# amaas/stanford-ctc

Measured on AMD Instinct MI355X. Metric: audio frames/sec (CTC fwd-bwd + BRNN grad) at T=1000, L=5, H=1824, |Sigma|=33, higher is better.
Workload: dtype f32; 1 GPU; WSJ-shape cfg-3: T=1000 A=33 5x1824 BRNN (temporalLayer 3, inputDim 483) U=100, minibatch 32 per GPU, one costAndGrad per step; utterances_per_gpu=32, parallelism=single-gpu

## Files before the change

### include/sctc.h

```cpp
#ifndef SCTC_H_
#define SCTC_H_

#include <stddef.h>
#include <stdint.h>

#ifdef __cplusplus
extern "C" {
#endif

#define SCTC_ABI_VERSION 6

#define SCTC_OK 0
#define SCTC_ERR_ARG (-1)
#define SCTC_ERR_HIP (-2)
#define SCTC_ERR_WORKSPACE (-3)
#define SCTC_ERR_TIMEOUT (-4)
#define SCTC_ERR_STATE (-5)

#define SCTC_F32 0
#define SCTC_F64 1
#define SCTC_F16 2
#define SCTC_BF16 3
#define SCTC_BF16X3 4
#define SCTC_OPERANDS_16BIT 0x100
// ... 262 lines not shown
int sctc_word_lm_score_batch(const sctc_word_lm_score_config* cfg, const int32_t* labels_dev, float* terms_dev,
                             int32_t* word_ids_dev, double* sums_dev, int32_t* counts_dev, int32_t* status_dev,
                             void* workspace_dev, size_t workspace_bytes, void* stream);

int sctc_nbest_rank_words_batch(int32_t B, int32_t K, const int32_t* K_b, const int32_t* U_b, double alpha, double beta,
                                const double* scores_dev, const int32_t* status_dev, const double* lm_sums_dev,
                                const double* first_scores_dev, const double* word_sums_dev,
                                const int32_t* word_counts_dev, const int32_t* word_status_dev, double word_alpha,
                                double word_beta, double* rescored_dev, int32_t* order_dev, void* stream);


typedef struct sctc_intern_config {
    int32_t N;
    int32_t G;
    int32_t A;
    int32_t space;
    const int32_t* U_b;
    const int64_t* label_off;
    const int32_t* group_off;
} sctc_intern_config;

int sctc_intern_words_workspace_bytes(const sctc_intern_config* cfg, size_t* bytes);

int sctc_intern_words_batch(const sctc_intern_config* cfg, const int32_t* labels_dev, int32_t* word_ids_dev,
                            int32_t* counts_dev, int32_t* status_dev, void* workspace_dev, size_t workspace_bytes,
                            void* stream);

#define SCTC_MBR_CHARS 0
#define SCTC_MBR_WORDS 1
#define SCTC_MBR_CONF 1
#define SCTC_MBR_DIST 2

typedef struct sctc_mbr_config {
    int32_t B;
    int32_t K;
    int32_t unit;
    int32_t flags;
    int32_t A;
    int32_t space;
    double scale;
    const int32_t* K_b;
    const int32_t* U_b;
    const int64_t* label_off;
} sctc_mbr_config;

int sctc_nbest_mbr_workspace_bytes(const sctc_mbr_config* cfg, size_t* bytes);

int sctc_nbest_mbr_batch(const sctc_mbr_config* cfg, const int32_t* labels_dev, const double* scores_dev,
                         const int32_t* order_dev, double* post_dev, double* risk_dev, int32_t* best_dev,
                         int32_t* mbr_order_dev, int32_t* dist_dev, double* conf_dev, int32_t* conf_len_dev,
                         void* workspace_dev, size_t workspace_bytes, void* stream);


#define SCTC_TNC_LOG_PROBS 0
#define SCTC_TNC_LOGITS 1

typedef struct sctc_tnc_config {
    int32_t T, N, C;
    int32_t dtype;
    int32_t mode;
    int32_t blank;
    int64_t stride_t, stride_n, stride_c;
} sctc_tnc_config;


int sctc_ctc_tnc_probs(const sctc_tnc_config* cfg, const void* input_dev, const int32_t* T_n_dev, void* probs_dev,
                       void* stream);

int sctc_ctc_tnc_empty(const sctc_tnc_config* cfg, const void* probs_dev, const int32_t* T_n_dev, const int32_t* idx_dev,
                       const int32_t* sym_dev, int32_t n_idx, void* grad_dev, double* cost_dev, int32_t* skip_dev,
                       void* stream);

int sctc_ctc_tnc_grad(const sctc_tnc_config* cfg, const void* grad_dev, const int32_t* T_n_dev, const double* cost_dev,
                      const int32_t* skip_dev, const double* scale_dev, void* out_dev, void* stream);

typedef struct sctc_mwer_config {
    int32_t T, N, K, C;
    int32_t dtype;
    int32_t mode;
    int64_t stride_t, stride_n, stride_c;
    double scale;
    int32_t subtract_mean;
} sctc_mwer_config;

int sctc_ctc_mwer_probs(const sctc_mwer_config* cfg, const void* input_dev, const int32_t* T_n_dev, const int32_t* K_n_dev,
                        void* probs_dev, void* stream);

int sctc_ctc_mwer_coef(const sctc_mwer_config* cfg, const double* cost_dev, const int32_t* skip_dev, const double* errors_dev,
                       const int32_t* T_n_dev, const int32_t* K_n_dev, double* loss_dev, double* coef_dev,
                       double* posterior_dev, double* expected_dev, int32_t* real_dev, int32_t* inactive_dev, void* stream);

int sctc_ctc_mwer_combine(const sctc_mwer_config* cfg, const void* probs_dev, const void* grad_dev, const double* coef_dev,
                          const int32_t* real_dev, const int32_t* T_n_dev, const int32_t* inactive_dev, void* out_dev,
                          void* stream);


typedef struct sctc_brnn_config {
    int32_t input_dim;
    int32_t output_dim;
    int32_t layer_size;
    int32_t num_layers;
    int32_t temporal_layer;
    int32_t max_frames;
    int32_t max_utts;
    float max_act;
    float reg;
    int32_t train;
    int32_t operand_dtype;
} sctc_brnn_config;

typedef struct sctc_tensor_info {
    int64_t offset;
    int32_t rows, cols, ld, kind;
} sctc_tensor_info;

typedef struct sctc_brnn_sizes {
    int64_t param_elems;
    int64_t param_count;
    size_t workspace_bytes;
    int32_t n_tensors;
} sctc_brnn_sizes;

typedef struct sctc_brnn* sctc_brnn_t;

int sctc_brnn_query(const sctc_brnn_config* cfg, sctc_brnn_sizes* out);
int sctc_brnn_create(const sctc_brnn_config* cfg, float* params_dev, float* grads_dev,
                     void* workspace_dev, size_t workspace_bytes, sctc_brnn_t* out);
int sctc_brnn_destroy(sctc_brnn_t h);
int sctc_brnn_tensor_info(sctc_brnn_t h, int32_t index, sctc_tensor_info* out);

typedef struct sctc_minibatch {
    int32_t B;
    const int32_t* T_b;
    const float* feats_dev;
    const int32_t* labels;
    const int32_t* U_b;
} sctc_minibatch;

#define SCTC_FLAG_SYNC_SKIP 1
#define SCTC_FLAG_ACCUMULATE 2
#define SCTC_FLAG_NO_REG_GRAD 4

int sctc_brnn_cost_and_grad(sctc_brnn_t h, const sctc_minibatch* mb, int32_t flags,
                            double* cost_host, int32_t* skip_host, double* regcost_host,
                            void* stream);
int sctc_brnn_cost_and_grad_async(sctc_brnn_t h, const sctc_minibatch* mb, int32_t flags,
                                  double* cost_dev, int32_t* skip_dev, void* stream);
void* sctc_brnn_grad_event(sctc_brnn_t h, int32_t index);
int sctc_stream_wait_event(void* stream, void* event);
int sctc_brnn_allreduce_grads(sctc_brnn_t h, void* rccl_comm, void* compute_stream, void* side_stream,
                              double* side_dev, int32_t side_count, int32_t backward_queued);
int sctc_brnn_check(sctc_brnn_t h, void* stream);
int sctc_brnn_recurrent_path(sctc_brnn_t h, int32_t* forward_path, int32_t* bptt_path, int32_t* retries);

int sctc_brnn_forward(sctc_brnn_t h, const sctc_minibatch* mb, float* probs_dev, void* stream);

int sctc_brnn_ctc_workspace_bytes(sctc_brnn_t h, const sctc_minibatch* mb, size_t* needed, size_t* reserved);
int sctc_brnn_set_ctc_workspace(sctc_brnn_t h, void* workspace_dev, size_t workspace_bytes);

typedef struct sctc_mwer_minibatch {
    int32_t K;
    const int32_t* K_b;
    const int32_t* hyp_labels;
    const int32_t* hyp_U;
    const double* errors;
    double scale;
    int32_t subtract_mean;
    double ctc_weight;
} sctc_mwer_minibatch;

typedef struct sctc_mwer_outputs {
    double* loss;
    double* expected;
    int32_t* inactive;
    double* ctc_cost;
    int32_t* ctc_skip;
    double* posterior;
    int32_t* real;
} sctc_mwer_outputs;

int sctc_brnn_mwer_workspace_bytes(sctc_brnn_t h, const sctc_minibatch* mb, const sctc_mwer_minibatch* mw, size_t* needed);
int sctc_brnn_set_mwer_workspace(sctc_brnn_t h, void* workspace_dev, size_t workspace_bytes);

int sctc_brnn_mwer_cost_and_grad(sctc_brnn_t h, const sctc_minibatch* mb, const sctc_mwer_minibatch* mw, int32_t flags,
                                 const sctc_mwer_outputs* out_host, double* regcost_host, void* stream);
int sctc_brnn_mwer_cost_and_grad_async(sctc_brnn_t h, const sctc_minibatch* mb, const sctc_mwer_minibatch* mw, int32_t flags,
                                       const sctc_mwer_outputs* out_dev, void* stream);

#define SCTC_PHASE_FWD_GEMM 0
#define SCTC_PHASE_FWD_REC 1
#define SCTC_PHASE_CTC 2
#define SCTC_PHASE_BWD_GEMM 3
#define SCTC_PHASE_BWD_REC 4
#define SCTC_PHASE_OTHER 5
#define SCTC_N_PHASES 6
int sctc_brnn_set_profiling(sctc_brnn_t h, int32_t enable);
int sctc_brnn_debug_buffer(sctc_brnn_t h, int32_t which, void** dev_ptr, int64_t* rows, int64_t* cols,
                           int64_t* ld);
int sctc_brnn_debug_buffer16(sctc_brnn_t h, int32_t which, void** dev_ptr, int64_t* rows, int64_t* cols,
                             int64_t* ld, int32_t* dtype);
int sctc_brnn_debug_read(sctc_brnn_t h, uint32_t* out, int32_t n_words);
int sctc_brnn_phase_ms(sctc_brnn_t h, float* ms_out );
int sctc_brnn_flops(sctc_brnn_t h, const sctc_minibatch* mb, double* total, double* gemm,
                    double* recurrent);

int sctc_gemm_f32(const float* A_dev, int64_t lda, int32_t a_kcontig, const float* B_dev,
                  int64_t ldb, int32_t b_kcontig, float* C_dev, int64_t ldc, int32_t M, int32_t N,
                  int32_t K, const float* bias_dev, int32_t relu, void* workspace_dev,
                  size_t workspace_bytes, void* stream);

int sctc_gemm_h16(const float* A_dev, int64_t lda, int32_t a_kcontig, const float* B_dev,
                  int64_t ldb, int32_t b_kcontig, float* C_dev, int64_t ldc, int32_t M, int32_t N,
                  int32_t K, const float* bias_dev, int32_t relu, int32_t operand_dtype,
                  void* workspace_dev, size_t workspace_bytes, void* stream);


int sctc_axpy(float* y_dev, const float* x_dev, float alpha, int64_t n, void* stream);
int sctc_scale(float* x_dev, float alpha, int64_t n, void* stream);
int sctc_sumsq(const float* x_dev, int64_t n, double* out_dev, void* workspace_dev,
               size_t workspace_bytes, void* stream);
int sctc_nesterov_step(float* w_dev, float* v_dev, const float* g_dev, int64_t n, float mom,
                       float alpha, float max_gnorm, float grad_scale, const double* sumsq_dev,
                       void* stream);

int sctc_sumsq_reg(const float* g_dev, const float* w_dev, const float* v_dev, float mom,
                   float grad_scale, float reg, int64_t n,
                   const int64_t* noreg_ranges_host, int32_t n_ranges, double* out_dev,
                   void* workspace_dev, size_t workspace_bytes, void* stream);
int sctc_nesterov_step_reg(float* w_dev, float* v_dev, const float* g_dev, int64_t n, float mom,
                           float alpha, float max_gnorm, float grad_scale, float reg,
                           const int64_t* noreg_ranges_host, int32_t n_ranges,
                           const double* sumsq_dev, void* stream);

#ifdef __cplusplus
}
#endif
#endif
```

### stanford-ctc_amd/_sctc.py

```python
import ctypes
import os

_HERE = os.path.dirname(os.path.abspath(__file__))
LIB_PATH = os.environ.get("SCTC_LIB_PATH") or os.path.join(_HERE, "libsctc_hip.so")

F32, F64, F16, BF16, BF16X3 = 0, 1, 2, 3, 4

c_i32p = ctypes.POINTER(ctypes.c_int32)
c_i64p = ctypes.POINTER(ctypes.c_int64)
c_f32p = ctypes.POINTER(ctypes.c_float)
c_f64p = ctypes.POINTER(ctypes.c_double)
vp = ctypes.c_void_p


class CtcBatch(ctypes.Structure):
    _fields_ = [("B", ctypes.c_int32), ("A", ctypes.c_int32), ("blank", ctypes.c_int32),
                ("dtype", ctypes.c_int32), ("ld", ctypes.c_int64), ("T_b", c_i32p),
                ("U_b", c_i32p), ("frame_off", c_i64p), ("labels", c_i32p),
                ("label_off", c_i64p), ("rowbase_dev", vp)]


class BrnnConfig(ctypes.Structure):
    _fields_ = [("input_dim", ctypes.c_int32), ("output_dim", ctypes.c_int32),
                ("layer_size", ctypes.c_int32), ("num_layers", ctypes.c_int32),
# ... 98 lines not shown


def word_lm_slots(U_b):
    import numpy as np
    per = (np.asarray(U_b, dtype=np.int64) + 1) // 2 + 1
    cuts = np.concatenate([[0], np.cumsum(per)]).astype(np.int64)
    return cuts[:-1], int(cuts[-1])


class InternConfig(ctypes.Structure):
    _fields_ = [("N", ctypes.c_int32), ("G", ctypes.c_int32), ("A", ctypes.c_int32), ("space", ctypes.c_int32),
                ("U_b", c_i32p), ("label_off", c_i64p), ("group_off", c_i32p)]


class MbrConfig(ctypes.Structure):
    _fields_ = [("B", ctypes.c_int32), ("K", ctypes.c_int32), ("unit", ctypes.c_int32), ("flags", ctypes.c_int32),
                ("A", ctypes.c_int32), ("space", ctypes.c_int32), ("scale", ctypes.c_double), ("K_b", c_i32p),
                ("U_b", c_i32p), ("label_off", c_i64p)]


MBR_CHARS, MBR_WORDS = 0, 1
MBR_CONF, MBR_DIST = 1, 2
MBR_MAX_U = ALIGN_MAX_U


def intern_slots(U_b):
    import numpy as np
    per = (np.asarray(U_b, dtype=np.int64) + 1) // 2
    cuts = np.concatenate([[0], np.cumsum(per)]).astype(np.int64)
    return cuts[:-1], int(cuts[-1])


class TncConfig(ctypes.Structure):
    _fields_ = [("T", ctypes.c_int32), ("N", ctypes.c_int32), ("C", ctypes.c_int32), ("dtype", ctypes.c_int32),
                ("mode", ctypes.c_int32), ("blank", ctypes.c_int32), ("stride_t", ctypes.c_int64),
                ("stride_n", ctypes.c_int64), ("stride_c", ctypes.c_int64)]


TNC_LOG_PROBS, TNC_LOGITS = 0, 1
TNC_LANE_MAX_C = 32


class MwerConfig(ctypes.Structure):
    _fields_ = [("T", ctypes.c_int32), ("N", ctypes.c_int32), ("K", ctypes.c_int32), ("C", ctypes.c_int32),
                ("dtype", ctypes.c_int32), ("mode", ctypes.c_int32), ("stride_t", ctypes.c_int64),
                ("stride_n", ctypes.c_int64), ("stride_c", ctypes.c_int64), ("scale", ctypes.c_double),
                ("subtract_mean", ctypes.c_int32)]


class MwerMinibatch(ctypes.Structure):
    _fields_ = [("K", ctypes.c_int32), ("K_b", c_i32p), ("hyp_labels", c_i32p), ("hyp_U", c_i32p), ("errors", c_f64p),
                ("scale", ctypes.c_double), ("subtract_mean", ctypes.c_int32), ("ctc_weight", ctypes.c_double)]


class MwerOutputs(ctypes.Structure):
    _fields_ = [("loss", vp), ("expected", vp), ("inactive", vp), ("ctc_cost", vp), ("ctc_skip", vp), ("posterior", vp),
                ("real", vp)]


MWER_MAX_K = 256

N_PHASES = 6

PROTOTYPES = {
    "sctc_abi_version": (ctypes.c_int, []),
    "sctc_last_error": (ctypes.c_char_p, []),
    "sctc_set_device": (ctypes.c_int, [ctypes.c_int]),
    "sctc_device_info": (ctypes.c_int, [c_i32p, c_i32p, c_i64p, ctypes.c_char_p, ctypes.c_int]),
    "sctc_set_shared_device": (ctypes.c_int, [ctypes.c_int32]),
    "sctc_shared_device": (ctypes.c_int, []),
    "sctc_device_pci_bus_id": (ctypes.c_int, [ctypes.c_int32, ctypes.c_char_p, ctypes.c_int32]),
    "sctc_ctc_workspace_bytes": (ctypes.c_size_t, [ctypes.POINTER(CtcBatch)]),
    "sctc_ctc_loss_batch": (ctypes.c_int, [ctypes.POINTER(CtcBatch), vp, vp, vp, vp, vp,
                                           ctypes.c_size_t, vp]),
    "sctc_softmax_rows": (ctypes.c_int, [vp, vp, ctypes.c_int64, ctypes.c_int32, ctypes.c_int64,
                                         vp]),
    "sctc_argmax_rows": (ctypes.c_int, [vp, ctypes.c_int32, vp, ctypes.c_int64, ctypes.c_int32,
                                        ctypes.c_int64, vp]),
    "sctc_lm_create": (ctypes.c_int, [vp, vp, vp, ctypes.c_int64, ctypes.c_int32, ctypes.c_int32,
                                      ctypes.POINTER(vp)]),
    "sctc_lm_destroy": (ctypes.c_int, [vp]),
    "sctc_ctc_beam_workspace_bytes": (ctypes.c_size_t, [ctypes.POINTER(BeamConfig)]),
    "sctc_ctc_beam_decode_batch": (ctypes.c_int, [ctypes.POINTER(BeamConfig), vp, vp, vp, vp, vp,
                                                  ctypes.c_size_t, vp]),
    "sctc_lexicon_create": (ctypes.c_int, [vp, vp, ctypes.c_int64, ctypes.c_int32, ctypes.c_int32, vp, vp,
                                           ctypes.c_int64, vp, vp, ctypes.c_int64, ctypes.c_int32,
                                           ctypes.POINTER(vp)]),
    "sctc_lexicon_create_ngram": (ctypes.c_int, [vp, vp, ctypes.c_int64, ctypes.c_int32, ctypes.c_int32, vp, vp,
                                                 ctypes.c_int64, vp, vp, vp, vp, ctypes.c_int64, ctypes.c_int64,
                                                 ctypes.c_int32, ctypes.c_int32, ctypes.POINTER(vp)]),
    "sctc_lexicon_destroy": (ctypes.c_int, [vp]),
    "sctc_lexicon_bytes": (ctypes.c_size_t, [vp]),
    "sctc_ctc_lexbeam_workspace_bytes": (ctypes.c_size_t, [ctypes.POINTER(LexBeamConfig)]),
    "sctc_ctc_lexbeam_decode_batch": (ctypes.c_int, [ctypes.POINTER(LexBeamConfig), vp, vp, vp, vp, vp,
                                                     ctypes.c_size_t, vp]),
    "sctc_nnlm_create": (ctypes.c_int, [ctypes.c_int32, ctypes.c_int32, ctypes.c_int32, c_i32p, ctypes.POINTER(vp),
                                        ctypes.POINTER(vp), ctypes.c_int32, ctypes.c_int32, ctypes.POINTER(vp)]),
    "sctc_nnlm_destroy": (ctypes.c_int, [vp]),
    "sctc_nnlm_bytes": (ctypes.c_size_t, [vp]),
    "sctc_nnlm_rows": (ctypes.c_int, [vp, vp, ctypes.c_int64, vp, vp]),
    "sctc_ctc_nnbeam_workspace_bytes": (ctypes.c_size_t, [ctypes.POINTER(NNBeamConfig)]),
    "sctc_ctc_nnbeam_decode_batch": (ctypes.c_int, [ctypes.POINTER(NNBeamConfig), vp, vp, vp, vp, vp,
                                                    ctypes.c_size_t, vp]),
    "sctc_rnnlm_create": (ctypes.c_int, [ctypes.c_int32, ctypes.c_int32, vp, vp, vp, vp, vp, ctypes.c_int32,
                                         ctypes.POINTER(vp)]),
    "sctc_rnnlm_destroy": (ctypes.c_int, [vp]),
    "sctc_rnnlm_bytes": (ctypes.c_size_t, [vp]),
    "sctc_rnnlm_step": (ctypes.c_int, [vp, vp, vp, ctypes.c_int64, vp, vp, vp]),
    "sctc_ctc_rnnbeam_workspace_bytes": (ctypes.c_size_t, [ctypes.POINTER(RNNBeamConfig)]),
    "sctc_ctc_rnnbeam_decode_batch": (ctypes.c_int, [ctypes.POINTER(RNNBeamConfig), vp, vp, vp, vp, vp,
                                                     ctypes.c_size_t, vp]),
    "sctc_edit_distance_workspace_bytes": (ctypes.c_int, [ctypes.POINTER(EditConfig), ctypes.POINTER(ctypes.c_size_t)]),
    "sctc_edit_distance_batch": (ctypes.c_int, [ctypes.POINTER(EditConfig), vp, vp, vp, vp, vp, vp, ctypes.c_size_t,
                                                vp]),
    "sctc_ctc_align_workspace_bytes": (ctypes.c_int, [ctypes.POINTER(AlignConfig), ctypes.POINTER(ctypes.c_size_t)]),
    "sctc_ctc_align_batch": (ctypes.c_int, [ctypes.POINTER(AlignConfig), vp, vp, vp, vp, vp, vp, vp, ctypes.c_size_t,
                                            vp]),
    "sctc_ctc_bestpath_batch": (ctypes.c_int, [ctypes.POINTER(BestPathConfig), vp, vp, vp, vp, vp, vp]),
    "sctc_log_rows": (ctypes.c_int, [vp, vp, ctypes.c_int64, ctypes.c_int32, ctypes.c_int64, vp]),
    "sctc_lm_score_workspace_bytes": (ctypes.c_int, [ctypes.POINTER(LmScoreConfig), ctypes.c_int32,
                                                     ctypes.POINTER(ctypes.c_size_t)]),
    "sctc_lm_score_batch": (ctypes.c_int, [ctypes.POINTER(LmScoreConfig), vp, vp, vp, vp, vp, ctypes.c_size_t, vp]),
    "sctc_nbest_rank_batch": (ctypes.c_int, [ctypes.c_int32, ctypes.c_int32, c_i32p, c_i32p, ctypes.c_double,
                                             ctypes.c_double, vp, vp, vp, vp, vp, vp, vp]),
    "sctc_word_lm_score_workspace_bytes": (ctypes.c_int, [ctypes.POINTER(WordLmScoreConfig),
                                                          ctypes.POINTER(ctypes.c_size_t)]),
    "sctc_word_lm_score_batch": (ctypes.c_int, [ctypes.POINTER(WordLmScoreConfig), vp, vp, vp, vp, vp, vp, vp,
                                                ctypes.c_size_t, vp]),
    "sctc_nbest_rank_words_batch": (ctypes.c_int, [ctypes.c_int32, ctypes.c_int32, c_i32p, c_i32p, ctypes.c_double,
                                                   ctypes.c_double, vp, vp, vp, vp, vp, vp, vp, ctypes.c_double,
                                                   ctypes.c_double, vp, vp, vp]),
    "sctc_intern_words_workspace_bytes": (ctypes.c_int, [ctypes.POINTER(InternConfig), ctypes.POINTER(ctypes.c_size_t)]),
    "sctc_intern_words_batch": (ctypes.c_int, [ctypes.POINTER(InternConfig), vp, vp, vp, vp, vp, ctypes.c_size_t, vp]),
    "sctc_nbest_mbr_workspace_bytes": (ctypes.c_int, [ctypes.POINTER(MbrConfig), ctypes.POINTER(ctypes.c_size_t)]),
    "sctc_nbest_mbr_batch": (ctypes.c_int, [ctypes.POINTER(MbrConfig), vp, vp, vp, vp, vp, vp, vp, vp, vp, vp, vp,
                                            ctypes.c_size_t, vp]),
    "sctc_ctc_tnc_probs": (ctypes.c_int, [ctypes.POINTER(TncConfig), vp, vp, vp, vp]),
    "sctc_ctc_tnc_empty": (ctypes.c_int, [ctypes.POINTER(TncConfig), vp, vp, vp, vp, ctypes.c_int32, vp, vp, vp, vp]),
    "sctc_ctc_tnc_grad": (ctypes.c_int, [ctypes.POINTER(TncConfig), vp, vp, vp, vp, vp, vp, vp]),
    "sctc_ctc_mwer_probs": (ctypes.c_int, [ctypes.POINTER(MwerConfig), vp, vp, vp, vp, vp]),
    "sctc_ctc_mwer_coef": (ctypes.c_int, [ctypes.POINTER(MwerConfig), vp, vp, vp, vp, vp, vp, vp, vp, vp, vp, vp, vp]),
    "sctc_ctc_mwer_combine": (ctypes.c_int, [ctypes.POINTER(MwerConfig), vp, vp, vp, vp, vp, vp, vp, vp]),
    "sctc_brnn_query": (ctypes.c_int, [ctypes.POINTER(BrnnConfig), ctypes.POINTER(BrnnSizes)]),
    "sctc_brnn_create": (ctypes.c_int, [ctypes.POINTER(BrnnConfig), vp, vp, vp, ctypes.c_size_t,
                                        ctypes.POINTER(vp)]),
    "sctc_brnn_destroy": (ctypes.c_int, [vp]),
    "sctc_brnn_tensor_info": (ctypes.c_int, [vp, ctypes.c_int32, ctypes.POINTER(TensorInfo)]),
    "sctc_brnn_cost_and_grad": (ctypes.c_int, [vp, ctypes.POINTER(Minibatch), ctypes.c_int32,
                                               c_f64p, c_i32p, c_f64p, vp]),
    "sctc_brnn_cost_and_grad_async": (ctypes.c_int, [vp, ctypes.POINTER(Minibatch),
                                                     ctypes.c_int32, vp, vp, vp]),
    "sctc_brnn_check": (ctypes.c_int, [vp, vp]),
    "sctc_brnn_recurrent_path": (ctypes.c_int, [vp, c_i32p, c_i32p, c_i32p]),
    "sctc_brnn_grad_event": (vp, [vp, ctypes.c_int32]),
    "sctc_stream_wait_event": (ctypes.c_int, [vp, vp]),
    "sctc_brnn_forward": (ctypes.c_int, [vp, ctypes.POINTER(Minibatch), vp, vp]),
    "sctc_brnn_ctc_workspace_bytes": (ctypes.c_int, [vp, ctypes.POINTER(Minibatch), ctypes.POINTER(ctypes.c_size_t),
                                                     ctypes.POINTER(ctypes.c_size_t)]),
    "sctc_brnn_set_ctc_workspace": (ctypes.c_int, [vp, vp, ctypes.c_size_t]),
    "sctc_brnn_mwer_workspace_bytes": (ctypes.c_int, [vp, ctypes.POINTER(Minibatch), ctypes.POINTER(MwerMinibatch),
                                                      ctypes.POINTER(ctypes.c_size_t)]),
    "sctc_brnn_set_mwer_workspace": (ctypes.c_int, [vp, vp, ctypes.c_size_t]),
    "sctc_brnn_mwer_cost_and_grad": (ctypes.c_int, [vp, ctypes.POINTER(Minibatch), ctypes.POINTER(MwerMinibatch),
                                                    ctypes.c_int32, ctypes.POINTER(MwerOutputs), c_f64p, vp]),
    "sctc_brnn_mwer_cost_and_grad_async": (ctypes.c_int, [vp, ctypes.POINTER(Minibatch), ctypes.POINTER(MwerMinibatch),
                                                          ctypes.c_int32, ctypes.POINTER(MwerOutputs), vp]),
    "sctc_brnn_set_profiling": (ctypes.c_int, [vp, ctypes.c_int32]),
    "sctc_brnn_debug_read": (ctypes.c_int, [vp, vp, ctypes.c_int32]),
    "sctc_brnn_debug_buffer": (ctypes.c_int, [vp, ctypes.c_int32, ctypes.POINTER(vp), c_i64p, c_i64p, c_i64p]),
    "sctc_brnn_debug_buffer16": (ctypes.c_int, [vp, ctypes.c_int32, ctypes.POINTER(vp), c_i64p, c_i64p, c_i64p, c_i32p]),
    "sctc_brnn_phase_ms": (ctypes.c_int, [vp, c_f32p]),
    "sctc_brnn_flops": (ctypes.c_int, [vp, ctypes.POINTER(Minibatch), c_f64p, c_f64p, c_f64p]),
    "sctc_gemm_f32": (ctypes.c_int, [vp, ctypes.c_int64, ctypes.c_int32, vp, ctypes.c_int64,
                                     ctypes.c_int32, vp, ctypes.c_int64, ctypes.c_int32,
                                     ctypes.c_int32, ctypes.c_int32, vp, ctypes.c_int32, vp,
                                     ctypes.c_size_t, vp]),
    "sctc_gemm_h16": (ctypes.c_int, [vp, ctypes.c_int64, ctypes.c_int32, vp, ctypes.c_int64,
                                     ctypes.c_int32, vp, ctypes.c_int64, ctypes.c_int32,
                                     ctypes.c_int32, ctypes.c_int32, vp, ctypes.c_int32,
                                     ctypes.c_int32, vp, ctypes.c_size_t, vp]),
    "sctc_axpy": (ctypes.c_int, [vp, vp, ctypes.c_float, ctypes.c_int64, vp]),
    "sctc_scale": (ctypes.c_int, [vp, ctypes.c_float, ctypes.c_int64, vp]),
    "sctc_sumsq": (ctypes.c_int, [vp, ctypes.c_int64, vp, vp, ctypes.c_size_t, vp]),
    "sctc_nesterov_step": (ctypes.c_int, [vp, vp, vp, ctypes.c_int64, ctypes.c_float,
                                          ctypes.c_float, ctypes.c_float, ctypes.c_float, vp,
                                          vp]),
    "sctc_brnn_allreduce_grads": (ctypes.c_int, [vp, vp, vp, vp, vp, ctypes.c_int32, ctypes.c_int32]),
    "sctc_sumsq_reg": (ctypes.c_int, [vp, vp, vp, ctypes.c_float, ctypes.c_float, ctypes.c_float, ctypes.c_int64,
                                      c_i64p, ctypes.c_int32, vp, vp, ctypes.c_size_t, vp]),
    "sctc_nesterov_step_reg": (ctypes.c_int, [vp, vp, vp, ctypes.c_int64, ctypes.c_float,
                                              ctypes.c_float, ctypes.c_float, ctypes.c_float,
                                              ctypes.c_float, c_i64p, ctypes.c_int32, vp, vp]),
}

FLAG_SYNC_SKIP = 1
FLAG_ACCUMULATE = 2
FLAG_NO_REG_GRAD = 4

_lib = None


class SctcError(RuntimeError):
    pass


def device_bus_id(device=-1):
    buf = ctypes.create_string_buffer(64)
    check(lib().sctc_device_pci_bus_id(device, buf, 64), "device_pci_bus_id")
    return buf.value.decode()


def shared_device_from_ids(ids, rank):
    me = tuple(ids[rank])
    return sum(1 for x in ids if tuple(x) == me) > 1


def resolve_shared_device(group=None, my_id=None, log=True, device=None):
    import socket
    import sys
    import torch.distributed as dist
    L = lib()
    if my_id is None:
        my_id = (socket.gethostname(), device_bus_id(-1 if device is None else int(device)))
    rank, ids = 0, [tuple(my_id)]
    if dist.is_available() and dist.is_initialized() and dist.get_world_size(group) > 1:
        rank = dist.get_rank(group)
        gathered = [None] * dist.get_world_size(group)
        dist.all_gather_object(gathered, tuple(my_id), group=group)
        ids = [tuple(x) for x in gathered]
    if "SCTC_SHARED_DEVICE" in os.environ:
        shared, why = bool(L.sctc_shared_device()), "SCTC_SHARED_DEVICE in the environment"
    else:
        shared, why = shared_device_from_ids(ids, rank), "bus ids of %d rank(s)" % len(ids)
        if shared:
            L.sctc_set_shared_device(1)
        elif L.sctc_shared_device():
            why += "; the mode was already on (a timeout or another process on this GPU) and stays on"
            shared = True
    if log:
        sys.stderr.write("sctc: rank %d -> %s %s, shared=%d (%s)\n"
                         % (rank, my_id[0], my_id[1], int(shared), why))
        sys.stderr.flush()
    return shared, ids


def lib():
    global _lib
    if _lib is None:
        if not os.path.exists(LIB_PATH):
            raise ImportError(
                "libsctc_hip.so is missing (%s): build it with `python -c 'import "
                "__graft_entry__ as g; g.build()'` -- there is no CPU fallback" % LIB_PATH)
        try:
            import torch
        except ImportError:
            pass
        L = ctypes.CDLL(LIB_PATH)
        for name, (res, args) in PROTOTYPES.items():
            fn = getattr(L, name)
            fn.restype = res
            fn.argtypes = args
        if L.sctc_abi_version() != 6:
            raise ImportError("libsctc_hip.so ABI version mismatch")
        _lib = L
    return _lib


def check(rc, what=""):
    if rc < 0:
        msg = lib().sctc_last_error()
        msg = msg.decode() if msg else ""
        if rc == -1:
            raise ValueError("%s: %s" % (what, msg))
        raise SctcError("%s failed (rc=%d): %s" % (what, rc, msg))
    return rc


def require_gpu():
    import torch
    if not torch.cuda.is_available():
        raise SctcError("no HIP device visible: the stanford-ctc MI355X path has no CPU fallback")
    return torch


def current_stream_ptr():
    import torch
    return ctypes.c_void_p(torch.cuda.current_stream().cuda_stream)


def i32(arr):
    return arr.ctypes.data_as(c_i32p)


def i64(arr):
    return arr.ctypes.data_as(c_i64p)
```

### stanford-ctc_amd/csrc/brnn_engine.hip

```cpp
#include <algorithm>
#include <cmath>
#include <numeric>
#include <vector>

#include "common.h"
#include <dlfcn.h>

#include <mutex>

#include "brnn_mwer.h"
#include "brnn_mwer_plan.h"
#include "ctc_kernels.h"
#include "elementwise.h"
#include "gemm_f32.h"
#include "recurrent.h"

namespace sctc {
int ctc_run_batch(const sctc_ctc_batch* bt, const void* probs, void* grad, double* cost,
                  int32_t* skip, void* ws, size_t ws_bytes, hipStream_t stream, void* keep_stage);
void* ctc_new_stage();
void ctc_free_stage(void* p);
}

using namespace sctc;

static constexpr int PAD = 32;
static inline int LD(int padded_dim) { return (int)((padded_dim + 63) / 64 * 64); }
static constexpr int CTC_LP_MAX = 2048;

static int fwd_prec(int operand_dtype)
{
    return operand_dtype == SCTC_F16 ? 1 : (operand_dtype == SCTC_BF16X3 ? 3 : 0);
}
static int bwd_prec(int operand_dtype)
{
    return operand_dtype == SCTC_F16 ? 2 : (operand_dtype == SCTC_BF16X3 ? 3 : 0);
}

struct sctc_brnn {
    sctc_brnn_config cfg;
    int D, Dp, H, Hp, A, Ap, NL, TL;
    int64_t maxF;
    int maxB;
    float* params;
    float* grads;
    std::vector<sctc_tensor_info> tinfo;
    int64_t param_elems, param_count;

    float* X0;
    std::vector<float*> act;
    float *Z, *hF, *hB;
    float *logits, *probs, *dlogits;
    float *dA, *dBuf, *dF, *dBk;
    std::vector<uint16_t*> act16f, act16b;
    uint16_t *hF16b = nullptr, *hB16b = nullptr, *dF16b = nullptr, *dBk16b = nullptr;
    uint16_t *dlogits16 = nullptr, *dA16 = nullptr, *dBuf16 = nullptr;
    uint16_t* W16f = nullptr;
    std::vector<uint16_t*> WT16b;
    int32_t *d_rowbase, *d_nact, *d_Ts, *d_src_row, *d_idx_lo, *d_idx_hi, *d_xbase;
    void* ctc_ws;
    size_t ctc_ws_bytes;
    void* ctc_ws_ext = nullptr;
    size_t ctc_ws_ext_bytes = 0;
    float* splitk_ws;
    int64_t splitk_floats;
    float* xbuf;
    unsigned* counters;
    unsigned* rec_debug = nullptr;
    int rec_debug_on = 0;
    double* d_cost;
    int32_t* d_skip;
    double* d_cost_out;
    int32_t* d_skip_out;
    double* d_sumsq;
    double* sumsq_ws;
    int32_t* d_perm;

    std::vector<int32_t> order, Ts, rowbase, nact, src_row, idx_lo, idx_hi, xbase;
    int64_t n_xrows = 0;
    int64_t N = 0;
    int B = 0, Tmax = 0;
    int64_t npairs = 0;
    bool pairs_contig = false;

    std::vector<hipEvent_t> grad_ev;

    int profiling = 0;
    std::vector<hipEvent_t> tev;
    int tev_phase[128];
    int tev_n = 0;
    hipEvent_t ev[SCTC_N_PHASES + 1][2];
    bool ev_ready = false;
    float phase_ms[SCTC_N_PHASES];
    int rec_sync_mode = 0;
    bool fuse_add = true;
    int rec_poll_delay = -1;
    int rec_variant = REC_V_AUTO;
    int rec_force_fallback = 0;
    int rec_path[2] = {0, 0};
    int rec_retries = 0;
    const float* last_delta1 = nullptr;
    const uint16_t* last_delta1_16 = nullptr;
    void* ctc_stage = nullptr;
    PinnedStage plan_stage;
    std::vector<int32_t> ctc_U, ctc_labels;
    std::vector<int64_t> ctc_frame_off, ctc_label_off;
    void* mwer_ws = nullptr;
    size_t mwer_ws_bytes = 0;
    PinnedStage mwer_stage;
    std::vector<int32_t> mwer_T;
    std::vector<char> mwer_head;
};

static int weight_index(const sctc_brnn* h, int layer) { return 2 * layer; }
static int bias_index(const sctc_brnn* h, int layer) { return 2 * layer + 1; }
static int wf_index(const sctc_brnn* h) { return 2 * (h->NL + 1); }
static int wb_index(const sctc_brnn* h) { return 2 * (h->NL + 1) + 1; }

struct Dims {
    int D, Dp, H, Hp, A, Ap, NL, TL;
};

static int derive_dims(const sctc_brnn_config* c, Dims* d)
{
    SCTC_CHECK_ARG(c, "brnn: null config");
    SCTC_CHECK_ARG(c->input_dim >= 1 && c->output_dim >= 2 && c->layer_size >= 1 &&
                       c->num_layers >= 1,
                   "brnn: bad dimensions (inputDim %d outputDim %d layerSize %d numLayers %d)",
                   c->input_dim, c->output_dim, c->layer_size, c->num_layers);
    SCTC_CHECK_ARG(c->max_frames >= 1 && c->max_utts >= 1, "brnn: bad capacity");
    SCTC_CHECK_ARG(c->operand_dtype == SCTC_F32 || c->operand_dtype == SCTC_F16 || c->operand_dtype == SCTC_BF16X3,
                   "brnn: operand_dtype must be SCTC_F32, SCTC_F16 or SCTC_BF16X3 (got %d)", c->operand_dtype);
    d->D = c->input_dim;
    d->H = c->layer_size;
    d->A = c->output_dim;
    d->NL = c->num_layers;
    d->TL = (c->temporal_layer <= 0 || c->temporal_layer >= c->num_layers) ? -1 : c->temporal_layer;
    d->Dp = (int)round_up(d->D, PAD);
    d->Hp = (int)round_up(d->H, PAD);
    d->Ap = (int)round_up(d->A, PAD);
    if (d->TL > 0) {
        char why[128];
        if (!recurrent_supported(d->Hp, c->max_utts, why, sizeof(why)))
            return set_error(SCTC_ERR_ARG, "brnn: %s", why);
    }
    return SCTC_OK;
}

static void build_tensor_table(const Dims& d, std::vector<sctc_tensor_info>* t, int64_t* elems,
                               int64_t* count)
{
    t->clear();
    int64_t off = 0, cnt = 0;
    for (int l = 0; l <= d.NL; ++l) {
        const int in = l == 0 ? d.D : d.H, inp = l == 0 ? d.Dp : d.Hp;
        const int out = l == d.NL ? d.A : d.H, outp = l == d.NL ? d.Ap : d.Hp;
        sctc_tensor_info w = {off, out, in, LD(inp), 0};
        t->push_back(w);
        off += (int64_t)outp * LD(inp);
        sctc_tensor_info b = {off, out, 1, 1, 1};
        t->push_back(b);
        off += outp;
        cnt += (int64_t)out * in + out;
    }
    if (d.TL > 0) {
        for (int k = 0; k < 2; ++k) {
            sctc_tensor_info w = {off, d.H, d.H, LD(d.Hp), 2};
            t->push_back(w);
            off += (int64_t)d.Hp * LD(d.Hp);
            cnt += (int64_t)d.H * d.H;
        }
    }
    *elems = off;
    *count = cnt;
}

static size_t carve(const sctc_brnn_config* c, const Dims& d, sctc_brnn* h, void* ws, size_t bytes)
{
    Arena ar;
    ar.init(ws ? ws : (void*)256, ws ? bytes : (size_t)-1 / 2);
    const int64_t F = c->max_frames;
    const int Bm = c->max_utts;
    auto f = [&](int64_t n) { return ar.take<float>((size_t)n); };
    float* X0 = f(F * LD(d.Dp));
    std::vector<float*> act(d.NL + 1);
    act[0] = X0;
    for (int i = 1; i <= d.NL; ++i) act[i] = f(F * LD(d.Hp));
    float *Z = nullptr, *hF = nullptr, *hB = nullptr;
    if (d.TL > 0) { Z = f(F * LD(d.Hp)); hF = f(F * LD(d.Hp)); hB = f(F * LD(d.Hp)); }
    float* logits = f(F * LD(d.Ap));
    float* probs = f(F * LD(d.Ap));
    float *dlogits = nullptr, *dA = nullptr, *dBuf = nullptr, *dF = nullptr, *dBk = nullptr;
    if (c->train) {
        dlogits = f(F * LD(d.Ap));
        dA = f(F * LD(d.Hp));
        dBuf = f(F * LD(d.Hp));
        if (d.TL > 0) { dF = f(F * LD(d.Hp)); dBk = f(F * LD(d.Hp)); }
    }
    const bool h16 = c->operand_dtype == SCTC_F16;
    std::vector<uint16_t*> act16f(d.NL + 1, nullptr), act16b(d.NL + 1, nullptr), WT16b(d.NL + 1, nullptr);
    uint16_t *hF16b = nullptr, *hB16b = nullptr, *dF16b = nullptr, *dBk16b = nullptr, *dlogits16 = nullptr,
             *dA16 = nullptr, *dBuf16 = nullptr, *W16f = nullptr;
    if (h16) {
        auto hh = [&](int64_t n) { return ar.take<uint16_t>((size_t)n); };
        int64_t pe = 0, pc = 0;
        {
            std::vector<sctc_tensor_info> t;
            build_tensor_table(d, &t, &pe, &pc);
        }
        W16f = hh(pe);
        for (int i = 0; i <= d.NL; ++i) {
            const int dim = i == 0 ? d.Dp : d.Hp;
            act16f[i] = hh(F * LD(dim));
            if (c->train) act16b[i] = hh(F * LD(dim));
        }
        if (c->train) {
            for (int l = 1; l <= d.NL; ++l) {
                const int outp = l == d.NL ? d.Ap : d.Hp;
                WT16b[l] = hh((int64_t)d.Hp * LD(outp));
            }
            dlogits16 = hh(F * LD(d.Ap));
            dA16 = hh(F * LD(d.Hp));
            dBuf16 = hh(F * LD(d.Hp));
            if (d.TL > 0) {
                hF16b = hh(F * LD(d.Hp)); hB16b = hh(F * LD(d.Hp));
                dF16b = hh(F * LD(d.Hp)); dBk16b = hh(F * LD(d.Hp));
            }
        }
    }
    int32_t* d_rowbase = ar.take<int32_t>(F);
    int32_t* d_nact = ar.take<int32_t>(F);
    int32_t* d_Ts = ar.take<int32_t>(Bm);
    int32_t* d_src_row = ar.take<int32_t>(F);
    int32_t* d_idx_lo = ar.take<int32_t>(F);
    int32_t* d_idx_hi = ar.take<int32_t>(F);
    int32_t* d_xbase = ar.take<int32_t>(F);
    int32_t* d_perm = ar.take<int32_t>(Bm);
    size_t ctc_bytes = 0;
    void* ctc_ws = nullptr;
    if (c->train) {
        ctc_bytes = ctc_layout_slices(CTC_GENERIC, Bm, d.A, F, F * CTC_LP_MAX, CTC_LP_MAX, 8).bytes;
        ctc_ws = ar.take<char>(ctc_bytes);
    }
    const int64_t sk = brnn_splitk_floats(d.Dp, d.Hp, d.Ap, d.NL, d.TL > 0, F, c->train != 0, bwd_prec(c->operand_dtype),
                                          c->operand_dtype == SCTC_F16, gemm_switches_from_env());
    float* splitk_ws = sk ? f(sk) : nullptr;
    float* xbuf = d.TL > 0 ? f((int64_t)recurrent_xbuf_floats(d.Hp, recurrent_xrows_bound(F, F))) : nullptr;
    unsigned* counters = ar.take<unsigned>(REC_COUNTER_WORDS);
    unsigned* rec_debug = ar.take<unsigned>(2 * REC_DEBUG_WORDS);
    double* d_cost = ar.take<double>(Bm);
    int32_t* d_skip = ar.take<int32_t>(Bm);
    double* d_cost_out = ar.take<double>(Bm);
    int32_t* d_skip_out = ar.take<int32_t>(Bm);
    double* d_sumsq = ar.take<double>(d.NL + 3);
    double* sumsq_ws = ar.take<double>(sumsq_ws_bytes() / sizeof(double));
    if (h && !ar.overflow) {
        h->X0 = X0; h->act = act; h->Z = Z; h->hF = hF; h->hB = hB;
        h->logits = logits; h->probs = probs; h->dlogits = dlogits;
        h->dA = dA; h->dBuf = dBuf; h->dF = dF; h->dBk = dBk;
        h->d_rowbase = d_rowbase; h->d_nact = d_nact; h->d_Ts = d_Ts; h->d_src_row = d_src_row;
        h->d_idx_lo = d_idx_lo; h->d_idx_hi = d_idx_hi; h->d_perm = d_perm; h->d_xbase = d_xbase;
        h->ctc_ws = ctc_ws; h->ctc_ws_bytes = ctc_bytes;
        h->splitk_ws = splitk_ws; h->splitk_floats = sk;
        h->xbuf = xbuf; h->counters = counters; h->rec_debug = rec_debug;
        h->act16f = act16f; h->act16b = act16b; h->WT16b = WT16b; h->W16f = W16f;
        h->hF16b = hF16b; h->hB16b = hB16b; h->dF16b = dF16b; h->dBk16b = dBk16b;
        h->dlogits16 = dlogits16; h->dA16 = dA16; h->dBuf16 = dBuf16;
        h->d_cost = d_cost; h->d_skip = d_skip; h->d_cost_out = d_cost_out;
        h->d_skip_out = d_skip_out; h->d_sumsq = d_sumsq; h->sumsq_ws = sumsq_ws;
    }
    return ar.overflow && ws ? 0 : ar.used;
}


static int make_plan(sctc_brnn* h, const sctc_minibatch* mb, bool need_labels, hipStream_t stream)
{
    SCTC_CHECK_ARG(mb && mb->T_b && mb->feats_dev, "brnn: null minibatch field");
    SCTC_CHECK_ARG(mb->B >= 1 && mb->B <= h->maxB, "brnn: %d utterances, capacity %d", mb->B,
                   h->maxB);
    if (need_labels) SCTC_CHECK_ARG(mb->labels && mb->U_b, "brnn: labels required for training");
    const int B = mb->B;
    int64_t N = 0;
    for (int b = 0; b < B; ++b) {
        SCTC_CHECK_ARG(mb->T_b[b] >= 1, "brnn: utterance %d has no frames", b);
        N += mb->T_b[b];
    }
    SCTC_CHECK_ARG(N <= h->maxF, "Batch size exceeds max batch (%lld frames > %lld)", (long long)N,
                   (long long)h->maxF);
    h->B = B;
    h->N = N;
    h->order.resize(B);
    std::iota(h->order.begin(), h->order.end(), 0);
    std::stable_sort(h->order.begin(), h->order.end(),
                     [&](int a, int b) { return mb->T_b[a] > mb->T_b[b]; });
    h->Ts.resize(B);
    std::vector<int64_t> foff(B);
    {
        int64_t o = 0;
        for (int b = 0; b < B; ++b) { foff[b] = o; o += mb->T_b[b]; }
    }
    for (int r = 0; r < B; ++r) h->Ts[r] = mb->T_b[h->order[r]];
    const int Tmax = h->Ts[0];
    h->Tmax = Tmax;
    h->rowbase.assign(Tmax, 0);
    h->nact.assign(Tmax, 0);
    h->xbase.assign(Tmax, 0);
    {
        int na = B;
        int64_t base = 0, xb = 0;
        for (int t = 0; t < Tmax; ++t) {
            while (na > 0 && h->Ts[na - 1] <= t) --na;
            h->nact[t] = na;
            h->rowbase[t] = (int32_t)base;
            h->xbase[t] = (int32_t)xb;
            base += na;
            xb += recurrent_step_xrows(na);
        }
        h->n_xrows = xb;
    }
    h->src_row.resize(N);
    h->idx_lo.clear();
    h->idx_hi.clear();
    for (int t = 0; t < Tmax; ++t)
        for (int r = 0; r < h->nact[t]; ++r) {
            const int row = h->rowbase[t] + r;
            h->src_row[row] = (int32_t)(foff[h->order[r]] + t);
            if (t >= 1) {
                h->idx_hi.push_back(row);
                h->idx_lo.push_back(h->rowbase[t - 1] + r);
            }
        }
    h->npairs = (int64_t)h->idx_hi.size();
    h->pairs_contig = h->npairs > 0;
    for (int64_t k = 1; k < h->npairs && h->pairs_contig; ++k)
        h->pairs_contig = h->idx_hi[k] == h->idx_hi[0] + k && h->idx_lo[k] == h->idx_lo[0] + k;
    const size_t I = sizeof(int32_t);
    const size_t total = I * (3 * (size_t)Tmax + 2 * (size_t)B + (size_t)N + 2 * (size_t)h->npairs) + 8 * 64;
    char* pin = static_cast<char*>(h->plan_stage.acquire(total));
    size_t off = 0;
    auto up = [&](void* dev, const void* src, size_t bytes) -> int {
        if (bytes == 0) return SCTC_OK;
        const void* from = src;
        if (pin) {
            memcpy(pin + off, src, bytes);
            from = pin + off;
            off += (bytes + 63) & ~(size_t)63;
        }
        SCTC_HIP_TRY(hipMemcpyAsync(dev, from, bytes, hipMemcpyHostToDevice, stream));
        return SCTC_OK;
    };
    SCTC_TRY(up(h->d_rowbase, h->rowbase.data(), I * Tmax));
    SCTC_TRY(up(h->d_nact, h->nact.data(), I * Tmax));
    SCTC_TRY(up(h->d_xbase, h->xbase.data(), I * Tmax));
    SCTC_TRY(up(h->d_Ts, h->Ts.data(), I * B));
    SCTC_TRY(up(h->d_src_row, h->src_row.data(), I * N));
    SCTC_TRY(up(h->d_perm, h->order.data(), I * B));
    SCTC_TRY(up(h->d_idx_lo, h->idx_lo.data(), I * h->npairs));
    SCTC_TRY(up(h->d_idx_hi, h->idx_hi.data(), I * h->npairs));
    if (pin) SCTC_HIP_TRY(h->plan_stage.uploaded(stream));
    return SCTC_OK;
}


struct PhaseTimer {
    sctc_brnn* h;
    hipStream_t s;
    int cur = -1;
    void mark(int phase)
    {
        if (h->tev_n >= (int)h->tev.size()) return;
        (void)hipEventRecord(h->tev[h->tev_n], s);
        h->tev_phase[h->tev_n++] = phase;
    }
    void begin(int phase)
    {
        if (!h->profiling) return;
        if (h->profiling == 2) { mark(phase); return; }
        end();
        cur = phase;
        (void)hipEventRecord(h->ev[SCTC_N_PHASES][0], s);
    }
    void end()
    {
        if (h->profiling == 2) { mark(-1); return; }
        if (!h->profiling || cur < 0) return;
        (void)hipEventRecord(h->ev[SCTC_N_PHASES][1], s);
        (void)hipEventSynchronize(h->ev[SCTC_N_PHASES][1]);
        float ms = 0.f;
        (void)hipEventElapsedTime(&ms, h->ev[SCTC_N_PHASES][0], h->ev[SCTC_N_PHASES][1]);
        h->phase_ms[cur] += ms;
        cur = -1;
    }
};

struct GemmOperand { const float* p; int64_t ld; int kcontig; };
static GemmArgs gemm_args(GemmOperand A, GemmOperand B, int64_t M, int64_t N, int64_t K, float* C, int64_t ldc, int prec)
{
    GemmArgs g;
    memset(&g, 0, sizeof(g));
    g.A = A.p; g.lda = A.ld; g.a_kcontig = A.kcontig;
    g.B = B.p; g.ldb = B.ld; g.b_kcontig = B.kcontig;
    g.M = (int)M; g.N = (int)N; g.K = (int)K;
    g.C = C; g.ldc = ldc;
    g.prec = prec;
    g.splits = 1;
    return g;
}

static int launch_gemm(const sctc_brnn* h, GemmArgs& g, hipStream_t s)
{
    const GemmPlan p = gemm_plan(g);
    if (p.splits > 1 && h->splitk_ws && p.ws_floats <= h->splitk_floats) {
        g.splits = p.splits;
        g.splitk_ws = h->splitk_ws;
    }
    return launch_gemm_f32(g, s);
}

static const float* tensor_ptr(const sctc_brnn* h, const float* base, int idx)
{
    return base + h->tinfo[idx].offset;
}

static RecArgs rec_args(const sctc_brnn* h, bool bptt, float* pre)
{
    RecArgs r;
    memset(&r, 0, sizeof(r));
    r.W[0] = tensor_ptr(h, h->params, wf_index(h));
    r.W[1] = tensor_ptr(h, h->params, wb_index(h));
    r.ldw = LD(h->Hp);
    r.transpose = bptt;
    r.descending[0] = bptt;
    r.descending[1] = !bptt;
    r.pre[0] = r.pre[1] = pre;
    r.act[0] = bptt ? h->hF : nullptr;
    r.act[1] = bptt ? h->hB : nullptr;
    r.out[0] = bptt ? h->dF : h->hF;
    r.out[1] = bptt ? h->dBk : h->hB;
    r.ld = LD(h->Hp);
    r.Hp = h->Hp;
    r.B = h->B;
    r.Tmax = h->Tmax;
    r.rowbase = h->d_rowbase;
    r.T_b = h->d_Ts;
    r.max_act = h->cfg.max_act;
    r.xbuf = h->xbuf;
    r.xbase = h->d_xbase;
    r.n_xrows = (int)h->n_xrows;
    r.counters = h->counters;
    r.sync_mode = h->rec_sync_mode;
    r.variant = h->rec_force_fallback ? REC_V_FALLBACK : h->rec_variant;
    r.poll_delay = h->rec_poll_delay;
    r.debug = h->rec_debug_on ? h->rec_debug + (bptt ? REC_DEBUG_WORDS : 0) : nullptr;
    r.prec16 = h->cfg.operand_dtype == SCTC_F16;
    r.T_host = h->Ts.data();
    return r;
}


static int run_forward(sctc_brnn* h, const sctc_minibatch* mb, hipStream_t s, PhaseTimer& pt)
{
    const int64_t N = h->N;
    pt.begin(SCTC_PHASE_OTHER);
    const bool h16 = h->cfg.operand_dtype == SCTC_F16;
    if (h16) {
        SCTC_TRY(launch_gather_rows16(h->X0, h->act16f[0], h->cfg.train ? h->act16b[0] : nullptr, LD(h->Dp),
                                      mb->feats_dev, h->D, h->d_src_row, N, h->D, s));
        SCTC_TRY(launch_cvt16(h->params, h->W16f, nullptr, round_up(h->param_elems, 4), s));
    } else {
        SCTC_TRY(launch_gather_rows(h->X0, LD(h->Dp), mb->feats_dev, h->D, h->d_src_row, N, h->D, s));
    }
    bool fused_sum = false;
    for (int i = 1; i <= h->NL + 1; ++i) {
        pt.begin(SCTC_PHASE_FWD_GEMM);
        const int l = i - 1;
        const sctc_tensor_info& wi = h->tinfo[weight_index(h, l)];
        const int inp = l == 0 ? h->Dp : h->Hp;
        const int outp = i == h->NL + 1 ? h->Ap : h->Hp;
        float* dst = i == h->NL + 1 ? h->logits : (i == h->TL ? h->Z : h->act[i]);
        GemmArgs g = gemm_args({h->act[i - 1], LD(inp), 1}, {h->params + wi.offset, LD(inp), 1}, N, outp, inp, dst, LD(outp),
                               fwd_prec(h->cfg.operand_dtype));
        g.bias = tensor_ptr(h, h->params, bias_index(h, l));
        g.relu = (i <= h->NL && i != h->TL) ? 1 : 0;
        if (fused_sum) {
            g.A = h->hF;
            g.A2 = h->hB;
            g.a_sum = h->act[i - 1];
            fused_sum = false;
        }
        if (h16) {
            g.in16 = 1;
            g.A = reinterpret_cast<const float*>(h->act16f[i - 1]);
            g.B = reinterpret_cast<const float*>(h->W16f + wi.offset);
            if (dst != h->Z && dst != h->logits) {
                g.C16a = h->act16f[i];
                g.C16b = h->cfg.train ? h->act16b[i] : nullptr;
                g.ldc16 = LD(outp);
                g.skip_c32 = 1;
            }
        }
        SCTC_TRY(launch_gemm(h, g, s));
        if (i == h->TL) {
            pt.begin(SCTC_PHASE_FWD_REC);
            const RecArgs r = rec_args(h, false, h->Z);
            SCTC_TRY(launch_recurrent(r, s, &h->rec_path[0]));
            pt.begin(SCTC_PHASE_OTHER);
            if (h16) {
                SCTC_TRY(launch_add16(nullptr, h->hF, h->hB, h->act16f[i], h->cfg.train ? h->act16b[i] : nullptr,
                                      N * LD(h->Hp), s, h->cfg.train ? h->hF16b : nullptr,
                                      h->cfg.train ? h->hB16b : nullptr));
            } else if (g.prec == 0 && h->fuse_add) {
                fused_sum = true;
            } else {
                SCTC_TRY(launch_add(h->act[i], h->hF, h->hB, N * LD(h->Hp), s));
            }
        }
    }
    pt.begin(SCTC_PHASE_CTC);
    SCTC_TRY(launch_softmax_rows(h->logits, h->probs, N, h->A, LD(h->Ap), s));
    return SCTC_OK;
}

static int check_recurrent_error(sctc_brnn* h, hipStream_t s)
{
    if (h->TL <= 0) return SCTC_OK;
    unsigned e = 0;
    SCTC_HIP_TRY(hipMemcpyAsync(&e, h->counters + 2, sizeof(unsigned), hipMemcpyDeviceToHost, s));
    SCTC_HIP_TRY(hipStreamSynchronize(s));
    if (e != 0) {
        if (!recurrent_shared_device_mode())
            fprintf(stderr, "sctc: a persistent recurrent launch timed out (its workgroups were not co-resident): "
                            "shared-device mode is on for the rest of this process\n");
        recurrent_set_shared_device_mode(1);
        return set_error(SCTC_ERR_TIMEOUT, "recurrent kernel: a persistent launch gave up waiting for "
                         "its peers (the %d workgroups of a pass were not co-resident: device shared "
                         "with another process or CU-masked); shared-device mode is now on",
                         2 * (h->Hp / 16));
    }
    return SCTC_OK;
}

template <typename Step>
static int with_retry(sctc_brnn* h, bool retry_ok, Step step)
{
    int rc = step();
    for (int attempt = 0; rc == SCTC_ERR_TIMEOUT && retry_ok && attempt < 2; ++attempt) {
        if (getenv("SCTC_VERBOSE"))
            fprintf(stderr, "sctc: %s -- retrying the step %s\n", err_buf(),
                    attempt == 0 ? "under the device lease" : "on the per-step fallback");
        ++h->rec_retries;
        h->rec_force_fallback = attempt == 1;
        rc = step();
        h->rec_force_fallback = 0;
    }
    return rc;
}


static int run_ctc(sctc_brnn* h, const sctc_minibatch* mb, hipStream_t s)
{
    const int B = h->B;
    std::vector<int32_t>& U = h->ctc_U;
    std::vector<int32_t>& labels = h->ctc_labels;
    std::vector<int64_t>& frame_off = h->ctc_frame_off;
    std::vector<int64_t>& label_off = h->ctc_label_off;
    U.assign(B, 0);
    labels.clear();
    frame_off.assign(B, 0);
    label_off.assign(B, 0);
    std::vector<int64_t> src_off(B);
    {
        int64_t o = 0;
        for (int b = 0; b < B; ++b) { src_off[b] = o; o += mb->U_b[b]; }
    }
    for (int r = 0; r < B; ++r) {
        const int b = h->order[r];
        U[r] = mb->U_b[b];
        frame_off[r] = r;
        label_off[r] = (int64_t)labels.size();
        labels.insert(labels.end(), mb->labels + src_off[b], mb->labels + src_off[b] + mb->U_b[b]);
    }
    sctc_ctc_batch bt;
    bt.B = B;
    bt.A = h->A;
    bt.blank = 0;
    bt.dtype = SCTC_F32;
    bt.ld = LD(h->Ap);
    bt.T_b = h->Ts.data();
    bt.U_b = U.data();
    bt.frame_off = frame_off.data();
    bt.labels = labels.data();
    bt.label_off = label_off.data();
    bt.rowbase_dev = h->d_rowbase;
    if (!h->ctc_stage) h->ctc_stage = ctc_new_stage();
    return ctc_run_batch(&bt, h->probs, h->dlogits, h->d_cost, h->d_skip, h->ctc_ws_ext ? h->ctc_ws_ext : h->ctc_ws,
                         h->ctc_ws_ext ? h->ctc_ws_ext_bytes : h->ctc_ws_bytes, s, h->ctc_stage);
}

__global__ void unpermute_results_kernel(const double* cost, const int32_t* skip,
                                         const int32_t* perm, int B, double* cost_out,
                                         int32_t* skip_out)
{
    const int r = blockIdx.x * blockDim.x + threadIdx.x;
    if (r < B) {
        cost_out[perm[r]] = cost[r];
        skip_out[perm[r]] = skip[r];
    }
}

static int run_backward(sctc_brnn* h, int flags, hipStream_t s, PhaseTimer& pt)
{
    const int64_t N = h->N;
    const int acc = (flags & SCTC_FLAG_ACCUMULATE) ? 1 : 0;
    const float reg = (flags & SCTC_FLAG_NO_REG_GRAD) ? 0.f : h->cfg.reg;
    const int bprec = bwd_prec(h->cfg.operand_dtype);
    const bool h16 = h->cfg.operand_dtype == SCTC_F16;
    const float* d_in = h->dlogits;
    const uint16_t* d_in16 = h->dlogits16;
    int d_in_ld = LD(h->Ap);
    float* bufs[2] = {h->dA, h->dBuf};
    uint16_t* bufs16[2] = {h->dA16, h->dBuf16};
    if (h16) {
        SCTC_TRY(launch_cvt16(h->dlogits, nullptr, h->dlogits16, N * LD(h->Ap), s));
        for (int l = 1; l <= h->NL; ++l) {
            const sctc_tensor_info& wl = h->tinfo[weight_index(h, l)];
            const int outp = l == h->NL ? h->Ap : h->Hp;
            SCTC_TRY(launch_transpose_bf16(h->params + wl.offset, LD(h->Hp), h->WT16b[l], LD(outp), outp, h->Hp, s));
        }
    }
    int which = 0;
    bool fused_sum = false;
    for (int i = h->NL; i >= 0; --i) {
        pt.begin(SCTC_PHASE_BWD_GEMM);
        const sctc_tensor_info& wi = h->tinfo[weight_index(h, i)];
        const int inp = i == 0 ? h->Dp : h->Hp;
        const int outp = i == h->NL ? h->Ap : h->Hp;
        const float* W = h->params + wi.offset;
        {
            GemmArgs g = gemm_args({d_in, d_in_ld, 0}, {h->act[i], LD(inp), 0}, outp, inp, N, h->grads + wi.offset, LD(inp), bprec);
            if (fused_sum) {
                g.A = h->dF;
                g.A2 = h->dBk;
                g.a_sum = const_cast<float*>(d_in);
                fused_sum = false;
            }
            g.accumulate = acc;
            if (reg > 0.f) { g.addend = W; g.ldadd = LD(inp); g.add_scale = reg; }
            g.colsum_a = h->grads + h->tinfo[bias_index(h, i)].offset;
            g.splitk_ws = h->splitk_ws;
            if (h16) {
                g.in16 = 1;
                g.A = reinterpret_cast<const float*>(d_in16);
                g.B = reinterpret_cast<const float*>(h->act16b[i]);
            }
            SCTC_TRY(launch_gemm(h, g, s));
            if (!(h->TL > 0 && i >= h->TL))
                SCTC_HIP_TRY(hipEventRecord(h->grad_ev[weight_index(h, i)], s));
        }
        if (i == 0) break;
        pt.begin(SCTC_PHASE_BWD_GEMM);
        float* d_out = bufs[which];
        {
            GemmArgs g = gemm_args({d_in, d_in_ld, 1}, {W, LD(inp), 0}, N, inp, outp, d_out, LD(inp), bprec);
            if (i != h->TL) { g.mask = h->act[i]; g.ldmask = LD(h->Hp); }
            if (h16) {
                g.in16 = 1;
                g.A = reinterpret_cast<const float*>(d_in16);
                g.B = reinterpret_cast<const float*>(h->WT16b[i]);
                g.ldb = LD(outp);
                g.b_kcontig = 1;
                g.C16b = bufs16[which];
                g.ldc16 = LD(inp);
                if (i != h->TL) {
                    g.mask = nullptr;
                    g.mask16 = h->act16b[i];
                    g.ldmask16 = LD(h->Hp);
                    g.skip_c32 = 1;
                }
            }
            SCTC_TRY(launch_gemm(h, g, s));
        }
        if (i == h->TL) {
            pt.begin(SCTC_PHASE_BWD_REC);
            const RecArgs r = rec_args(h, true, d_out);
            SCTC_TRY(launch_recurrent(r, s, &h->rec_path[1]));
            for (int l = h->NL; l >= h->TL; --l)
                SCTC_HIP_TRY(hipEventRecord(h->grad_ev[weight_index(h, l)], s));
            pt.begin(SCTC_PHASE_BWD_GEMM);
            if (h16) SCTC_TRY(launch_add16(nullptr, h->dF, h->dBk, nullptr, bufs16[which], N * LD(h->Hp), s,
                                           h->dF16b, h->dBk16b));
            for (int k = 0; k < 2; ++k) {
                const sctc_tensor_info& ri = h->tinfo[k == 0 ? wf_index(h) : wb_index(h)];
                GemmArgs g = gemm_args({k == 0 ? h->dF : h->dBk, LD(h->Hp), 0}, {k == 0 ? h->hF : h->hB, LD(h->Hp), 0}, h->Hp, h->Hp,
                                       h->npairs, h->grads + ri.offset, LD(h->Hp), bprec);
                const uint16_t* a16 = k == 0 ? h->dF16b : h->dBk16b;
                const uint16_t* b16 = k == 0 ? h->hF16b : h->hB16b;
                if (h->pairs_contig) {
                    const int64_t hi0 = h->idx_hi[0], lo0 = h->idx_lo[0];
                    g.A += (k == 0 ? hi0 : lo0) * LD(h->Hp);
                    g.B += (k == 0 ? lo0 : hi0) * LD(h->Hp);
                    a16 += (k == 0 ? hi0 : lo0) * LD(h->Hp);
                    b16 += (k == 0 ? lo0 : hi0) * LD(h->Hp);
                } else {
                    g.idx_a = k == 0 ? h->d_idx_hi : h->d_idx_lo;
                    g.idx_b = k == 0 ? h->d_idx_lo : h->d_idx_hi;
                }
                g.accumulate = acc;
                if (reg > 0.f) {
                    g.addend = h->params + ri.offset;
                    g.ldadd = LD(h->Hp);
                    g.add_scale = reg;
                }
                g.splitk_ws = h->splitk_ws;
                if (h16) {
                    g.in16 = 1;
                    g.A = reinterpret_cast<const float*>(a16);
                    g.B = reinterpret_cast<const float*>(b16);
                }
                SCTC_TRY(launch_gemm(h, g, s));
                SCTC_HIP_TRY(hipEventRecord(h->grad_ev[k == 0 ? wf_index(h) : wb_index(h)], s));
            }
            pt.begin(SCTC_PHASE_OTHER);
            if (!h16) {
                if (bprec == 0 && h->fuse_add) fused_sum = true;
                else SCTC_TRY(launch_add(d_out, h->dF, h->dBk, N * LD(h->Hp), s));
            }
        }
        d_in = d_out;
        d_in16 = bufs16[which];
        d_in_ld = LD(h->Hp);
        which ^= 1;
    }
    h->last_delta1 = d_in;
    h->last_delta1_16 = h16 ? d_in16 : nullptr;
    return SCTC_OK;
}

static int run_cost_and_grad(sctc_brnn* h, const sctc_minibatch* mb, int flags, hipStream_t s,
                             bool* all_skipped)
{
    SCTC_CHECK_ARG(h && h->cfg.train, "brnn: model was created with train=0");
    PhaseTimer pt{h, s};
    if (h->profiling) memset(h->phase_ms, 0, sizeof(h->phase_ms));
    h->tev_n = 0;
    SCTC_TRY(make_plan(h, mb, true, s));
    if (h->TL > 0) SCTC_TRY(recurrent_clear_error(h->counters, s));
    SCTC_TRY(run_forward(h, mb, s, pt));
    SCTC_TRY(run_ctc(h, mb, s));
    pt.begin(SCTC_PHASE_OTHER);
    hipLaunchKernelGGL(unpermute_results_kernel, dim3((h->B + 63) / 64), dim3(64), 0, s, h->d_cost,
                       h->d_skip, h->d_perm, h->B, h->d_cost_out, h->d_skip_out);
    *all_skipped = false;
    if (flags & SCTC_FLAG_SYNC_SKIP) {
        std::vector<int32_t> sk(h->B);
        SCTC_HIP_TRY(hipMemcpyAsync(sk.data(), h->d_skip, sizeof(int32_t) * h->B,
                                    hipMemcpyDeviceToHost, s));
        SCTC_HIP_TRY(hipStreamSynchronize(s));
        bool all = true;
        for (int v : sk) all = all && v != 0;
        *all_skipped = all;
    }
    if (!*all_skipped) SCTC_TRY(run_backward(h, flags, s, pt));
    pt.end();
    return SCTC_OK;
}


static int mwer_check_desc(const sctc_mwer_minibatch* mw, const char* what)
{
    SCTC_CHECK_ARG(mw, "%s: null MWER descriptor", what);
    SCTC_CHECK_ARG(mw->K >= 1 && mw->K <= BRNN_MWER_MAX_K, "%s: K = %d hypotheses outside 1..%d", what, mw->K, BRNN_MWER_MAX_K);
    SCTC_CHECK_ARG(std::isfinite(mw->scale) && mw->scale >= 0.0, "%s: scale %g is not finite or is negative", what, mw->scale);
    SCTC_CHECK_ARG(std::isfinite(mw->ctc_weight) && mw->ctc_weight >= 0.0, "%s: ctc_weight %g is not finite or is negative", what,
                   mw->ctc_weight);
    SCTC_CHECK_ARG(mw->subtract_mean == 0 || mw->subtract_mean == 1, "%s: subtract_mean %d is neither 0 nor 1", what,
                   mw->subtract_mean);
    SCTC_CHECK_ARG(mw->K_b && mw->hyp_U && mw->errors, "%s: null field in the MWER descriptor", what);
    return SCTC_OK;
}

struct MwerHost {
    std::vector<int32_t> T, U, labels;
    std::vector<int64_t> frame_off, label_off;
    std::vector<int32_t> src, kb;
    std::vector<double> errors;
    BrnnMwerPlan plan;
};

static int mwer_prepare(const sctc_brnn* h, const sctc_minibatch* mb, const sctc_mwer_minibatch* mw, const char* what, MwerHost* out)
{
    SCTC_CHECK_ARG(mb && mb->T_b, "%s: null minibatch field", what);
    SCTC_CHECK_ARG(mb->B >= 1 && mb->B <= h->maxB, "%s: %d utterances, capacity %d", what, mb->B, h->maxB);
    const int B = mb->B, K = mw->K, A = h->A;
    const bool with_ref = mw->ctc_weight > 0.0;
    const int S = K + (with_ref ? 1 : 0);
    if (with_ref) SCTC_CHECK_ARG(mb->labels && mb->U_b, "%s: ctc_weight > 0 needs the reference labels", what);
    int64_t N = 0;
    int Tmax = 0;
    for (int b = 0; b < B; ++b) {
        SCTC_CHECK_ARG(mb->T_b[b] >= 1, "%s: utterance %d has no frames", what, b);
        N += mb->T_b[b];
        Tmax = std::max(Tmax, mb->T_b[b]);
    }
    SCTC_CHECK_ARG(N <= h->maxF, "Batch size exceeds max batch (%lld frames > %lld)", (long long)N, (long long)h->maxF);
    SCTC_CHECK_ARG(N * S <= INT32_MAX, "%s: N * S = %lld rows do not fit the int32 row index", what, (long long)(N * S));
    std::vector<int64_t> hyp_off((size_t)B * K, -1), ref_off(B, 0);
    {
        int64_t at = 0, rat = 0;
        for (int b = 0; b < B; ++b) {
            SCTC_CHECK_ARG(mw->K_b[b] >= 0 && mw->K_b[b] <= K, "%s: K_b[%d] = %d outside 0..%d", what, b, mw->K_b[b], K);
            for (int k = 0; k < mw->K_b[b]; ++k) {
                const int64_t o = (int64_t)b * K + k;
                if (!std::isfinite(mw->errors[o])) continue;
                const int32_t U = mw->hyp_U[o];
                SCTC_CHECK_ARG(U >= 0, "%s: hypothesis %d of utterance %d has length %d", what, k, b, U);
                SCTC_CHECK_ARG(U == 0 || mw->hyp_labels, "%s: null hyp_labels", what);
                for (int i = 0; i < U; ++i)
                    SCTC_CHECK_ARG(mw->hyp_labels[at + i] >= 1 && mw->hyp_labels[at + i] < A, "%s: label %d of hypothesis %d of "
                                   "utterance %d is %d, outside [1, %d)", what, i, k, b, mw->hyp_labels[at + i], A);
                hyp_off[o] = at;
                at += U;
            }
            if (with_ref) {
                const int32_t U = mb->U_b[b];
                SCTC_CHECK_ARG(U >= 1, "%s: utterance %d has an empty reference label sequence", what, b);
                for (int i = 0; i < U; ++i)
                    SCTC_CHECK_ARG(mb->labels[rat + i] >= 1 && mb->labels[rat + i] < A, "%s: reference label %d of utterance %d is "
                                   "%d, outside [1, %d)", what, i, b, mb->labels[rat + i], A);
                ref_off[b] = rat;
                rat += U;
            }
        }
    }
    std::vector<int> order(B);
    std::iota(order.begin(), order.end(), 0);
    std::stable_sort(order.begin(), order.end(), [&](int a, int b) { return mb->T_b[a] > mb->T_b[b]; });
    MwerHost& m = *out;
    m.T.clear(); m.U.clear(); m.labels.clear(); m.frame_off.clear(); m.label_off.clear();
    m.src.assign((size_t)B * S, BRNN_MWER_SRC_UNREAD);
    m.kb.assign(B, 0);
    m.errors.assign((size_t)B * K, 0.0);
    auto add_row = [&](int r, int s, int T, int U, const int32_t* lab) {
        m.src[(size_t)r * S + s] = (int32_t)m.T.size();
        m.T.push_back(T);
        m.U.push_back(U);
        m.frame_off.push_back((int64_t)r * S + s);
        m.label_off.push_back((int64_t)m.labels.size());
        m.labels.insert(m.labels.end(), lab, lab + U);
    };
    for (int r = 0; r < B; ++r) {
        const int b = order[r];
        m.kb[r] = mw->K_b[b];
        for (int k = 0; k < K; ++k) {
            const int64_t o = (int64_t)b * K + k;
            m.errors[(size_t)r * K + k] = mw->errors[o];
            if (hyp_off[o] < 0) continue;
            if (mw->hyp_U[o] == 0) m.src[(size_t)r * S + k] = BRNN_MWER_SRC_EMPTY;
            else add_row(r, k, mb->T_b[b], mw->hyp_U[o], mw->hyp_labels + hyp_off[o]);
        }
        if (with_ref) add_row(r, K, mb->T_b[b], mb->U_b[b], mb->labels + ref_off[b]);
    }
    size_t ctc_bytes = 0;
    if (!m.T.empty())
        SCTC_TRY(ctc_workspace_bytes((int)m.T.size(), A, 0, SCTC_F32, m.T.data(), m.U.data(), &ctc_bytes));
    m.plan = brnn_mwer_plan(B, K, with_ref, A, N, Tmax, ctc_bytes);
    return SCTC_OK;
}

static int run_mwer(sctc_brnn* h, const sctc_mwer_minibatch* mw, MwerHost& m, hipStream_t s)
{
    const BrnnMwerPlan& pl = m.plan;
    const int B = pl.B, K = pl.K, S = pl.S;
    char* const base = static_cast<char*>(h->mwer_ws);
    {
        std::vector<int32_t> rb(pl.Tmax);
        for (int t = 0; t < pl.Tmax; ++t) rb[t] = h->rowbase[t] * S;
        char* pin = static_cast<char*>(h->mwer_stage.acquire(pl.head_bytes));
        h->mwer_head.resize(pin ? 0 : pl.head_bytes);
        char* host = pin ? pin : h->mwer_head.data();
        memset(host, 0, pl.head_bytes);
        memcpy(host + pl.off_errors, m.errors.data(), sizeof(double) * m.errors.size());
        memcpy(host + pl.off_rowbase, rb.data(), sizeof(int32_t) * rb.size());
        memcpy(host + pl.off_kb, m.kb.data(), sizeof(int32_t) * m.kb.size());
        memcpy(host + pl.off_src, m.src.data(), sizeof(int32_t) * m.src.size());
// ... 34 lines not shown
        bt.B = (int32_t)m.T.size();
        bt.A = h->A;
        bt.blank = 0;
        bt.dtype = SCTC_F32;
        bt.ld = pl.ldk;
        bt.T_b = m.T.data();
        bt.U_b = m.U.data();
        bt.frame_off = m.frame_off.data();
        bt.labels = m.labels.data();
        bt.label_off = m.label_off.data();
        bt.rowbase_dev = a.rowbase_S;
        if (!h->ctc_stage) h->ctc_stage = ctc_new_stage();
        SCTC_TRY(ctc_run_batch(&bt, a.kprobs, a.kgrad, const_cast<double*>(a.ctc_cost), const_cast<int32_t*>(a.ctc_skip),
                               at(pl.off_ctc), pl.ctc_bytes, s, h->ctc_stage));
    }
    SCTC_TRY(launch_brnn_mwer_empty(a, s));
    sctc_mwer_config mc;
    memset(&mc, 0, sizeof(mc));
    mc.T = pl.Tmax; mc.N = B; mc.K = K; mc.C = h->A;
    mc.dtype = SCTC_F32;
    mc.mode = SCTC_TNC_LOGITS;
    mc.scale = mw->scale;
    mc.subtract_mean = mw->subtract_mean;
    SCTC_TRY(sctc_ctc_mwer_coef(&mc, a.cost, a.skip, reinterpret_cast<const double*>(at(pl.off_errors)), h->d_Ts, a.kb,
                                reinterpret_cast<double*>(at(pl.off_loss)), const_cast<double*>(a.coef),
                                reinterpret_cast<double*>(at(pl.off_post)), reinterpret_cast<double*>(at(pl.off_expected)),
                                const_cast<int32_t*>(a.real), const_cast<int32_t*>(a.inactive), s));
    SCTC_TRY(launch_brnn_mwer_combine(a, s));
    BrnnMwerResults rs;
    memset(&rs, 0, sizeof(rs));
    rs.perm = h->d_perm;
    rs.loss = reinterpret_cast<const double*>(at(pl.off_loss));
    rs.expected = reinterpret_cast<const double*>(at(pl.off_expected));
    rs.post = reinterpret_cast<const double*>(at(pl.off_post));
    rs.ref_cost = a.ref_cost;
    rs.inactive = a.inactive;
    rs.real = a.real;
    rs.ref_skip = a.ref_skip;
    rs.out_loss = reinterpret_cast<double*>(at(pl.off_out_loss));
    rs.out_expected = reinterpret_cast<double*>(at(pl.off_out_expected));
    rs.out_post = reinterpret_cast<double*>(at(pl.off_out_post));
    rs.out_ctc_cost = reinterpret_cast<double*>(at(pl.off_out_ctc_cost));
    rs.out_inactive = reinterpret_cast<int32_t*>(at(pl.off_out_inactive));
    rs.out_real = reinterpret_cast<int32_t*>(at(pl.off_out_real));
    rs.out_ctc_skip = reinterpret_cast<int32_t*>(at(pl.off_out_ctc_skip));
    rs.ctc_weight = mw->ctc_weight;
    rs.B = B; rs.K = K; rs.with_ref = S > K;
    return launch_brnn_mwer_results(rs, s);
}

static int run_mwer_cost_and_grad(sctc_brnn* h, const sctc_minibatch* mb, const sctc_mwer_minibatch* mw, int flags,
                                  const sctc_mwer_outputs* out, bool out_on_host, hipStream_t s)
{
    SCTC_TRY(mwer_check_desc(mw, "brnn_mwer"));
    SCTC_CHECK_ARG(h, "brnn_mwer: null handle");
    SCTC_CHECK_ARG(h->cfg.train, "brnn_mwer: model was created with train=0");
    SCTC_CHECK_ARG(!(flags & SCTC_FLAG_SYNC_SKIP), "brnn_mwer: SCTC_FLAG_SYNC_SKIP does not apply to the MWER step");
    SCTC_CHECK_ARG(mb && mb->feats_dev, "brnn_mwer: null minibatch field");
    MwerHost m;
    SCTC_TRY(mwer_prepare(h, mb, mw, "brnn_mwer", &m));
    if (m.plan.bytes > h->mwer_ws_bytes || !h->mwer_ws)
        return set_error(SCTC_ERR_WORKSPACE, "brnn_mwer: workspace %zu bytes < %zu needed (sctc_brnn_set_mwer_workspace)",
                         h->mwer_ws_bytes, m.plan.bytes);
    PhaseTimer pt{h, s};
    if (h->profiling) memset(h->phase_ms, 0, sizeof(h->phase_ms));
    h->tev_n = 0;
    SCTC_TRY(make_plan(h, mb, false, s));
    if (h->TL > 0) SCTC_TRY(recurrent_clear_error(h->counters, s));
    SCTC_TRY(run_forward(h, mb, s, pt));
    SCTC_TRY(run_mwer(h, mw, m, s));
    pt.begin(SCTC_PHASE_OTHER);
    SCTC_TRY(run_backward(h, flags, s, pt));
    pt.end();
    if (out) {
        const BrnnMwerPlan& pl = m.plan;
        const char* base = static_cast<const char*>(h->mwer_ws);
        const hipMemcpyKind kind = out_on_host ? hipMemcpyDeviceToHost : hipMemcpyDeviceToDevice;
        const size_t nB = (size_t)pl.B, nBK = (size_t)pl.B * pl.K;
        auto copy = [&](void* dst, size_t off, size_t bytes) -> int {
            if (dst) SCTC_HIP_TRY(hipMemcpyAsync(dst, base + off, bytes, kind, s));
            return SCTC_OK;
        };
        SCTC_TRY(copy(out->loss, pl.off_out_loss, nB * sizeof(double)));
        SCTC_TRY(copy(out->expected, pl.off_out_expected, nB * sizeof(double)));
        SCTC_TRY(copy(out->inactive, pl.off_out_inactive, nB * sizeof(int32_t)));
        SCTC_TRY(copy(out->ctc_cost, pl.off_out_ctc_cost, nB * sizeof(double)));
        SCTC_TRY(copy(out->ctc_skip, pl.off_out_ctc_skip, nB * sizeof(int32_t)));
        SCTC_TRY(copy(out->posterior, pl.off_out_post, nBK * sizeof(double)));
        SCTC_TRY(copy(out->real, pl.off_out_real, nBK * sizeof(int32_t)));
    }
    return SCTC_OK;
}

extern "C" {

int sctc_brnn_query(const sctc_brnn_config* cfg, sctc_brnn_sizes* out)
{
    SCTC_CHECK_ARG(out, "brnn_query: null output");
    Dims d;
    SCTC_TRY(derive_dims(cfg, &d));
    std::vector<sctc_tensor_info> t;
    build_tensor_table(d, &t, &out->param_elems, &out->param_count);
    out->n_tensors = (int32_t)t.size();
    out->workspace_bytes = carve(cfg, d, nullptr, nullptr, 0);
    return SCTC_OK;
}

int sctc_brnn_create(const sctc_brnn_config* cfg, float* params_dev, float* grads_dev,
                     void* workspace_dev, size_t workspace_bytes, sctc_brnn_t* out)
{
    SCTC_CHECK_ARG(out && params_dev && workspace_dev, "brnn_create: null argument");
    Dims d;
    SCTC_TRY(derive_dims(cfg, &d));
    SCTC_CHECK_ARG(!cfg->train || grads_dev, "brnn_create: train model needs a gradient buffer");
    SCTC_CHECK_ARG(((uintptr_t)params_dev & 15) == 0 && ((uintptr_t)workspace_dev & 255) == 0,
                   "brnn_create: params must be 16-byte and workspace 256-byte aligned");
    sctc_brnn* h = new sctc_brnn();
    h->cfg = *cfg;
    h->D = d.D; h->Dp = d.Dp; h->H = d.H; h->Hp = d.Hp; h->A = d.A; h->Ap = d.Ap;
    h->NL = d.NL; h->TL = d.TL;
    h->maxF = cfg->max_frames;
    h->maxB = cfg->max_utts;
    h->params = params_dev;
    h->grads = grads_dev;
    build_tensor_table(d, &h->tinfo, &h->param_elems, &h->param_count);
    const size_t need = carve(cfg, d, nullptr, nullptr, 0);
    if (workspace_bytes < need) {
        delete h;
        return set_error(SCTC_ERR_WORKSPACE, "brnn_create: workspace %zu bytes < %zu needed",
                         workspace_bytes, need);
    }
    carve(cfg, d, h, workspace_dev, workspace_bytes);
    hipError_t e = hipSuccess;
    if (cfg->train) e = hipMemset(h->dlogits, 0, sizeof(float) * h->maxF * LD(h->Ap));
    if (e == hipSuccess) e = hipMemset(h->counters, 0, sizeof(unsigned) * REC_COUNTER_WORDS);
    if (e != hipSuccess) {
        delete h;
        return set_error(SCTC_ERR_HIP, "brnn_create: %s", hipGetErrorString(e));
    }
    h->grad_ev.resize(h->tinfo.size(), nullptr);
    for (size_t i = 0; i < h->tinfo.size(); ++i)
        if (cfg->train && h->tinfo[i].kind != 1 &&
            hipEventCreateWithFlags(&h->grad_ev[i], hipEventDisableTiming) != hipSuccess) {
            delete h;
            return set_error(SCTC_ERR_HIP, "brnn_create: hipEventCreate failed");
        }
    const char* sm = getenv("SCTC_REC_SYNC");
    h->rec_sync_mode = sm ? atoi(sm) : 1;
    const char* rv = getenv("SCTC_REC_VARIANT");
    h->rec_variant = rv ? atoi(rv) : REC_V_AUTO;
    const char* pd = getenv("SCTC_REC_POLL_DELAY");
    h->rec_poll_delay = pd ? atoi(pd) : -1;
    if (const char* fa = getenv("SCTC_FUSE_ADD")) h->fuse_add = atoi(fa) != 0;
    const char* dbg = getenv("SCTC_REC_DEBUG");
    h->rec_debug_on = dbg ? atoi(dbg) : 0;
    *out = h;
    return SCTC_OK;
}

int sctc_brnn_destroy(sctc_brnn_t h)
{
    if (!h) return SCTC_OK;
    if (h->ev_ready)
        for (int i = 0; i <= SCTC_N_PHASES; ++i) {
            (void)hipEventDestroy(h->ev[i][0]);
            (void)hipEventDestroy(h->ev[i][1]);
        }
    if (h->ctc_stage) ctc_free_stage(h->ctc_stage);
    for (hipEvent_t e : h->grad_ev)
        if (e) (void)hipEventDestroy(e);
    for (hipEvent_t e : h->tev)
        if (e) (void)hipEventDestroy(e);
    delete h;
    return SCTC_OK;
}

int sctc_brnn_tensor_info(sctc_brnn_t h, int32_t index, sctc_tensor_info* out)
{
    SCTC_CHECK_ARG(h && out && index >= 0 && index < (int)h->tinfo.size(),
                   "brnn_tensor_info: bad index %d", index);
    *out = h->tinfo[index];
    return SCTC_OK;
}

int sctc_brnn_cost_and_grad_async(sctc_brnn_t h, const sctc_minibatch* mb, int32_t flags,
                                  double* cost_dev, int32_t* skip_dev, void* stream)
{
    hipStream_t s = (hipStream_t)stream;
    bool all_skipped = false;
    SCTC_TRY(run_cost_and_grad(h, mb, flags, s, &all_skipped));
    if (cost_dev)
        SCTC_HIP_TRY(hipMemcpyAsync(cost_dev, h->d_cost_out, sizeof(double) * h->B,
                                    hipMemcpyDeviceToDevice, s));
    if (skip_dev)
        SCTC_HIP_TRY(hipMemcpyAsync(skip_dev, h->d_skip_out, sizeof(int32_t) * h->B,
                                    hipMemcpyDeviceToDevice, s));
    return SCTC_OK;
}

void* sctc_brnn_grad_event(sctc_brnn_t h, int32_t index)
{
    if (!h || index < 0 || index >= (int)h->grad_ev.size()) {
        set_error(SCTC_ERR_ARG, "brnn_grad_event: bad index %d", index);
        return nullptr;
    }
    return (void*)h->grad_ev[index];
}

int sctc_stream_wait_event(void* stream, void* event)
{
    SCTC_CHECK_ARG(event, "stream_wait_event: null event");
    SCTC_HIP_TRY(hipStreamWaitEvent((hipStream_t)stream, (hipEvent_t)event, 0));
    return SCTC_OK;
}

namespace {
struct Rccl {
    typedef int (*AllReduce)(const void*, void*, size_t, int, int, void*, hipStream_t);
    typedef const char* (*ErrStr)(int);
    void* lib = nullptr;
    AllReduce all_reduce = nullptr;
    ErrStr err_str = nullptr;
    bool tried = false;
};
Rccl g_rccl;
std::mutex g_rccl_mu;
}

int sctc_brnn_allreduce_grads(sctc_brnn_t h, void* rccl_comm, void* compute_stream, void* side_stream,
                              double* side_dev, int32_t side_count, int32_t backward_queued)
{
    SCTC_CHECK_ARG(h && rccl_comm, "brnn_allreduce_grads: null handle / communicator");
    SCTC_CHECK_ARG(h->grads, "brnn_allreduce_grads: the model has no gradient buffer (train = 0)");
    SCTC_CHECK_ARG(side_stream && side_stream != compute_stream, "brnn_allreduce_grads: needs a side stream of its own");
    SCTC_CHECK_ARG(side_count >= 0 && (side_count == 0 || side_dev), "brnn_allreduce_grads: bad side message");
    Rccl::AllReduce rccl_all_reduce = nullptr;
    Rccl::ErrStr rccl_err_str = nullptr;
    {
        std::lock_guard<std::mutex> lock(g_rccl_mu);
        if (!g_rccl.tried) {
            g_rccl.tried = true;
            const char* names[3] = {"librccl.so.1", "librccl.so", "/opt/rocm/lib/librccl.so"};
            for (int k = 0; k < 3 && !g_rccl.lib; ++k) g_rccl.lib = dlopen(names[k], RTLD_NOW | RTLD_GLOBAL);
            if (g_rccl.lib) {
                g_rccl.all_reduce = (Rccl::AllReduce)dlsym(g_rccl.lib, "ncclAllReduce");
                g_rccl.err_str = (Rccl::ErrStr)dlsym(g_rccl.lib, "ncclGetErrorString");
            }
        }
        rccl_all_reduce = g_rccl.all_reduce;
        rccl_err_str = g_rccl.err_str;
    }
    if (!rccl_all_reduce)
        return set_error(SCTC_ERR_STATE, "brnn_allreduce_grads: librccl.so (ncclAllReduce) could not be loaded");
    hipStream_t cs = (hipStream_t)compute_stream, ss = (hipStream_t)side_stream;
    constexpr int NCCL_SUM = 0, NCCL_FLOAT = 7, NCCL_DOUBLE = 8;
    auto reduce = [&](void* p, size_t n, int dt) -> int {
        const int rc = rccl_all_reduce(p, p, n, dt, NCCL_SUM, rccl_comm, ss);
        if (rc != 0)
            return set_error(SCTC_ERR_HIP, "ncclAllReduce failed: %s", rccl_err_str ? rccl_err_str(rc) : "?");
        return SCTC_OK;
    };
    hipEvent_t ev = nullptr;
    SCTC_HIP_TRY(hipEventCreateWithFlags(&ev, hipEventDisableTiming));
    int rc = SCTC_OK;
    auto after_compute = [&]() -> int {
        SCTC_HIP_TRY(hipEventRecord(ev, cs));
        SCTC_HIP_TRY(hipStreamWaitEvent(ss, ev, 0));
        return SCTC_OK;
    };
    if (!backward_queued) rc = after_compute();
    const int n = (int)h->tinfo.size();
    auto slice_end = [&](int i) -> int64_t { return i + 1 < n ? h->tinfo[i + 1].offset : h->param_elems; };
    for (int i = h->NL; i >= 0 && rc == SCTC_OK; --i) {
        const int w = weight_index(h, i);
        if (backward_queued) {
            const hipError_t e = hipStreamWaitEvent(ss, h->grad_ev[w], 0);
            if (e != hipSuccess) { rc = set_error(SCTC_ERR_HIP, "hipStreamWaitEvent: %s", hipGetErrorString(e)); break; }
        }
        rc = reduce(h->grads + h->tinfo[w].offset, (size_t)(slice_end(w + 1) - h->tinfo[w].offset), NCCL_FLOAT);
        if (rc == SCTC_OK && i == h->TL) {
            for (int k : {wf_index(h), wb_index(h)}) {
                if (backward_queued) {
                    const hipError_t e = hipStreamWaitEvent(ss, h->grad_ev[k], 0);
                    if (e != hipSuccess) { rc = set_error(SCTC_ERR_HIP, "hipStreamWaitEvent: %s", hipGetErrorString(e)); break; }
                }
                rc = reduce(h->grads + h->tinfo[k].offset, (size_t)(slice_end(k) - h->tinfo[k].offset), NCCL_FLOAT);
                if (rc != SCTC_OK) break;
            }
        }
    }
    if (rc == SCTC_OK && side_count > 0) {
        rc = after_compute();
        if (rc == SCTC_OK) rc = reduce(side_dev, (size_t)side_count, NCCL_DOUBLE);
    }
    if (rc == SCTC_OK) {
        hipError_t e = hipEventRecord(ev, ss);
        if (e == hipSuccess) e = hipStreamWaitEvent(cs, ev, 0);
        if (e != hipSuccess) rc = set_error(SCTC_ERR_HIP, "brnn_allreduce_grads: %s", hipGetErrorString(e));
    }
    (void)hipEventDestroy(ev);
    return rc;
}

int sctc_brnn_check(sctc_brnn_t h, void* stream)
{
    SCTC_CHECK_ARG(h, "brnn_check: null handle");
    return check_recurrent_error(h, (hipStream_t)stream);
}

static int cost_and_grad_once(sctc_brnn_t h, const sctc_minibatch* mb, int32_t flags,
                              double* cost_host, int32_t* skip_host, double* regcost_host,
                              void* stream)
{
    hipStream_t s = (hipStream_t)stream;
    bool all_skipped = false;
    SCTC_TRY(run_cost_and_grad(h, mb, flags, s, &all_skipped));
    int nw = 0;
    if (regcost_host && h->cfg.reg > 0.f) {
        for (size_t i = 0; i < h->tinfo.size(); ++i) {
            const sctc_tensor_info& t = h->tinfo[i];
            if (t.kind == 1) continue;
            const int64_t rows_p = round_up(t.rows, PAD);
            SCTC_TRY(launch_sumsq(h->params + t.offset, rows_p * t.ld, h->d_sumsq + nw,
                                  h->sumsq_ws, s));
            ++nw;
        }
    }
    if (cost_host)
        SCTC_HIP_TRY(hipMemcpyAsync(cost_host, h->d_cost_out, sizeof(double) * h->B,
                                    hipMemcpyDeviceToHost, s));
    if (skip_host)
        SCTC_HIP_TRY(hipMemcpyAsync(skip_host, h->d_skip_out, sizeof(int32_t) * h->B,
                                    hipMemcpyDeviceToHost, s));
    std::vector<double> ss(nw);
    if (nw)
        SCTC_HIP_TRY(hipMemcpyAsync(ss.data(), h->d_sumsq, sizeof(double) * nw,
                                    hipMemcpyDeviceToHost, s));
    SCTC_TRY(check_recurrent_error(h, s));
    if (regcost_host) {
        double rc = 0.0;
        for (double v : ss) rc += 0.5 * (double)h->cfg.reg * v;
        *regcost_host = rc;
    }
    return SCTC_OK;
}

int sctc_brnn_cost_and_grad(sctc_brnn_t h, const sctc_minibatch* mb, int32_t flags,
                            double* cost_host, int32_t* skip_host, double* regcost_host,
                            void* stream)
{
    SCTC_CHECK_ARG(h, "brnn_cost_and_grad: null handle");
    return with_retry(h, !(flags & SCTC_FLAG_ACCUMULATE), [&]() {
        return cost_and_grad_once(h, mb, flags, cost_host, skip_host, regcost_host, stream);
    });
}

static int forward_once(sctc_brnn_t h, const sctc_minibatch* mb, float* probs_dev, void* stream)
{
    hipStream_t s = (hipStream_t)stream;
    PhaseTimer pt{h, s};
    if (h->profiling) memset(h->phase_ms, 0, sizeof(h->phase_ms));
    h->tev_n = 0;
    SCTC_TRY(make_plan(h, mb, false, s));
    if (h->TL > 0) SCTC_TRY(recurrent_clear_error(h->counters, s));
    SCTC_TRY(run_forward(h, mb, s, pt));
    SCTC_TRY(launch_scatter_rows(probs_dev, h->A, h->probs, LD(h->Ap), h->d_src_row, h->N, h->A, s));
    pt.end();
    return check_recurrent_error(h, s);
}

int sctc_brnn_forward(sctc_brnn_t h, const sctc_minibatch* mb, float* probs_dev, void* stream)
{
    SCTC_CHECK_ARG(h && probs_dev, "brnn_forward: null argument");
    return with_retry(h, true, [&]() { return forward_once(h, mb, probs_dev, stream); });
}

int sctc_set_shared_device(int32_t on)
{
    recurrent_set_shared_device_mode(on);
    return SCTC_OK;
}

int sctc_shared_device(void) { return recurrent_shared_device_mode(); }

int sctc_device_pci_bus_id(int32_t device, char* out, int32_t out_len)
{
    SCTC_CHECK_ARG(out && out_len >= 16, "device_pci_bus_id: buffer of >= 16 bytes needed");
    int dev = device;
    if (dev < 0) SCTC_HIP_TRY(hipGetDevice(&dev));
    SCTC_HIP_TRY(hipDeviceGetPCIBusId(out, out_len, dev));
    return SCTC_OK;
}

int sctc_brnn_recurrent_path(sctc_brnn_t h, int32_t* forward_path, int32_t* bptt_path, int32_t* retries)
{
    SCTC_CHECK_ARG(h, "brnn_recurrent_path: null handle");
    if (forward_path) *forward_path = h->rec_path[0];
    if (bptt_path) *bptt_path = h->rec_path[1];
    if (retries) *retries = h->rec_retries;
    return SCTC_OK;
}

int sctc_brnn_debug_read(sctc_brnn_t h, uint32_t* out, int32_t n_words)
{
    SCTC_CHECK_ARG(h && out && n_words >= 0 && n_words <= 2 * REC_DEBUG_WORDS, "debug_read: bad argument");
    SCTC_HIP_TRY(hipMemcpy(out, h->rec_debug, sizeof(uint32_t) * n_words, hipMemcpyDeviceToHost));
    return SCTC_OK;
}

int sctc_brnn_debug_buffer(sctc_brnn_t h, int32_t which, void** dev_ptr, int64_t* rows, int64_t* cols,
                           int64_t* ld)
{
    SCTC_CHECK_ARG(h && dev_ptr && rows && cols && ld, "debug_buffer: null argument");
    SCTC_CHECK_ARG(!(h->cfg.operand_dtype == SCTC_F16 && ((which >= 1 && which <= h->NL) || which == 200)),
                   "debug_buffer: in the fp16-operand configuration the hidden layers' activations and the deltas "
                   "between them exist as 16-bit shadows only (buffer %d has no fp32 copy; 0, 100, 101 do)", which);
    const float* p = nullptr;
    int64_t c = h->Hp, l = LD(h->Hp);
    if (which >= 0 && which <= h->NL) {
        p = h->act[which];
        if (which == 0) { c = h->Dp; l = LD(h->Dp); }
    } else if (which == 100) p = h->hF;
    else if (which == 101) p = h->hB;
    else if (which == 102) p = h->Z;
    else if (which == 200) p = h->last_delta1;
    else if (which == 201) p = h->dF;
    else if (which == 202) p = h->dBk;
    SCTC_CHECK_ARG(p, "debug_buffer: no buffer %d (layers 0..%d, 100 hF, 101 hB, 102 z of the temporal layer, 200 delta_1, "
                   "201 / 202 the BPTT outputs deltasFor / deltasBack)", which, h->NL);
    *dev_ptr = (void*)p;
    *rows = h->N;
    *cols = c;
    *ld = l;
    return SCTC_OK;
}

int sctc_brnn_debug_buffer16(sctc_brnn_t h, int32_t which, void** dev_ptr, int64_t* rows, int64_t* cols,
                             int64_t* ld, int32_t* dtype)
{
    SCTC_CHECK_ARG(h && dev_ptr && rows && cols && ld && dtype, "debug_buffer16: null argument");
    SCTC_CHECK_ARG(h->cfg.operand_dtype == SCTC_F16, "debug_buffer16: only the fp16-operand configuration keeps 16-bit shadows");
    const uint16_t* p = nullptr;
    int64_t c = h->Hp, l = LD(h->Hp);
    int32_t dt = SCTC_BF16;
    if (which >= 0 && which <= h->NL) { p = h->act16f[which]; dt = SCTC_F16; }
    else if (which >= 50 && which <= 50 + h->NL) p = h->act16b[which - 50];
    else if (which == 100) p = h->hF16b;
    else if (which == 101) p = h->hB16b;
    else if (which == 200) p = h->last_delta1_16;
    else if (which == 201) p = h->dF16b;
    else if (which == 202) p = h->dBk16b;
    else if (which == 203 && h->NL >= 2 && h->last_delta1_16)
        p = h->last_delta1_16 == h->dA16 ? h->dBuf16 : h->dA16;
    if (which == 0 || which == 50) { c = h->Dp; l = LD(h->Dp); }
    SCTC_CHECK_ARG(p, "debug_buffer16: no buffer %d (0..%d float16 / 50..%d bfloat16 shadows of hActs[i]; bfloat16: 100 hF, 101 hB, "
                   "200 delta_1, 201 deltasFor, 202 deltasBack, 203 the delta the other ping-pong buffer was left with; the "
                   "bfloat16 ones exist in a training model after a cost_and_grad call)", which, h->NL, 50 + h->NL);
    *dev_ptr = (void*)p;
    *rows = h->N;
    *cols = c;
    *ld = l;
    *dtype = dt;
    return SCTC_OK;
}

int sctc_brnn_ctc_workspace_bytes(sctc_brnn_t h, const sctc_minibatch* mb, size_t* needed, size_t* reserved)
{
    SCTC_CHECK_ARG(h && mb && needed, "brnn_ctc_workspace_bytes: null argument");
    SCTC_CHECK_ARG(h->cfg.train, "brnn_ctc_workspace_bytes: the model was created with train = 0 (no CTC)");
    SCTC_CHECK_ARG(mb->B >= 1 && mb->B <= h->cfg.max_utts && mb->T_b && mb->U_b, "brnn_ctc_workspace_bytes: bad minibatch");
    SCTC_TRY(ctc_workspace_bytes(mb->B, h->A, 0, SCTC_F32, mb->T_b, mb->U_b, needed));
    if (reserved) *reserved = h->ctc_ws_ext ? h->ctc_ws_ext_bytes : h->ctc_ws_bytes;
    return SCTC_OK;
}

int sctc_brnn_set_ctc_workspace(sctc_brnn_t h, void* workspace_dev, size_t workspace_bytes)
{
    SCTC_CHECK_ARG(h, "null handle");
    SCTC_CHECK_ARG(h->cfg.train, "brnn_set_ctc_workspace: the model was created with train = 0 (no CTC)");
    SCTC_CHECK_ARG((workspace_dev == nullptr) == (workspace_bytes == 0), "brnn_set_ctc_workspace: a buffer and its size, or NULL and 0");
    SCTC_CHECK_ARG(((uintptr_t)workspace_dev & 255) == 0, "brnn_set_ctc_workspace: the buffer must be 256-byte aligned");
    h->ctc_ws_ext = workspace_dev;
    h->ctc_ws_ext_bytes = workspace_bytes;
    return SCTC_OK;
}

int sctc_brnn_mwer_workspace_bytes(sctc_brnn_t h, const sctc_minibatch* mb, const sctc_mwer_minibatch* mw, size_t* needed)
{
    SCTC_TRY(mwer_check_desc(mw, "brnn_mwer_workspace_bytes"));
    SCTC_CHECK_ARG(h && needed, "brnn_mwer_workspace_bytes: null argument");
    SCTC_CHECK_ARG(h->cfg.train, "brnn_mwer_workspace_bytes: the model was created with train = 0");
    MwerHost m;
    SCTC_TRY(mwer_prepare(h, mb, mw, "brnn_mwer_workspace_bytes", &m));
    *needed = m.plan.bytes;
    return SCTC_OK;
}

int sctc_brnn_set_mwer_workspace(sctc_brnn_t h, void* workspace_dev, size_t workspace_bytes)
{
    SCTC_CHECK_ARG(h, "null handle");
    SCTC_CHECK_ARG(h->cfg.train, "brnn_set_mwer_workspace: the model was created with train = 0");
    SCTC_CHECK_ARG((workspace_dev == nullptr) == (workspace_bytes == 0), "brnn_set_mwer_workspace: a buffer and its size, or NULL and 0");
    SCTC_CHECK_ARG(((uintptr_t)workspace_dev & 255) == 0, "brnn_set_mwer_workspace: the buffer must be 256-byte aligned");
    h->mwer_ws = workspace_dev;
    h->mwer_ws_bytes = workspace_bytes;
    return SCTC_OK;
}

int sctc_brnn_mwer_cost_and_grad_async(sctc_brnn_t h, const sctc_minibatch* mb, const sctc_mwer_minibatch* mw, int32_t flags,
                                       const sctc_mwer_outputs* out_dev, void* stream)
{
    return run_mwer_cost_and_grad(h, mb, mw, flags, out_dev, false, (hipStream_t)stream);
}

static int mwer_cost_and_grad_once(sctc_brnn_t h, const sctc_minibatch* mb, const sctc_mwer_minibatch* mw, int32_t flags,
                                   const sctc_mwer_outputs* out_host, double* regcost_host, void* stream)
{
    hipStream_t s = (hipStream_t)stream;
    SCTC_TRY(run_mwer_cost_and_grad(h, mb, mw, flags, out_host, true, s));
    int nw = 0;
    if (regcost_host && h->cfg.reg > 0.f) {
        for (size_t i = 0; i < h->tinfo.size(); ++i) {
            const sctc_tensor_info& t = h->tinfo[i];
            if (t.kind == 1) continue;
            SCTC_TRY(launch_sumsq(h->params + t.offset, round_up(t.rows, PAD) * t.ld, h->d_sumsq + nw, h->sumsq_ws, s));
            ++nw;
        }
    }
    std::vector<double> ss(nw);
    if (nw) SCTC_HIP_TRY(hipMemcpyAsync(ss.data(), h->d_sumsq, sizeof(double) * nw, hipMemcpyDeviceToHost, s));
    SCTC_HIP_TRY(hipStreamSynchronize(s));
    SCTC_TRY(check_recurrent_error(h, s));
    if (regcost_host) {
        double rc = 0.0;
        for (double v : ss) rc += 0.5 * (double)h->cfg.reg * v;
        *regcost_host = rc;
    }
    return SCTC_OK;
}

int sctc_brnn_mwer_cost_and_grad(sctc_brnn_t h, const sctc_minibatch* mb, const sctc_mwer_minibatch* mw, int32_t flags,
                                 const sctc_mwer_outputs* out_host, double* regcost_host, void* stream)
{
    SCTC_TRY(mwer_check_desc(mw, "brnn_mwer"));
    SCTC_CHECK_ARG(h, "brnn_mwer: null handle");
    return with_retry(h, !(flags & SCTC_FLAG_ACCUMULATE), [&]() {
        return mwer_cost_and_grad_once(h, mb, mw, flags, out_host, regcost_host, stream);
    });
}

int sctc_brnn_set_profiling(sctc_brnn_t h, int32_t enable)
{
    SCTC_CHECK_ARG(h, "null handle");
    if (enable && !h->ev_ready) {
        for (int i = 0; i <= SCTC_N_PHASES; ++i) {
            SCTC_HIP_TRY(hipEventCreate(&h->ev[i][0]));
            SCTC_HIP_TRY(hipEventCreate(&h->ev[i][1]));
        }
        h->ev_ready = true;
    }
    if (enable == 2 && h->tev.empty()) {
        h->tev.resize(128);
        for (hipEvent_t& e : h->tev) SCTC_HIP_TRY(hipEventCreate(&e));
    }
    h->profiling = enable == 2 ? 2 : (enable ? 1 : 0);
    h->tev_n = 0;
    return SCTC_OK;
}

int sctc_brnn_phase_ms(sctc_brnn_t h, float* ms_out)
{
    SCTC_CHECK_ARG(h && ms_out, "null argument");
    if (h->profiling == 2 && h->tev_n >= 2) {
        SCTC_HIP_TRY(hipEventSynchronize(h->tev[h->tev_n - 1]));
        memset(h->phase_ms, 0, sizeof(h->phase_ms));
        for (int i = 0; i + 1 < h->tev_n; ++i) {
            if (h->tev_phase[i] < 0) continue;
            float ms = 0.f;
            SCTC_HIP_TRY(hipEventElapsedTime(&ms, h->tev[i], h->tev[i + 1]));
            h->phase_ms[h->tev_phase[i]] += ms;
        }
    }
    memcpy(ms_out, h->phase_ms, sizeof(h->phase_ms));
    return SCTC_OK;
}

int sctc_brnn_flops(sctc_brnn_t h, const sctc_minibatch* mb, double* total, double* gemm,
                    double* recurrent)
{
    SCTC_CHECK_ARG(h && mb && mb->T_b, "null argument");
    double fg = 0.0, fr = 0.0;
    for (int b = 0; b < mb->B; ++b) {
        const double T = mb->T_b[b];
        for (int l = 0; l <= h->NL; ++l) {
            const double in = l == 0 ? h->D : h->H, out = l == h->NL ? h->A : h->H;
            fg += 2.0 * out * in * T;
            if (h->cfg.train) {
                fg += 2.0 * out * in * T;
                if (l > 0) fg += 2.0 * out * in * T;
            }
        }
        if (h->TL > 0) {
            const double HH = (double)h->H * h->H;
            fr += 2.0 * 2.0 * HH * (T - 1);
            if (h->cfg.train) {
                fr += 2.0 * 2.0 * HH * (T - 1);
                fg += 2.0 * 2.0 * HH * (T - 1);
            }
        }
    }
    if (total) *total = fg + fr;
    if (gemm) *gemm = fg;
    if (recurrent) *recurrent = fr;
    return SCTC_OK;
}

}
```

### stanford-ctc_amd/csrc/recurrent.h

```cpp
#pragma once
#include <hip/hip_runtime.h>
#include <stdint.h>

#include "recurrent_plan.h"

namespace sctc {

struct RecArgs {
    const float* W[2];
    int64_t ldw;
    int32_t transpose;
    int32_t descending[2];
    const float* pre[2];
    const float* act[2];
    float* out[2];
    int64_t ld;
    int32_t Hp;
    int32_t B;
    int32_t Tmax;
    const int32_t* rowbase;
    const int32_t* T_b;
    float max_act;
    float* xbuf;
    const int32_t* xbase;
    int32_t n_xrows;
    unsigned* counters;
    int32_t sync_mode;
    int32_t poll_delay;
    int32_t variant;
    unsigned* debug;
    int32_t b_off;
    const int32_t* T_host;
    int32_t linear_map;
    int32_t prec16;
};
static constexpr int REC_DEBUG_ALL_OFF = 2 * 16 * 8;
static constexpr int REC_DEBUG_WORDS = 2 * 16 * 8 + 512 * 8;
#ifndef SCTC_REC_FLAG_STRIDE
#define SCTC_REC_FLAG_STRIDE 8
#endif
static constexpr int REC_FLAG_STRIDE = SCTC_REC_FLAG_STRIDE;
static constexpr int REC_COUNTER_WORDS = 32 + 4 * 128 * REC_FLAG_STRIDE;

static inline int recurrent_step_xrows(int alive) { return alive >= 17 ? (alive + 15) & ~15 : (alive + 3) & ~3; }
static inline int64_t recurrent_xrows_bound(int64_t rows, int64_t tmax) { return rows + 3 * tmax + 12 * (rows / 17 + 1); }
size_t recurrent_xbuf_floats(int Hp, int64_t max_xrows);
int recurrent_supported(int Hp, int B, char* why, int why_len);
static constexpr int REC_PATH_NONE = 0;
static constexpr int REC_PATH_PERSISTENT = 1;
static constexpr int REC_PATH_PERSISTENT_LEASED = 2;
static constexpr int REC_PATH_FALLBACK = 3;
int launch_recurrent(const RecArgs& a, hipStream_t stream, int* path = nullptr);
int recurrent_clear_error(unsigned* counters, hipStream_t stream);
int recurrent_shared_device_mode();
void recurrent_set_shared_device_mode(int on);

}
```

### stanford-ctc_amd/csrc/recurrent.hip

```cpp
#include <algorithm>
#include <map>
#include <mutex>
#include <string>
#include <type_traits>
#include <utility>

#include "common.h"
#include "device_share.h"
#include "recurrent.h"
#include "xlane.h"

namespace sctc {

typedef void (*RecKernel)(RecArgs);
static constexpr int REC_THREADS = 256;
typedef float f32x4 __attribute__((ext_vector_type(4)));
typedef unsigned int u32x4 __attribute__((ext_vector_type(4)));
typedef unsigned int u32x2 __attribute__((ext_vector_type(2)));

static constexpr unsigned long long SPIN_TIMEOUT_TICKS = 50000000ull;

__device__ __forceinline__ void first_poll_delay(int units)
{
    for (int i = 0; i < units; ++i) __builtin_amdgcn_s_sleep(1);
// ... 356 lines not shown
    const int base = nch >> 2, rem = nch & 3;
    const int cnt = base + (wave < rem ? 1 : 0);
    const int c_beg = wave * base + min(wave, rem);
    float4* Wl = lds4 + (size_t)wave * NLDS * 64;
    float4* red = lds4 + (size_t)4 * NLDS * 64;

    auto load_w = [&](int c) {
        const float* W = p.W[g];
        float4 v;
        if (!p.transpose) {
            v = *reinterpret_cast<const float4*>(W + (int64_t)(row0 + uj) * p.ldw + 16 * c + 4 * kq);
        } else {
            const float* col = W + (int64_t)(16 * c + 4 * kq) * p.ldw + row0 + uj;
            v.x = col[0];
            v.y = col[p.ldw];
            v.z = col[2 * p.ldw];
            v.w = col[3 * p.ldw];
        }
        return v;
    };
    float4 wreg[NREG > 0 ? NREG : 1];
#pragma unroll
    for (int u = 0; u < NREG; ++u) wreg[u] = load_w(c_beg + min(u, cnt - 1));
#pragma unroll 4
    for (int u = NREG; u < NCQ; ++u) Wl[(u - NREG) * 64 + lane] = load_w(c_beg + min(u, cnt - 1));
    __syncthreads();

    const bool desc = p.descending[g] != 0;
    const float* pre = p.pre[g];
    const float* act = p.act[g];
    float* out = p.out[g];
    const int64_t ld = p.ld;
    const float hi = p.max_act > 0.f ? p.max_act : INFINITY;
    unsigned* flags = p.counters + 32 + chain * 128 * REC_FLAG_STRIDE;
    unsigned* err = p.counters + 2;
    const unsigned chunk_stride = (unsigned)p.n_xrows * 64u;
    float* xg = p.xbuf + (size_t)g * p.n_xrows * Hp;
    const __amdgpu_buffer_rsrc_t xrsrc = __builtin_amdgcn_make_buffer_rsrc(
        xg, 0, (int)((size_t)p.n_xrows * Hp * sizeof(float)), 0x00020000);

    const int ub = tile * 16 + uj;
    const int uT = ub < p.B ? p.T_b[ub] : 0;
    const int Tchain = tile * 16 < p.B ? p.T_b[tile * 16] : 0;
    const int tile_T = lane_order_steps(uT, tile, p.b_off, p.variant);

    const int dbg_sel = (p.debug && chain == 0 && tid == 0) ? (wg == 0 ? 0 : (wg == nwg - 1 ? 1 : -1)) : -1;
    auto stamp = [&](int j, int k) {
        if (dbg_sel >= 0 && j >= 64 && j < 80)
            p.debug[(dbg_sel * 16 + (j - 64)) * 8 + k] = (unsigned)clock64();
        if (p.debug && tid == 0 && j == 70) {
            p.debug[REC_DEBUG_ALL_OFF + blockIdx.x * 8 + k] = (unsigned)wall_clock64();
            if (k == 0) p.debug[REC_DEBUG_ALL_OFF + blockIdx.x * 8 + 7] = 1u + (unsigned)chain;
#ifdef SCTC_REC_WHERE
            if (k == 0)
                p.debug[REC_DEBUG_ALL_OFF + blockIdx.x * 8 + 6] =
                    ((__builtin_amdgcn_s_getreg(20 | (0 << 6) | ((4 - 1) << 11)) & 0xf) << 16) |
                    ((__builtin_amdgcn_s_getreg(4 | (0 << 6) | ((32 - 1) << 11)) >> 8) & 0xff);
#endif
        }
    };

    if ((p.variant == REC_V_Q_PRIO_DIR && g == 0) || (p.variant == REC_V_Q_PRIO_TILE && tile == 0) || (p.variant == REC_V_Q_PRIO_PARITY && ((g ^ tile) & 1) == 0))
        __builtin_amdgcn_s_setprio(3);
    int rb_next = uT > 0 ? p.rowbase[desc ? uT - 1 : 0] : 0;
    int xb_next = p.xbase[0], xb_cur = 0;
    for (int j = 0; j < Tchain; ++j) {
        stamp(j, 0);
        f32x4 acc[4];
#pragma unroll
        for (int q = 0; q < 4; ++q) acc[q] = {0.f, 0.f, 0.f, 0.f};
        const bool active = j < uT;
        const int xb_prev = xb_cur;
        const int rb = rb_next;
        xb_cur = xb_next;
        {
            const int jn = min(j + 1, Tchain - 1);
            const int tn = desc ? uT - 1 - jn : jn;
            rb_next = p.rowbase[min(max(tn, 0), p.Tmax - 1)];
            xb_next = p.xbase[jn];
        }
        const int64_t orow = active ? (int64_t)rb + p.b_off + ub : 0;
        const unsigned xrow = active ? (unsigned)xb_cur + (unsigned)ub : 0u;
        const unsigned prow = (active && j > 0) ? (unsigned)xb_prev + (unsigned)ub : 0u;
        unsigned xin = prow * 64u + (unsigned)kq * 16u;
        unsigned xout = xrow * 64u + (unsigned)kq * 16u;
        if (j > 0 && j <= tile_T && active) xin = ((unsigned)xb_prev + (unsigned)tile * 16u) * 64u + (unsigned)lane * 16u;
        if (j < tile_T) xout = ((unsigned)xb_cur + (unsigned)tile * 16u) * 64u + (unsigned)lane * 16u;
        float4 pre4 = make_float4(0.f, 0.f, 0.f, 0.f), act4 = pre4;
        if (wave == 0 && active) {
            pre4 = *reinterpret_cast<const float4*>(pre + orow * ld + row0 + 4 * kq);
            if (act) act4 = *reinterpret_cast<const float4*>(act + orow * ld + row0 + 4 * kq);
        }

        if (j > 0) {
            wait_all(flags, nwg, (unsigned)j, err, p.poll_delay);
            stamp(j, 1);
            float4 x[NCQ];
#pragma unroll
            for (int u = 0; u < NCQ; ++u) {
                x[u] = ld_x(xrsrc, xin, (unsigned)(c_beg + min(u, cnt - 1)) * chunk_stride);
                __builtin_amdgcn_sched_barrier(0);
                __builtin_amdgcn_s_sleep(1);
                __builtin_amdgcn_sched_barrier(0);
            }
            __builtin_amdgcn_sched_barrier(0);
#pragma unroll
            for (int u = 0; u < NCQ; ++u) {
                if (u < NCQ - 1 || cnt == NCQ) {
                    const float4 a = u < NREG ? wreg[u < NREG ? u : 0] : Wl[(u - NREG) * 64 + lane];
                    SCTC_MFMA4(acc, a, x[u])
                }
            }
            if (p.debug) {
                asm volatile("" : "+v"(acc[0]), "+v"(acc[1]), "+v"(acc[2]), "+v"(acc[3]));
                stamp(j, 2);
            }
            if (wave != 0) {
                const f32x4 s = (acc[0] + acc[1]) + (acc[2] + acc[3]);
                red[(wave - 1) * 64 + lane] = make_float4(s[0], s[1], s[2], s[3]);
            }
            __syncthreads();
            stamp(j, 3);
        }

        if (wave == 0 && active) {
            float4 s = make_float4(0.f, 0.f, 0.f, 0.f);
            if (j > 0) {
                const float4 r1 = red[lane], r2 = red[64 + lane], r3 = red[128 + lane];
                const f32x4 q = (acc[0] + acc[1]) + (acc[2] + acc[3]);
                s = make_float4((q[0] + r1.x) + (r2.x + r3.x), (q[1] + r1.y) + (r2.y + r3.y),
                                (q[2] + r1.z) + (r2.z + r3.z), (q[3] + r1.w) + (r2.w + r3.w));
            }
            const float4 o = step_result(pre4, s, act4, act != nullptr, hi);
            *reinterpret_cast<float4*>(out + orow * ld + row0 + 4 * kq) = o;
            st_x(xrsrc, xout, (unsigned)wg * chunk_stride, o, sync_mode);
        }
        stamp(j, 4);
        if (j + 1 < Tchain) publish_step(flags + wg * REC_FLAG_STRIDE, (unsigned)(j + 1), sync_mode);
        stamp(j, 5);
    }
}

template <int... I, class F>
__device__ __forceinline__ void static_for_seq(std::integer_sequence<int, I...>, F&& f)
{
    (f(std::integral_constant<int, I>()), ...);
}
template <int N, class F>
__device__ __forceinline__ void static_for(F&& f)
{
    static_for_seq(std::make_integer_sequence<int, N>(), static_cast<F&&>(f));
}

template <int NCQ, int NREGF, int NT, int NBAT, int R, int PUB, int PB, int UG = 2>
__global__ __launch_bounds__(256, 1) void brnn_recurrent_t_kernel(RecArgs p)
{
    extern __shared__ __attribute__((aligned(16))) float4 lds4[];
    constexpr int NFR = UG * NCQ;
    constexpr int NLDSF = NFR - NREGF;
    constexpr int XB = (NCQ + NBAT - 1) / NBAT;
    constexpr int NC = UG * NT;
    constexpr int NPL = UG == 1 ? 2 : 1;
    static_assert(UG == 1 || UG == 2, "16 or 32 units per block");
    static_assert(NC <= 4 && NPL * NC <= 4, "one result per wave, one 16-byte flag load per lane");
    static_assert(NBAT % R == 0 && NBAT >= 2 * R && R >= 2, "ring");
    static_assert((NBAT - 1) * XB < NCQ, "no empty batch");
    static_assert(PUB >= 0 && PUB + 2 <= PB && PB <= NBAT - R + 1 && PB >= 1,
                  "the flag is published (behind batch PUB) before the next phase's flags are polled (in front of batch PB - 1) and "
                  "seen (in front of batch PB), and that before the next phase's first exchange loads (batch NBAT - R + 1)");
    const int tid = threadIdx.x, lane = tid & 63;
    const int wave = __builtin_amdgcn_readfirstlane(tid >> 6);
    const int Hp = p.Hp, nch = Hp >> 4, nprod = nch / UG;
    const int combo = blockIdx.x & (2 * UG - 1), ublk = blockIdx.x / (2 * UG);
    const int g = combo & 1, half = combo >> 1;
    const int row0 = ublk * 16 * UG;
    const int uj = lane & 15, kq = lane >> 4;
    const int sync_mode = p.sync_mode;
    const int base = nch >> 2, rem = nch & 3;
    const int cnt = base + (wave < rem ? 1 : 0);
    const int c_beg = wave * base + min(wave, rem);
    float4* Wl = lds4 + (size_t)wave * NLDSF * 64;
    float4* red = lds4 + (size_t)4 * NLDSF * 64;

    auto load_w = [&](int c, int ug) {
        const float* W = p.W[g];
        const int r = row0 + 16 * ug + uj;
        float4 v;
        if (!p.transpose) {
            v = *reinterpret_cast<const float4*>(W + (int64_t)r * p.ldw + 16 * c + 4 * kq);
        } else {
            const float* col = W + (int64_t)(16 * c + 4 * kq) * p.ldw + r;
            v.x = col[0];
            v.y = col[p.ldw];
            v.z = col[2 * p.ldw];
            v.w = col[3 * p.ldw];
        }
        return v;
    };
    float4 wreg[NREGF > 0 ? NREGF : 1];
    auto load_w0 = [&](int f) {
        const float4 w = load_w(c_beg + min(f / UG, cnt - 1), f % UG);
        return (f / UG) < cnt ? w : make_float4(0.f, 0.f, 0.f, 0.f);
    };
#pragma unroll
    for (int f = 0; f < NREGF; ++f) {
        const float4 w = load_w0(f);
        asm("v_accvgpr_write_b32 %0, %1" : "=a"(wreg[f].x) : "v"(w.x));
        asm("v_accvgpr_write_b32 %0, %1" : "=a"(wreg[f].y) : "v"(w.y));
        asm("v_accvgpr_write_b32 %0, %1" : "=a"(wreg[f].z) : "v"(w.z));
        asm("v_accvgpr_write_b32 %0, %1" : "=a"(wreg[f].w) : "v"(w.w));
    }
#pragma unroll 4
    for (int f = NREGF; f < NFR; ++f) Wl[(f - NREGF) * 64 + lane] = load_w0(f);
    __syncthreads();

    const bool desc = p.descending[g] != 0;
    const float* pre = p.pre[g];
    const float* act = p.act[g];
    const float* act_or_pre = act ? act : pre;
    float* out = p.out[g];
    const int64_t ld = p.ld;
    const float hi = p.max_act > 0.f ? p.max_act : INFINITY;
    unsigned* err = p.counters + 2;
    const unsigned chunk_stride = (unsigned)p.n_xrows * 64u;
    float* xg = p.xbuf + (size_t)g * p.n_xrows * Hp;
    const __amdgpu_buffer_rsrc_t xrsrc = __builtin_amdgcn_make_buffer_rsrc(
        xg, 0, (int)((size_t)p.n_xrows * Hp * sizeof(float)), 0x00020000);

    struct Sub {
        int ub[NT], uT[NT], tile_T[NT];
        unsigned trow[NT];
        int T;
        unsigned* flags;
        int rb_next[NT];
        unsigned xb_next, xb_cur;
    };
    auto init_sub = [&](Sub& S, int sub) {
#pragma unroll
        for (int i = 0; i < NT; ++i) {
            const int tile = (i * 2 + sub) * UG + half;
            S.trow[i] = (unsigned)tile * 16u;
            S.ub[i] = tile * 16 + uj;
            S.uT[i] = S.ub[i] < p.B ? p.T_b[S.ub[i]] : 0;
            S.tile_T[i] = lane_order_steps(S.uT[i], tile, p.b_off, p.variant);
            S.rb_next[i] = S.uT[i] > 0 ? p.rowbase[desc ? S.uT[i] - 1 : 0] : 0;
        }
        S.T = __builtin_amdgcn_readfirstlane((int)S.trow[0] < p.B ? p.T_b[S.trow[0]] : 0);
        S.flags = p.counters + 32 + (size_t)((combo * 2 + sub) * 64) * REC_FLAG_STRIDE;
        S.xb_next = (unsigned)p.xbase[0];
        S.xb_cur = 0;
    };
    int vzero;
    asm volatile("v_mov_b32 %0, 0" : "=v"(vzero));
    Sub A, Bc;
    init_sub(A, 0);
    init_sub(Bc, 1);

    const int dbg_sel = (p.debug && combo == 0 && tid == 0) ? (ublk == 0 ? 0 : (ublk == nprod - 1 ? 1 : -1)) : -1;
    unsigned* dbg_lds = reinterpret_cast<unsigned*>(red + (size_t)2 * NC * 3 * 64);
#if defined(SCTC_T_STAMPS) || defined(SCTC_T_STAMP_CHUNKS)
    auto stamp = [&](int sub, int j, int k) {
        if (dbg_sel >= 0 && j >= 64 && j < 72)
            dbg_lds[((j - 64) * 2 + sub) * 8 + k] = (unsigned)wall_clock64();
    };
#else
    auto stamp = [&](int, int, int) {};
    (void)dbg_lds;
#endif
#ifdef SCTC_T_STAMP_CHUNKS
    unsigned* dbg_fine = dbg_lds + 16 * 8;
    auto stamp_chunk = [&](int sub, int j, int c) {
        if (dbg_sel >= 0 && j >= 64 && j < 68 && c < 32)
            dbg_fine[((j - 64) * 2 + sub) * 32 + c] = (unsigned)wall_clock64();
    };
#else
    auto stamp_chunk = [&](int, int, int) {};
#endif

    float4 x[R][XB][NT];

    auto xin_of = [&](const Sub& S, int j, unsigned xb_prev, unsigned (&xin)[NT]) {
#pragma unroll
        for (int i = 0; i < NT; ++i) {
            const bool active = j < S.uT[i];
            const unsigned prow = (active && j > 0) ? xb_prev + (unsigned)S.ub[i] : 0u;
            xin[i] = prow * 64u + (unsigned)kq * 16u;
            if (j > 0 && j <= S.tile_T[i] && active)
                xin[i] = (xb_prev + S.trow[i]) * 64u + (unsigned)lane * 16u;
            if (p.variant == REC_V_T_STALE) xin[i] = (unsigned)lane * 16u;
        }
    };
    auto issue_part = [&](const unsigned (&xin)[NT], auto bi_c, auto lo_c, auto hi_c) {
        constexpr int bi = decltype(bi_c)::value, lo = decltype(lo_c)::value, hi_ = decltype(hi_c)::value;
#pragma unroll
        for (int u = lo; u < hi_; ++u) {
            const int cu = bi * XB + u;
            if (cu < NCQ) {
#pragma unroll
                for (int i = 0; i < NT; ++i)
                    x[bi % R][u][i] = ld_x(xrsrc, xin[i], (unsigned)(c_beg + min(cu, cnt - 1)) * chunk_stride);
            }
        }
    };
    auto issue_batch = [&](const unsigned (&xin)[NT], auto bi_c) {
        issue_part(xin, bi_c, std::integral_constant<int, 0>(), std::integral_constant<int, XB>());
    };
    const __amdgpu_buffer_rsrc_t frsrc = __builtin_amdgcn_make_buffer_rsrc(
        p.counters, 0, (int)(REC_COUNTER_WORDS * sizeof(unsigned)), 0x00020000);
    const unsigned flane = (unsigned)min(lane, nprod - 1) * (REC_FLAG_STRIDE * 4u);
    auto flags_off = [&](const unsigned* fl) -> unsigned { return (unsigned)((fl - p.counters) * 4); };
    auto poll_issue = [&](unsigned fl_off) -> u32x4 {
        return __builtin_amdgcn_raw_buffer_load_b128(frsrc, flane, fl_off, 16 );
    };
    auto poll_min = [&](const u32x4& v) -> unsigned {
        unsigned f = v[0];
#pragma unroll
        for (int c = 1; c < NC; ++c) f = min(f, v[c]);
        if constexpr (NPL == 2) {
            const bool second = lane + 64 < nprod;
#pragma unroll
            for (int c = 0; c < NC; ++c) f = second ? min(f, v[NC + c]) : f;
        }
        return f;
    };
    auto wait_flags = [&](unsigned fl_off, unsigned f, unsigned target) {
        if (__all(f >= target)) return;
        const unsigned long long t0 = wall_clock64();
        unsigned spins = 0;
        for (;;) {
            __builtin_amdgcn_s_sleep(1);
            asm volatile("" ::: "memory");
            f = poll_min(poll_issue(fl_off));
            if (__all(f >= target)) break;
            if ((++spins & 255u) == 0) {
                if (spin_expired(err, t0, lane)) break;
            }
        }
    };
    auto prologue = [&](const Sub& S, int j) {
        first_poll_delay(p.poll_delay);
        wait_flags(flags_off(S.flags), poll_min(poll_issue(flags_off(S.flags))), (unsigned)j);
        unsigned xin[NT];
        xin_of(S, j, S.xb_cur, xin);
        static_for<R - 1>([&](auto b) { issue_batch(xin, b); });
    };

    struct Epi {
        bool pending, zero;
        bool lane_active;
        int parity;
        f32x4 mine;
        float4 pre4, act4, r0, r1, r2, s, o;
        int64_t out_off;
        unsigned xo, xchunk;
        unsigned* flag;
        unsigned val;
    };
    Epi E;
    E.pending = false;
    auto epi_barrier = [&](const Epi& e) {
        if (e.pending && !e.zero) {
            asm volatile("s_waitcnt lgkmcnt(0)" ::: "memory");
            __builtin_amdgcn_s_barrier();
            asm volatile("" ::: "memory");
        }
    };
    auto epi_read = [&](Epi& e) {
        if (e.pending && !e.zero && wave < NC) {
            const float4* r = red + (size_t)((e.parity * NC + wave) * 3) * 64 + lane;
            e.r0 = r[0];
            e.r1 = r[64];
            e.r2 = r[128];
        }
    };
    auto epi_sum = [&](Epi& e) {
        e.s = make_float4(0.f, 0.f, 0.f, 0.f);
        if (e.pending && wave < NC && !e.zero) {
            const float4 m = make_float4(e.mine[0], e.mine[1], e.mine[2], e.mine[3]);
            float4 p0 = m, p1 = e.r0, p2 = e.r1, p3 = e.r2;
            if (wave == 1) { p0 = e.r0; p1 = m; }
            if (wave == 2) { p0 = e.r0; p1 = e.r1; p2 = m; }
            if (wave == 3) { p0 = e.r0; p1 = e.r1; p2 = e.r2; p3 = m; }
            e.s = make_float4((p0.x + p1.x) + (p2.x + p3.x), (p0.y + p1.y) + (p2.y + p3.y),
                              (p0.z + p1.z) + (p2.z + p3.z), (p0.w + p1.w) + (p2.w + p3.w));
        }
    };
    auto epi_result = [&](Epi& e) {
        if (e.pending && wave < NC) e.o = step_result(e.pre4, e.s, e.act4, act != nullptr, hi);
    };
    auto epi_stores = [&](const Epi& e) {
        if (e.pending && wave < NC && e.lane_active) {
            *reinterpret_cast<float4*>(out + e.out_off) = e.o;
            st_x(xrsrc, e.xo, e.xchunk, e.o, sync_mode);
// ... 529 lines not shown
                                    const int item = c * 64 + lane;
                                    if (item < n16)
                                        *reinterpret_cast<u32x4*>(xs + (size_t)(wave + 4 * r) * xld + 8 * item) = v[r][c];
                                }
                                need[r] = false;
                            } else {
                                pending = true;
                            }
                        }
                    }
                    if (!pending) break;
                    if ((++spins & 255u) == 0) {
                        if (spin_expired(err, t0, lane)) break;
                    }
                }
            }
            __syncthreads();
            const unsigned short* xrow = xs + (size_t)uj * xld + 8 * kq;
#pragma unroll
            for (int u = 0; u < NCH; ++u) {
                if (u < NCH - 1 || cnt == NCH) {
                    const V8 x = *reinterpret_cast<const V8*>(xrow + 32 * (c_beg + u));
                    acc[u & 1] = R::mfma(wf[u], x, acc[u & 1]);
                }
            }
            if (wave != 0) {
                const f32x4 sres = acc[0] + acc[1];
                red[(wave - 1) * 64 + lane] = make_float4(sres[0], sres[1], sres[2], sres[3]);
            }
            __syncthreads();
        }
        if (wave == 0 && active) {
            float4 sv = make_float4(0.f, 0.f, 0.f, 0.f);
            if (j > 0) {
                const float4 r1 = red[lane], r2 = red[64 + lane], r3 = red[128 + lane];
                const f32x4 q = acc[0] + acc[1];
                sv = make_float4((q[0] + r1.x) + (r2.x + r3.x), (q[1] + r1.y) + (r2.y + r3.y),
                                 (q[2] + r1.z) + (r2.z + r3.z), (q[3] + r1.w) + (r2.w + r3.w));
            }
            const float4 o = step_result(pre4, sv, act4, act != nullptr, hi);
            *reinterpret_cast<float4*>(out + orow * ld + row0 + 4 * kq) = o;
            const u32x2 ou = {(unsigned)R::bits(o.x) | ((unsigned)R::bits(o.y) << 16),
                              (unsigned)R::bits(o.z) | ((unsigned)R::bits(o.w) << 16)};
            __builtin_amdgcn_raw_buffer_store_b64(ou, xrsrc, (unsigned)(row0 + 4 * kq) * 2u,
                                                  (unsigned)(xb_cur + uj) * (unsigned)Hp * 2u, 16 );
        }
        __syncthreads();
    }
}

__global__ __launch_bounds__(256) void brnn_recurrent_step_kernel(RecArgs p, int j)
{
    __shared__ float4 red[3 * 64];
    const int tid = threadIdx.x, lane = tid & 63;
    const int wave = __builtin_amdgcn_readfirstlane(tid >> 6);
    const int wg = blockIdx.x, g = blockIdx.y, tile = blockIdx.z;
    const int Ttile = tile * 16 < p.B ? p.T_b[tile * 16] : 0;
    if (j >= Ttile) return;
    const int nch = p.Hp >> 4;
    const int row0 = wg * 16;
    const int uj = lane & 15, kq = lane >> 4;
    const int base = nch >> 2, rem = nch & 3;
    const int cnt = base + (wave < rem ? 1 : 0);
    const int c_beg = wave * base + min(wave, rem);
    const bool desc = p.descending[g] != 0;
    const float* W = p.W[g];
    const float* pre = p.pre[g];
    const float* act = p.act[g];
    float* out = p.out[g];
    const int64_t ld = p.ld;
    const float hi = p.max_act > 0.f ? p.max_act : INFINITY;
    const int ub = tile * 16 + uj;
    const int uT = ub < p.B ? p.T_b[ub] : 0;
    const bool active = j < uT;
    const int t = desc ? uT - 1 - j : j;
    const int tp = desc ? t + 1 : t - 1;
    const int64_t orow = active ? (int64_t)p.rowbase[t] + p.b_off + ub : 0;
    const int64_t prow = (active && j > 0) ? (int64_t)p.rowbase[tp] + p.b_off + ub : 0;
    float4 pre4 = make_float4(0.f, 0.f, 0.f, 0.f), act4 = pre4;
    if (wave == 0 && active) {
        pre4 = *reinterpret_cast<const float4*>(pre + orow * ld + row0 + 4 * kq);
        if (act) act4 = *reinterpret_cast<const float4*>(act + orow * ld + row0 + 4 * kq);
    }
    f32x4 acc[4];
#pragma unroll
    for (int q = 0; q < 4; ++q) acc[q] = {0.f, 0.f, 0.f, 0.f};
    if (j > 0) {
        const float* xr = out + prow * ld + 4 * kq;
        for (int u = 0; u < cnt; ++u) {
            const int c = c_beg + u;
            float4 a;
            if (!p.transpose) {
                a = *reinterpret_cast<const float4*>(W + (int64_t)(row0 + uj) * p.ldw + 16 * c + 4 * kq);
            } else {
                const float* col = W + (int64_t)(16 * c + 4 * kq) * p.ldw + row0 + uj;
                a.x = col[0];
                a.y = col[p.ldw];
                a.z = col[2 * p.ldw];
                a.w = col[3 * p.ldw];
            }
            const float4 x = *reinterpret_cast<const float4*>(xr + 16 * c);
            SCTC_MFMA4(acc, a, x)
        }
        if (wave != 0) {
            const f32x4 s = (acc[0] + acc[1]) + (acc[2] + acc[3]);
            red[(wave - 1) * 64 + lane] = make_float4(s[0], s[1], s[2], s[3]);
        }
        __syncthreads();
    }
    if (wave == 0 && active) {
        float4 s = make_float4(0.f, 0.f, 0.f, 0.f);
        if (j > 0) {
            const float4 r1 = red[lane], r2 = red[64 + lane], r3 = red[128 + lane];
            const f32x4 q = (acc[0] + acc[1]) + (acc[2] + acc[3]);
            s = make_float4((q[0] + r1.x) + (r2.x + r3.x), (q[1] + r1.y) + (r2.y + r3.y),
                            (q[2] + r1.z) + (r2.z + r3.z), (q[3] + r1.w) + (r2.w + r3.w));
        }
        const float4 o = step_result(pre4, s, act4, act != nullptr, hi);
        *reinterpret_cast<float4*>(out + orow * ld + row0 + 4 * kq) = o;
    }
}

size_t recurrent_xbuf_floats(int Hp, int64_t max_xrows)
{
    return (size_t)2 * (size_t)max_xrows * Hp;
}

int recurrent_supported(int Hp, int B, char* why, int why_len)
{
    if (Hp % 32 != 0) { snprintf(why, why_len, "layer size %d not padded to 32", Hp); return 0; }
    (void)B;
    return 1;
}

#define SCTC_REC_KERNELS_OF_SIZE(X, NCQ, NREG, NK, NCH)                                                         \
    X(REC_FAM_Q, brnn_recurrent_q_kernel, NCQ, NREG)                                                            \
    X(REC_FAM_S, brnn_recurrent_s_kernel, NK, 4) X(REC_FAM_S, brnn_recurrent_s_kernel, NK, 8)                   \
    X(REC_FAM_MH, brnn_recurrent_mh_kernel, NCH, false) X(REC_FAM_MH, brnn_recurrent_mh_kernel, NCH, true)      \
    X(REC_FAM_SLAB, brnn_recurrent_kernel, 1, NK, false) X(REC_FAM_SLAB, brnn_recurrent_kernel, 2, NK, false)   \
    X(REC_FAM_SLAB, brnn_recurrent_kernel, 4, NK, false) X(REC_FAM_SLAB, brnn_recurrent_kernel, 4, NK, true)
#define SCTC_REC_T(X, ...) X(REC_FAM_T, brnn_recurrent_t_kernel, __VA_ARGS__)
#define SCTC_REC_KERNELS(X)                                                                                     \
    SCTC_REC_KERNELS_OF_SIZE(X, 8, 0, 16, 4) SCTC_REC_KERNELS_OF_SIZE(X, 16, 0, 32, 8)       \
    SCTC_REC_KERNELS_OF_SIZE(X, 29, 10, 57, 15) SCTC_REC_KERNELS_OF_SIZE(X, 32, 13, 64, 16)  \
    X(REC_FAM_SLAB, brnn_recurrent_kernel, 1, 0, false) X(REC_FAM_SLAB, brnn_recurrent_kernel, 2, 0, false)     \
    X(REC_FAM_SLAB, brnn_recurrent_kernel, 4, 0, false)                                     \
    SCTC_REC_T(X, 29, 29, 1, 8, 4, 1, 5, 1) SCTC_REC_T(X, 29, 29, 1, 6, 3, 1, 4, 1) SCTC_REC_T(X, 29, 0, 1, 8, 4, 1, 5, 1) \
    SCTC_REC_T(X, 32, 32, 1, 8, 4, 1, 5, 1) SCTC_REC_T(X, 32, 32, 1, 6, 3, 1, 4, 1) SCTC_REC_T(X, 32, 0, 1, 8, 4, 1, 5, 1) \
    SCTC_REC_T(X, 8, 0, 1, 4, 2, 0, 3, 2) SCTC_REC_T(X, 8, 0, 2, 4, 2, 0, 3, 2)                                 \
    SCTC_REC_T(X, 16, 0, 1, 4, 2, 1, 3, 2) SCTC_REC_T(X, 16, 0, 2, 4, 2, 1, 3, 2)                               \
    SCTC_REC_T(X, 29, 25, 1, 8, 4, 1, 5, 2) SCTC_REC_T(X, 29, 25, 1, 6, 3, 1, 4, 2) SCTC_REC_T(X, 29, 25, 1, 8, 2, 1, 7, 2) \
    SCTC_REC_T(X, 29, 25, 2, 6, 3, 1, 4, 2) SCTC_REC_T(X, 29, 25, 2, 8, 4, 1, 5, 2) SCTC_REC_T(X, 29, 25, 2, 8, 2, 1, 7, 2) \
    SCTC_REC_T(X, 32, 31, 1, 8, 4, 1, 5, 2) SCTC_REC_T(X, 32, 31, 1, 6, 3, 1, 4, 2)                             \
    SCTC_REC_T(X, 32, 31, 2, 8, 4, 1, 5, 2) SCTC_REC_T(X, 32, 31, 2, 6, 3, 1, 4, 2)

static RecKernel rec_kernel(const RecCandidate& c)
{
#define SCTC_REC_MATCH(FAMILY, KERNEL, ...)                                                                     \
    {                                                                                                           \
        static constexpr int t[] = {__VA_ARGS__};                                                               \
        constexpr int n = sizeof(t) / sizeof(t[0]);                                                             \
        if (c.family == FAMILY && c.ntarg == n && std::equal(t, t + n, c.targ)) return KERNEL<__VA_ARGS__>;     \
    }
    SCTC_REC_KERNELS(SCTC_REC_MATCH)
#undef SCTC_REC_MATCH
    return nullptr;
}


int recurrent_shared_device_mode() { return device_share().mode.get(); }
void recurrent_set_shared_device_mode(int on) { device_share().mode.set(on); }

static const std::string& device_share_key(int dev)
{
    static std::mutex mu;
    static std::map<int, std::string> keys;
    std::lock_guard<std::mutex> lock(mu);
    auto it = keys.find(dev);
    if (it == keys.end()) {
        char bus[64] = "";
        (void)hipDeviceGetPCIBusId(bus, sizeof(bus), dev);
        it = keys.emplace(dev, share_key(bus)).first;
    }
    return it->second;
}

struct HipEvents {
    typedef hipEvent_t Event;
    typedef hipStream_t Stream;
    bool done(hipEvent_t ev)
    {
        const hipError_t q = hipEventQuery(ev);
        if (q != hipSuccess && q != hipErrorNotReady) (void)hipGetLastError();
        return q == hipSuccess;
    }
    int wait(hipEvent_t ev) { SCTC_HIP_TRY(hipEventSynchronize(ev)); return SCTC_OK; }
    int create(hipEvent_t* ev) { SCTC_HIP_TRY(hipEventCreateWithFlags(ev, hipEventDisableTiming)); return SCTC_OK; }
    int record(hipEvent_t ev, hipStream_t stream) { SCTC_HIP_TRY(hipEventRecord(ev, stream)); return SCTC_OK; }
};
static PersistentGate<HipEvents> g_gate;

static int prepare_kernel(RecKernel k, size_t smem, int max_per_cu, int dev, int* blocks_per_cu)
{
    struct Info { size_t smem_set = 0; size_t occ_smem = (size_t)-1; int occ = 0; };
    static std::mutex mu;
    static std::map<std::pair<int, const void*>, Info> table;
    std::lock_guard<std::mutex> lock(mu);
    Info& in = table[std::make_pair(dev, reinterpret_cast<const void*>(k))];
    if (in.smem_set < smem) {
        SCTC_HIP_TRY(hipFuncSetAttribute(reinterpret_cast<const void*>(k),
                                         hipFuncAttributeMaxDynamicSharedMemorySize, (int)smem));
        in.smem_set = smem;
    }
    if (in.occ_smem != smem) {
        int n = 0, lds = 0;
        SCTC_HIP_TRY(hipOccupancyMaxActiveBlocksPerMultiprocessor(&n, reinterpret_cast<const void*>(k), REC_THREADS, smem));
        SCTC_HIP_TRY(hipDeviceGetAttribute(&lds, hipDeviceAttributeMaxSharedMemoryPerMultiprocessor, dev));
        const int by_lds = smem ? (int)std::min<size_t>((size_t)max_per_cu, (size_t)lds / smem) : max_per_cu;
        in.occ = std::max(std::min(n, max_per_cu), by_lds);
        in.occ_smem = smem;
        if (getenv("SCTC_VERBOSE"))
            fprintf(stderr, "sctc: recurrent kernel %p on device %d: %zu B LDS, occupancy query %d, LDS model %d blocks/CU\n",
                    reinterpret_cast<const void*>(k), dev, smem, n, by_lds);
    }
    *blocks_per_cu = in.occ;
    return SCTC_OK;
}

static int launch_fallback(const RecArgs& a, hipStream_t stream)
{
    const int nch = a.Hp / 16, ntiles = (a.B + 15) / 16;
    for (int j = 0; j < a.Tmax; ++j)
        hipLaunchKernelGGL(brnn_recurrent_step_kernel, dim3(nch, 2, ntiles), dim3(256), 0, stream, a, j);
    SCTC_HIP_TRY(hipGetLastError());
    return SCTC_OK;
}

struct LaunchCtx {
    int dev, cus;
    hipStream_t stream;
    int* path;
    int tcfg;
};

static int read_error_word(const RecArgs& a, hipStream_t stream, unsigned* e)
{
    *e = 0;
    SCTC_HIP_TRY(hipMemcpyAsync(e, a.counters + 2, sizeof(unsigned), hipMemcpyDeviceToHost, stream));
    SCTC_HIP_TRY(hipStreamSynchronize(stream));
    return SCTC_OK;
}

static int launch_persistent(RecKernel k, int grid, size_t smem, int max_per_cu, size_t sentinel_bytes,
                             const RecArgs& a, const LaunchCtx& cx, bool* done)
{
    *done = false;
    int per_cu = 0;
    SCTC_TRY(prepare_kernel(k, smem, max_per_cu, cx.dev, &per_cu));
    if (per_cu < 1 || (int64_t)per_cu * cx.cus < grid) return SCTC_OK;
    const int need_cus = (grid + per_cu - 1) / per_cu;
    if (sentinel_bytes)
        SCTC_HIP_TRY(hipMemsetAsync(a.xbuf, 0xFF, sentinel_bytes, cx.stream));
    DeviceShare& share = device_share();
    const std::string& key = device_share_key(cx.dev);
    if (share.shared_for_launch(key)) {
        SCTC_HIP_TRY(hipStreamSynchronize(cx.stream));
        LeaseGuard lease(share.lease, key);
        if (!lease.locked) return SCTC_OK;
        hipLaunchKernelGGL(k, dim3(grid), dim3(REC_THREADS), smem, cx.stream, a);
        SCTC_HIP_TRY(hipGetLastError());
        unsigned e = 0;
        SCTC_TRY(read_error_word(a, cx.stream, &e));
        *done = true;
        if (cx.path) *cx.path = REC_PATH_PERSISTENT_LEASED;
        if (e != 0)
            return set_error(SCTC_ERR_TIMEOUT, "recurrent kernel: a persistent launch under the device lease gave "
                             "up waiting for its peers (%d workgroups not co-resident)", grid);
        return SCTC_OK;
    }
    SCTC_TRY(g_gate.admit_and_launch(cx.dev, cx.stream, need_cus, cx.cus, [&]() -> int {
        hipLaunchKernelGGL(k, dim3(grid), dim3(REC_THREADS), smem, cx.stream, a);
        SCTC_HIP_TRY(hipGetLastError());
        return SCTC_OK;
    }));
    *done = true;
    if (cx.path) *cx.path = REC_PATH_PERSISTENT;
    return SCTC_OK;
}

static int launch_recurrent_one(const RecArgs& a, const LaunchCtx& cx)
{
    SCTC_HIP_TRY(hipMemsetAsync(a.counters + 32, 0, (REC_COUNTER_WORDS - 32) * sizeof(unsigned), cx.stream));
    RecCandidate plan[REC_MAX_CANDIDATES];
    const RecShape shape = {a.Hp, a.B, a.prec16, a.transpose, a.variant, cx.tcfg, cx.cus};
    const int n = rec_plan(shape, plan);
    for (int i = 0; i + 1 < n; ++i) {
        const RecCandidate& c = plan[i];
        const RecKernel k = rec_kernel(c);
        if (!k) {
            char name[96];
            rec_candidate_name(c, name, sizeof(name));
            return set_error(SCTC_ERR_ARG, "recurrent kernel: the plan names %s, which the library does not have", name);
        }
        RecArgs b = a;
        b.linear_map = c.linear_map;
        b.variant = c.variant;
        bool done = false;
        SCTC_TRY(launch_persistent(k, c.grid, c.lds, c.per_cu, (size_t)2 * a.n_xrows * a.Hp * c.fill, b, cx, &done));
        if (done) return SCTC_OK;
    }
    if (cx.path) *cx.path = REC_PATH_FALLBACK;
    return launch_fallback(a, cx.stream);
}

int recurrent_clear_error(unsigned* counters, hipStream_t stream)
{
    SCTC_HIP_TRY(hipMemsetAsync(counters, 0, 32 * sizeof(unsigned), stream));
    return SCTC_OK;
}

int launch_recurrent(const RecArgs& a_in, hipStream_t stream, int* path)
{
    RecArgs a = a_in;
    if (a.poll_delay < 0) a.poll_delay = a.Hp > 1024 ? 5 : 0;
    char why[128];
    if (!recurrent_supported(a.Hp, a.B, why, sizeof(why)))
        return set_error(SCTC_ERR_ARG, "recurrent kernel: %s", why);
    if (!rec_variant_known(a.variant))
        return set_error(SCTC_ERR_ARG, "recurrent kernel: SCTC_REC_VARIANT=%d is not a variant (RecVariant, csrc/recurrent_plan.h)", a.variant);
    if (a.Tmax <= 0 || a.B <= 0) return SCTC_OK;
    if ((size_t)a.n_xrows * a.Hp * sizeof(float) >= ((size_t)1 << 31))
        return set_error(SCTC_ERR_ARG, "recurrent kernel: %d exchange rows x %d units exceed the "
                         "2 GiB buffer addressing", a.n_xrows, a.Hp);
    LaunchCtx cx;
    cx.stream = stream;
    cx.path = path;
    cx.dev = 0;
    cx.cus = 0;
    static const int tcfg = getenv("SCTC_REC_TCFG") ? atoi(getenv("SCTC_REC_TCFG")) : 0;
    cx.tcfg = tcfg;
    SCTC_HIP_TRY(hipGetDevice(&cx.dev));
    SCTC_HIP_TRY(hipDeviceGetAttribute(&cx.cus, hipDeviceAttributeMultiprocessorCount, cx.dev));
    for (int b0 = 0; b0 < a_in.B;) {
        const RecShape rest = {a.Hp, a_in.B - b0, a.prec16, a.transpose, a.variant, cx.tcfg, cx.cus};
        const int nb = rec_cut(rest);
        RecArgs c = a;
        c.b_off = a_in.b_off + b0;
        c.T_b = a_in.T_b + b0;
        c.B = nb;
        if (a_in.T_host) c.Tmax = std::min(a_in.Tmax, (int)a_in.T_host[b0]);
        if (c.variant == REC_V_NO_CUT) c.variant = REC_V_AUTO;
        SCTC_TRY(launch_recurrent_one(c, cx));
        b0 += nb;
    }
    return SCTC_OK;
}

}
```

### stanford-ctc_amd/csrc/recurrent_plan.h

```cpp
#pragma once
#include <stdint.h>
#include <stdio.h>
#include <algorithm>
#include <initializer_list>

namespace sctc {

enum RecVariant : int32_t {
    REC_V_AUTO = 0,
    REC_V_SLAB = 1,
    REC_V_FALLBACK = 3,
    REC_V_S_TO_8 = 43,
    REC_V_Q_FROM_1 = 44,
    REC_V_NO_CUT = 45,
    REC_V_SLAB_LARGE = 47,
    REC_V_T_SMALL = 50,
    REC_V_Q_AT_32 = 51,
    REC_V_NO_PIPE = 40,
    REC_V_ROW_MAJOR = 46,
    REC_V_Q_LINEAR = 2,
    REC_V_Q_PRIO_DIR = 5, REC_V_Q_PRIO_TILE = 6, REC_V_Q_PRIO_PARITY = 7,
    REC_V_T_STALE = 49,
};

static inline bool rec_variant_known(int v)
{
    for (int known : {REC_V_AUTO, REC_V_SLAB, REC_V_FALLBACK, REC_V_S_TO_8, REC_V_Q_FROM_1, REC_V_NO_CUT, REC_V_SLAB_LARGE,
                      REC_V_T_SMALL, REC_V_Q_AT_32, REC_V_NO_PIPE, REC_V_ROW_MAJOR, REC_V_Q_LINEAR, REC_V_Q_PRIO_DIR,
                      REC_V_Q_PRIO_TILE, REC_V_Q_PRIO_PARITY, REC_V_T_STALE})
        if (v == known) return true;
    return false;
}

struct RecShape {
    int Hp, B;
    int prec16, transpose;
    int variant;
    int tcfg, cus;
};

enum RecFamily {
    REC_FAM_Q,
    REC_FAM_S,
    REC_FAM_MH,
    REC_FAM_T,
    REC_FAM_SLAB,
    REC_FAM_FALLBACK,
};

struct RecCandidate {
    RecFamily family;
    int ntarg, targ[8];
    int grid;
    size_t lds;
    int per_cu;
    int fill;
    int linear_map;
    int variant;
};
static constexpr int REC_MAX_CANDIDATES = 5;

struct RecTForm { int nregf, nbat, r, pub, pb; };
constexpr RecTForm rec_t84(int nregf) { return {nregf, 8, 4, 1, 5}; }
constexpr RecTForm rec_t63(int nregf) { return {nregf, 6, 3, 1, 4}; }
constexpr RecTForm rec_t82(int nregf) { return {nregf, 8, 2, 1, 7}; }
constexpr RecTForm rec_t42(int pub) { return {0, 4, 2, pub, 3}; }

struct RecSize {
    int Hp;
    int ncq, nreg;
    int nk;
    int nch;
    bool t_default;
    RecTForm t_ug1[4];
    RecTForm t_one[4];
    RecTForm t_two[4];
};
static constexpr RecSize REC_SIZES[] = {
    {512, 8, 0, 16, 4, false, {}, {rec_t42(0), rec_t42(0), rec_t42(0), rec_t42(0)}, {rec_t42(0), rec_t42(0), rec_t42(0), rec_t42(0)}},
    {1024, 16, 0, 32, 8, false, {}, {rec_t42(1), rec_t42(1), rec_t42(1), rec_t42(1)}, {rec_t42(1), rec_t42(1), rec_t42(1), rec_t42(1)}},
    {1824, 29, 10, 57, 15, true, {rec_t84(29), rec_t63(29), rec_t84(29), rec_t84(0)},
     {rec_t84(25), rec_t63(25), rec_t82(25), rec_t84(25)}, {rec_t63(25), rec_t84(25), rec_t82(25), rec_t63(25)}},
    {2048, 32, 13, 64, 16, true, {rec_t84(32), rec_t63(32), rec_t84(32), rec_t84(0)},
     {rec_t84(31), rec_t63(31), rec_t84(31), rec_t84(31)}, {rec_t84(31), rec_t63(31), rec_t84(31), rec_t84(31)}},
};
static inline const RecSize* rec_size(int Hp)
{
    for (const RecSize& r : REC_SIZES) if (r.Hp == Hp) return &r;
    return nullptr;
}

static constexpr size_t REC_LDS_MAX = 160 * 1024, REC_F4 = 16;
static inline size_t rec_lds_q(const RecSize& r) { return REC_F4 * ((size_t)4 * (r.ncq - r.nreg) * 64 + 3 * 64); }
static inline size_t rec_lds_s(int Hp, int sb) { return sizeof(float) * 2 * sb * Hp; }
static inline size_t rec_lds_mh(int Hp) { return (((size_t)16 * (Hp + 8) * 2 + 15) / 16) * 16 + 3 * 64 * REC_F4; }
static inline size_t rec_lds_t(const RecSize& r, const RecTForm& f, int nt, int ug) { return REC_F4 * 64 * ((size_t)4 * (ug * r.ncq - f.nregf) + 2 * 3 * (ug * nt)) + (16 * 8 + 8 * 32) * sizeof(unsigned); }
static inline size_t rec_lds_slab(int Hp, int ntw) { return REC_F4 * ((size_t)(Hp / 16) * 64 + 2 * ntw * 64); }

static inline bool rec_tiled_large(const RecShape& s)
{
    const RecSize* r = rec_size(s.Hp);
    return r && s.variant != REC_V_SLAB && s.variant != REC_V_NO_PIPE && s.variant != REC_V_SLAB_LARGE &&
           4 * (s.Hp / 32) <= s.cus && (r->t_default || s.variant == REC_V_T_SMALL);
}

static inline RecCandidate rec_candidate(const RecShape& s, RecFamily family, std::initializer_list<int> targ, int grid,
                                         size_t lds, int per_cu, int fill)
{
    RecCandidate c = {family, (int)targ.size(), {}, grid, lds, per_cu, fill, 0, s.variant};
    std::copy(targ.begin(), targ.end(), c.targ);
    return c;
}
static inline RecCandidate rec_candidate_t(const RecShape& s, const RecSize& r, const RecTForm& f, int nt, int ug, size_t lds_min)
{
    return rec_candidate(s, REC_FAM_T, {r.ncq, f.nregf, nt, f.nbat, f.r, f.pub, f.pb, ug}, 2 * ug * (s.Hp / (16 * ug)),
                         std::max(rec_lds_t(r, f, nt, ug), lds_min), 1, 0);
}

static inline int rec_plan(const RecShape& s, RecCandidate out[REC_MAX_CANDIDATES])
{
    if (!rec_variant_known(s.variant)) return -1;
    const int nwg = s.Hp / 16, ntiles = (s.B + 15) / 16, v = s.variant, B = s.B, sb = B <= 4 ? 4 : 8;
    const RecSize* r = rec_size(s.Hp);
    const int tcfg = s.tcfg >= 0 && s.tcfg <= 3 ? s.tcfg : 0;
    const bool persistent = v != REC_V_FALLBACK && 2 * nwg <= s.cus;
    int n = 0;
    if (persistent && r && (!s.prec16 || B <= 5) && (B >= 4 || v == REC_V_Q_FROM_1) && B <= 16 && v != REC_V_SLAB && v != REC_V_S_TO_8) {
        RecCandidate c = rec_candidate(s, REC_FAM_Q, {r->ncq, r->nreg}, 2 * nwg, rec_lds_q(*r), 2, 0);
        c.linear_map = 1;
        if (v == REC_V_Q_FROM_1) c.variant = REC_V_AUTO;
        out[n++] = c;
    }
    if (persistent && r && (B <= 5 || (B <= 8 && v == REC_V_S_TO_8)) && v != REC_V_SLAB)
        out[n++] = rec_candidate(s, REC_FAM_S, {r->nk, sb}, 2 * nwg, rec_lds_s(s.Hp, sb), 2, 4);
    if (persistent && r && s.prec16 && B > 5 && B <= 16 && v != REC_V_SLAB && rec_lds_mh(s.Hp) <= REC_LDS_MAX)
        out[n++] = rec_candidate(s, REC_FAM_MH, {r->nch, s.transpose != 0}, 2 * nwg, rec_lds_mh(s.Hp), 1, 2);
    if (persistent && r && r->t_ug1[tcfg].nbat && ntiles == 2 && !s.prec16 && (v == REC_V_AUTO || v == REC_V_ROW_MAJOR || v == REC_V_T_STALE))
        out[n++] = rec_candidate_t(s, *r, r->t_ug1[tcfg], 1, 1, (size_t)81 * 1024);
    if (persistent && r && ntiles == 2 && v != REC_V_SLAB && 4 * nwg <= 2 * s.cus)
        out[n++] = rec_candidate(s, REC_FAM_Q, {r->ncq, r->nreg}, 4 * nwg, rec_lds_q(*r), 2, 0);
    if (persistent && ntiles > 2 && rec_tiled_large(s))
        out[n++] = ntiles <= 4 ? rec_candidate_t(s, *r, r->t_one[tcfg], 1, 2, 0) : rec_candidate_t(s, *r, r->t_two[tcfg], 2, 2, 0);
    const int ntw = ntiles <= 2 ? 1 : (ntiles <= 4 ? 2 : 4);
    if (persistent && rec_lds_slab(s.Hp, ntw) <= REC_LDS_MAX)
        out[n++] = rec_candidate(s, REC_FAM_SLAB, {ntw, r ? r->nk : 0, ntw == 4 && r && v != REC_V_NO_PIPE}, 2 * nwg,
                                 rec_lds_slab(s.Hp, ntw), 1, 0);
    out[n++] = rec_candidate(s, REC_FAM_FALLBACK, {}, 0, 0, 0, 0);
    return n;
}

static inline int rec_cut(const RecShape& s)
{
    const int nb = s.B < 128 ? s.B : 128;
    const bool cuts = (s.variant == REC_V_AUTO || s.variant == REC_V_T_SMALL) && !s.prec16;
    if (cuts && rec_tiled_large(s)) return nb > 64 && nb <= 96 ? 64 : nb;
    if (cuts && s.variant == REC_V_AUTO) return nb > 32 && nb <= 48 ? 32 : (nb > 64 && nb <= 80 ? 64 : nb);
    return nb;
}

static inline void rec_candidate_name(const RecCandidate& c, char* buf, size_t len)
{
    static const char* const NAMES[] = {"brnn_recurrent_q_kernel", "brnn_recurrent_s_kernel", "brnn_recurrent_mh_kernel",
                                        "brnn_recurrent_t_kernel", "brnn_recurrent_kernel", "brnn_recurrent_step_kernel"};
    size_t at = snprintf(buf, len, "%s", NAMES[c.family]);
    for (int i = 0; i < c.ntarg && at < len; ++i) {
        const bool flag = (c.family == REC_FAM_MH && i == 1) || (c.family == REC_FAM_SLAB && i == 2);
        if (flag) at += snprintf(buf + at, len - at, "%s%s", i ? ", " : "<", c.targ[i] ? "true" : "false");
        else at += snprintf(buf + at, len - at, "%s%d", i ? ", " : "<", c.targ[i]);
    }
    if (c.ntarg && at < len) snprintf(buf + at, len - at, ">");
}

}
```

### stanford-ctc_amd/nnets/brnnet.py

```python
import ctypes
import pickle

import os

import numpy as np

import _sctc
import cudamat as cm


class TensorStack(list):
    flat = None


class NNet:

    def __init__(self, inputDim, outputDim, layerSize, numLayers, maxBatch,
                 train=True, temporalLayer=-1, reg=0.0, maxUtts=1, fp16=False, gemm=None):
        cm.cublas_init()
        self.outputDim = outputDim
        self.inputDim = inputDim
        self.layerSize = layerSize
        self.numLayers = numLayers
        self.layerSizes = [layerSize] * numLayers
# ... 300 lines not shown
        del keep
        if self.reg > 0:
            self.regcost = regcost.value
        res = (loss, self.grad, inactive.astype(bool))
        if return_stats:
            res += (dict(expected=expected, posterior=post, real=real.astype(bool), ctc_cost=ctc_cost,
                         ctc_skip=ctc_skip.astype(bool)),)
        return res

    def mwerCostAndGradBatchAsync(self, data_list, hyps_list, errors_list, labels_list=None, scale=1.0,
                                  subtract_mean=True, ctc_weight=0.0, accumulate=False, feats_dev=None, T_b=None,
                                  reg_in_grad=True):
        torch = _sctc.require_gpu()
        mb, mw, flags, B, K, keep = self._mwer_setup(data_list, hyps_list, errors_list, labels_list, scale, subtract_mean,
                                                     ctc_weight, accumulate, feats_dev, T_b, reg_in_grad, None, None)
        f64 = lambda *shape: torch.empty(shape, dtype=torch.float64, device="cuda")
        i32 = lambda *shape: torch.empty(shape, dtype=torch.int32, device="cuda")
        res = dict(loss=f64(B), expected=f64(B), inactive=i32(B), ctc_cost=f64(B), ctc_skip=i32(B), posterior=f64(B, K),
                   real=i32(B, K))
        out = _sctc.MwerOutputs(*[res[k].data_ptr() for k in ("loss", "expected", "inactive", "ctc_cost", "ctc_skip",
                                                               "posterior", "real")])
        rc = _sctc.lib().sctc_brnn_mwer_cost_and_grad_async(self._h, ctypes.byref(mb), ctypes.byref(mw), flags,
                                                            ctypes.byref(out), _sctc.current_stream_ptr())
        _sctc.check(rc, "mwerCostAndGrad")
        self._async_keep = keep
        return res

    def nbestBatch(self, data_list, refs_list, nbest, beam=40, unit="word", space=None, lm=None, alpha=1.0, beta=0.0):
        import ctc_fast
        if unit not in ("char", "word"):
            raise ValueError("nbestBatch: unit must be 'char' or 'word', not %r" % (unit,))
        K = int(nbest)
        if not 1 <= K <= _sctc.MWER_MAX_K:
            raise ValueError("nbestBatch: nbest = %d outside 1..%d" % (K, _sctc.MWER_MAX_K))
        if unit == "word" and (space is None or not 1 <= int(space) < self.outputDim):
            raise ValueError("nbestBatch: the word unit needs the space symbol, in [1, %d)" % self.outputDim)
        B = len(data_list)
        if len(refs_list) != B:
            raise ValueError("nbestBatch: %d references for %d utterances" % (len(refs_list), B))
        refs = [np.ascontiguousarray(np.asarray(r).reshape(-1), dtype=np.int32) for r in refs_list]
        lp, T_b = self.forwardDevice(data_list, log=True)
        rows, scores = ctc_fast.decode_beam_batch(lp, [int(t) for t in T_b], beam=beam, alpha=alpha, beta=beta, lm=lm,
                                                  nbest=K)
        if K == 1:
            rows, scores = [[r] for r in rows], np.asarray(scores).reshape(B, 1)
        hyps = [[np.asarray(rows[b][k], dtype=np.int32) for k in range(K) if scores[b, k] != float("-inf")]
                for b in range(B)]
        flat = [h for row in hyps for h in row]
        owner = [b for b, row in enumerate(hyps) for _ in row]
        errors = [np.zeros(len(row), dtype=np.float64) for row in hyps]
        if flat:
            if unit == "char":
                dist = ctc_fast.edit_distance_batch(refs, flat, a_index=owner)[:, 0]
            else:
                dist = ctc_fast.word_errors_batch([refs[b] for b in owner], flat, int(space), A=self.outputDim)[:, 0]
            at = 0
            for b, row in enumerate(hyps):
                errors[b][:] = dist[at:at + len(row)]
                at += len(row)
        return hyps, errors


    def _lanes_for(self, n_streams):
        torch = _sctc.require_gpu()
        lanes = getattr(self, "_lanes", None)
        if lanes is not None and len(lanes) == 2 * n_streams:
            return lanes
        L = _sctc.lib()
        for ln in lanes or []:
            L.sctc_brnn_destroy(ln["h"])
        self._lanes = None
        cfg = _sctc.BrnnConfig(self.inputDim, self.outputDim, self.layerSize, self.numLayers,
                               self.temporalLayer, int(self.maxBatch), 1,
                               float(self.maxAct) if self.maxAct else 0.0, float(self.reg), 1,
                               self._cfg.operand_dtype)
        sizes = _sctc.BrnnSizes()
        _sctc.check(L.sctc_brnn_query(ctypes.byref(cfg), ctypes.byref(sizes)), "NNet lanes")
        lanes = []
        streams = [torch.cuda.Stream() for _ in range(n_streams)]
        for k in range(2 * n_streams):
            grads = self._grads if k == 0 else torch.zeros_like(self._grads)
            ws = torch.empty(sizes.workspace_bytes, dtype=torch.uint8, device="cuda")
            h = ctypes.c_void_p()
            _sctc.check(L.sctc_brnn_create(ctypes.byref(cfg), self._params.data_ptr(), grads.data_ptr(),
                                           ws.data_ptr(), sizes.workspace_bytes, ctypes.byref(h)), "NNet lanes")
            lanes.append({"h": h, "grads": grads, "ws": ws, "stream": streams[k % n_streams], "cfg": cfg})
        self._lanes = lanes
        return lanes

    def costAndGradStreams(self, data_list, labels_list, n_streams=2, feats_dev=None, T_b=None,
                           reg_in_grad=True):
        torch = _sctc.require_gpu()
        if self._h is None:
            raise RuntimeError("initParams() / fromFile() first")
        if not self.train:
            raise RuntimeError("costAndGradStreams needs a train=True model")
        if feats_dev is None:
            T_b = [np.asarray(d).shape[1] for d in data_list]
            feats_dev = self._stage(data_list)
        for T in T_b:
            self.setViews(T)
        B = len(T_b)
        L = _sctc.lib()
        lanes = self._lanes_for(max(1, min(int(n_streams), B)))
        cur = torch.cuda.current_stream()
        cost_dev = torch.zeros(B, dtype=torch.float64, device="cuda")
        skip_dev = torch.zeros(B, dtype=torch.int32, device="cuda")
        keep = []
        used = [False] * len(lanes)
        for ln in lanes[:len(lanes) // 2]:
            ln["stream"].wait_stream(cur)
        off = 0
        for i in range(B):
            k = i % len(lanes)
            ln = lanes[k]
            mb, kp = self._minibatch(feats_dev[off:off + T_b[i]], [T_b[i]], [labels_list[i]])
            keep.append((mb, kp))
            off += T_b[i]
            if len(labels_list[i]) > 1023 and ln["h"] is not self._h:
                self._grow_ctc_workspace(mb, h=ln["h"])
            flags = (_sctc.FLAG_ACCUMULATE if used[k] else 0) | \
                    (0 if (reg_in_grad and i == 0) else _sctc.FLAG_NO_REG_GRAD)
            if used[k]:
                _sctc.check(L.sctc_brnn_check(ln["h"], ctypes.c_void_p(ln["stream"].cuda_stream)), "costAndGrad")
            used[k] = True
            rc = L.sctc_brnn_cost_and_grad_async(ln["h"], ctypes.byref(mb), flags,
                                                 cost_dev.data_ptr() + 8 * i, skip_dev.data_ptr() + 4 * i,
                                                 ctypes.c_void_p(ln["stream"].cuda_stream))
            _sctc.check(rc, "costAndGrad")
        for k, ln in enumerate(lanes):
            cur.wait_stream(ln["stream"])
            if not used[k]:
                continue
            _sctc.check(L.sctc_brnn_check(ln["h"], ctypes.c_void_p(ln["stream"].cuda_stream)), "costAndGrad")
            if k > 0:
                _sctc.check(L.sctc_axpy(self._grads.data_ptr(), ln["grads"].data_ptr(), 1.0,
                                        self._grads.numel(), _sctc.current_stream_ptr()), "costAndGrad")
        if self.reg > 0:
            self.regcost = float(self.regCostDev().item())
        cost = cost_dev.cpu().numpy()
        skip = skip_dev.cpu().numpy().astype(bool)
        del keep
        return cost, self.grad, skip

    def checkAsync(self):
        _sctc.check(_sctc.lib().sctc_brnn_check(self._h, _sctc.current_stream_ptr()), "costAndGrad")

    def recurrentPath(self):
        f, b, r = ctypes.c_int32(0), ctypes.c_int32(0), ctypes.c_int32(0)
        _sctc.check(_sctc.lib().sctc_brnn_recurrent_path(self._h, ctypes.byref(f), ctypes.byref(b),
                                                         ctypes.byref(r)), "recurrentPath")
        return f.value, b.value, r.value

    def debugBuffer(self, which):
        torch = _sctc.require_gpu()
        ptr, rows, cols, ld = ctypes.c_void_p(), ctypes.c_int64(), ctypes.c_int64(), ctypes.c_int64()
        _sctc.check(_sctc.lib().sctc_brnn_debug_buffer(self._h, which, ctypes.byref(ptr), ctypes.byref(rows),
                                                       ctypes.byref(cols), ctypes.byref(ld)), "debugBuffer")
        torch.cuda.synchronize()
        off = (ptr.value - self._ws.data_ptr()) // 4
        flat = self._ws.view(torch.float32)[off:off + rows.value * ld.value]
        return flat.view(rows.value, ld.value)[:, :cols.value].cpu().numpy().astype(np.float64)

    def debugBuffer16(self, which):
        torch = _sctc.require_gpu()
        ptr, rows, cols, ld = ctypes.c_void_p(), ctypes.c_int64(), ctypes.c_int64(), ctypes.c_int64()
        dt = ctypes.c_int32()
        _sctc.check(_sctc.lib().sctc_brnn_debug_buffer16(self._h, which, ctypes.byref(ptr), ctypes.byref(rows), ctypes.byref(cols),
                                                         ctypes.byref(ld), ctypes.byref(dt)), "debugBuffer16")
        torch.cuda.synchronize()
        off = (ptr.value - self._ws.data_ptr()) // 2
        flat = self._ws.view(torch.int16)[off:off + rows.value * ld.value]
        bits = flat.view(rows.value, ld.value)[:, :cols.value].contiguous().cpu().numpy().view(np.uint16)
        return bits, {_sctc.F16: "float16", _sctc.BF16: "bfloat16"}[dt.value]

    def gradBuckets(self):
        L = _sctc.lib()
        NL = self.numLayers
        offs = [int(ti.offset) for ti in self._infos] + [int(self._grads.numel())]
        out = []
        for i in range(NL, -1, -1):
            out.append((L.sctc_brnn_grad_event(self._h, 2 * i), offs[2 * i], offs[2 * i + 2]))
            if i == self.temporalLayer:
                for k in (2 * (NL + 1), 2 * (NL + 1) + 1):
                    out.append((L.sctc_brnn_grad_event(self._h, k), offs[k], offs[k + 1]))
        return out

    def regCostDev(self):
        torch = _sctc.require_gpu()
        L = _sctc.lib()
        if not hasattr(self, "_reg_ws"):
            self._reg_ws = torch.empty(8192, dtype=torch.uint8, device="cuda")
        mats = [ti for ti in self._infos if ti.kind != 1]
        out = torch.zeros(len(mats), dtype=torch.float64, device="cuda")
        for j, ti in enumerate(mats):
            rows_p, ld = cm.padded_layout(ti.rows, ti.cols)
            _sctc.check(L.sctc_sumsq(self._params.data_ptr() + 4 * int(ti.offset), rows_p * ld,
                                     out.data_ptr() + 8 * j, self._reg_ws.data_ptr(),
                                     self._reg_ws.numel(), _sctc.current_stream_ptr()), "regcost")
        return 0.5 * float(self.reg) * out.sum()

    def costAndGrad(self, data, labels=None, sentence=None):
        T = data.shape[1]
        self.setViews(T)
        if not self.train:
            return self.forwardProbs([data])[0]
        cost, grad, skip = self.costAndGradBatch([data], [labels], sync_skip=True)
        c = float(cost[0])
        if self.reg > 0:
            c = c + self.regcost
        return c, self.grad, bool(skip[0])

    def forwardDevice(self, data_list, log=False, out=None):
        torch = _sctc.require_gpu()
        if self._h is None:
            raise RuntimeError("initParams() / fromFile() first")
        T_b = [np.asarray(d).shape[1] for d in data_list]
        feats = self._stage(data_list)
        mb, keep = self._minibatch(feats, T_b, None)
        rows = int(sum(T_b))
        if out is None:
            out = torch.empty((rows, self.outputDim), dtype=torch.float32, device="cuda")
        elif not (out.is_cuda and out.dtype == torch.float32 and out.is_contiguous()
                  and tuple(out.shape) == (rows, self.outputDim)):
            raise ValueError("forwardDevice: out must be a contiguous float32 [%d][%d] device tensor"
                             % (rows, self.outputDim))
        rc = _sctc.lib().sctc_brnn_forward(self._h, ctypes.byref(mb), out.data_ptr(),
                                           _sctc.current_stream_ptr())
        _sctc.check(rc, "costAndGrad(train=False)")
        if log and rows:
            _sctc.check(_sctc.lib().sctc_log_rows(out.data_ptr(), out.data_ptr(), rows, self.outputDim,
                                                  self.outputDim, _sctc.current_stream_ptr()), "forwardDevice")
        return out, T_b

    def forwardProbs(self, data_list):
        out, T_b = self.forwardDevice(data_list)
        host = out.cpu().numpy()
        res, o = [], 0
        for T in T_b:
            res.append(np.asfortranarray(host[o:o + T].T))
            o += T
        return res

    def evaluate(self, data_list, label_rows, decode="best", drop=(), lm=None, beam=40, alpha=1.0, beta=0.0,
                 cost=True):
        import ctc_fast
        torch = _sctc.require_gpu()
        if self._h is None:
            raise RuntimeError("initParams() / fromFile() first")
        if decode not in ("best", "beam"):
            raise ValueError("evaluate: decode must be 'best' or 'beam'")
        B = len(data_list)
        if len(label_rows) != B:
            raise ValueError("evaluate: %d transcripts for %d utterances" % (len(label_rows), B))
        refs = [np.ascontiguousarray(np.asarray(l).reshape(-1), dtype=np.int32) for l in label_rows]
        T_b = [int(np.asarray(d).shape[1]) for d in data_list]
        off = np.concatenate([[0], np.cumsum(T_b)]).astype(np.int64)
        A = self.outputDim
        probs = torch.empty((int(off[-1]), A), dtype=torch.float32, device="cuda")
        step = max(1, int(self.maxUtts))
        for g in range(0, B, step):
            self.forwardDevice(data_list[g:g + step], out=probs[int(off[g]):int(off[min(B, g + step)])])
        costs = skips = None
        if cost and B:
            costs, _, skips = ctc_fast.ctc_loss_batch(probs, refs, blank=0, lengths=T_b)
        if decode == "best":
            ids, lens, _, _ = ctc_fast.decode_best_path_batch(probs, lengths=T_b, blank=0, drop=drop, device=True)
        else:
            ctc_fast.log_rows(probs, out=probs)
            if isinstance(lm, ctc_fast.DecodeLexicon):
                ids, lens, _ = ctc_fast.decode_lexicon_beam_batch(probs, lengths=T_b, lexicon=lm, beam=beam,
                                                                  alpha=alpha, beta=beta, device=True)
            else:
                ids, lens, _ = ctc_fast.decode_beam_batch(probs, lengths=T_b, beam=beam, alpha=alpha, beta=beta,
                                                          lm=lm, device=True)
        lens_h = lens.cpu().numpy()[:B]
        U_b = np.array([r.shape[0] for r in refs], dtype=np.int32)
        ref_off = np.concatenate([[0], np.cumsum(U_b)]).astype(np.int64)
        ref_dev = torch.from_numpy(np.concatenate(refs + [np.zeros(1, dtype=np.int32)])).cuda()
        stats = ctc_fast.edit_distance_device(ref_dev, U_b, ref_off[:B], ids, lens_h, off[:B])
        ids_h = ids.cpu().numpy()
        return {"stats": stats.cpu().numpy(),
                "hyps": [ids_h[o:o + n].copy() for o, n in zip(off[:B], lens_h)],
                "cost": costs.cpu().numpy() if costs is not None else None,
                "skip": skips.cpu().numpy().astype(bool) if skips is not None else None}

    def updateParams(self, scale, update):
        if isinstance(update, TensorStack) and update.flat is not None \
                and update.flat.numel() == self._params.numel():
            _sctc.check(_sctc.lib().sctc_axpy(self._params.data_ptr(), update.flat.data_ptr(),
                                              float(scale), self._params.numel(),
                                              _sctc.current_stream_ptr()), "updateParams")
            return
        for params, paramsDel in zip(self.stack, update):
            w, b = params
            dw, db = paramsDel
            w.add_mult(dw, alpha=scale)
            b.add_mult(db, alpha=scale)

    def zerosLikeStack(self):
        torch = _sctc.require_gpu()
        return self._make_stack(torch.zeros_like(self._params))


    def toFile(self, fid):
        stack = []
# ... 55 lines not shown
```

Baseline: 813,000 frames/s.

## Overlap deferred upper-layer weight-gradient GEMMs with backward recurrent kernel on side stream

The weight-gradient GEMMs of the layers at and above the temporal layer are no longer run in order. They are held back and launched on a separate non-blocking stream. That stream waits (via stream wait-value on the recurrent kernel's residency words) until the persistent backward recurrent kernel is resident, so the GEMMs use the CUs the recurrence leaves idle. A new HALF variant of the recurrent T-kernel uses fewer blocks, and LDS is capped so GEMM workgroups can co-reside. Extra delta buffers are carved to break the ping-pong dependency. The cost is added complexity, possible contention that slows the latency-critical recurrence, and hang risk if residency signalling fails.

Result: faster. 837,200 frames/s, median of 6 (+3.0%).

```diff
diff --git a/include/sctc.h b/include/sctc.h
--- a/include/sctc.h
+++ b/include/sctc.h
@@ -438,6 +438,7 @@
                               double* side_dev, int32_t side_count, int32_t backward_queued);
 int sctc_brnn_check(sctc_brnn_t h, void* stream);
 int sctc_brnn_recurrent_path(sctc_brnn_t h, int32_t* forward_path, int32_t* bptt_path, int32_t* retries);
+int sctc_brnn_bwd_overlap_mode(sctc_brnn_t h);
 
 int sctc_brnn_forward(sctc_brnn_t h, const sctc_minibatch* mb, float* probs_dev, void* stream);
 
diff --git a/stanford-ctc_amd/_sctc.py b/stanford-ctc_amd/_sctc.py
--- a/stanford-ctc_amd/_sctc.py
+++ b/stanford-ctc_amd/_sctc.py
@@ -274,6 +274,7 @@
                                                      ctypes.c_int32, vp, vp, vp]),
     "sctc_brnn_check": (ctypes.c_int, [vp, vp]),
     "sctc_brnn_recurrent_path": (ctypes.c_int, [vp, c_i32p, c_i32p, c_i32p]),
+    "sctc_brnn_bwd_overlap_mode": (ctypes.c_int, [vp]),
     "sctc_brnn_grad_event": (vp, [vp, ctypes.c_int32]),
     "sctc_stream_wait_event": (ctypes.c_int, [vp, vp]),
     "sctc_brnn_forward": (ctypes.c_int, [vp, ctypes.POINTER(Minibatch), vp, vp]),
diff --git a/stanford-ctc_amd/csrc/brnn_engine.hip b/stanford-ctc_amd/csrc/brnn_engine.hip
--- a/stanford-ctc_amd/csrc/brnn_engine.hip
+++ b/stanford-ctc_amd/csrc/brnn_engine.hip
@@ -9,6 +9,7 @@
 #include <mutex>
 
 #include "brnn_mwer.h"
+#include "bwd_overlap_plan.h"
 #include "brnn_mwer_plan.h"
 #include "ctc_kernels.h"
 #include "elementwise.h"
@@ -52,6 +53,10 @@
     float *Z, *hF, *hB;
     float *logits, *probs, *dlogits;
     float *dA, *dBuf, *dF, *dBk;
+    float* dX[BWD_MAX_EXTRA] = {};
+    int n_dx = 0;
+    hipStream_t ov_stream = nullptr;
+    hipEvent_t ov_fork = nullptr, ov_join = nullptr;
     std::vector<uint16_t*> act16f, act16b;
     uint16_t *hF16b = nullptr, *hB16b = nullptr, *dF16b = nullptr, *dBk16b = nullptr;
     uint16_t *dlogits16 = nullptr, *dA16 = nullptr, *dBuf16 = nullptr;
@@ -97,6 +102,11 @@
     int rec_poll_delay = -1;
     int rec_variant = REC_V_AUTO;
     int rec_force_fallback = 0;
+    int rec_retrying = 0;
+    int bwd_overlap = BWD_OVERLAP_DEFAULT;
+    int bwd_overlap_last = 0;
+    hipEvent_t ov_ev[2] = {};
+    bool ov_timed = false;
     int rec_path[2] = {0, 0};
     int rec_retries = 0;
     const float* last_delta1 = nullptr;
@@ -175,6 +185,19 @@
     *count = cnt;
 }
 
+static int bwd_overlap_wanted()
+{
+    int mode = BWD_OVERLAP_DEFAULT;
+    if (const char* ov = getenv("SCTC_BWD_OVERLAP")) mode = atoi(ov) == 1 ? BWD_OVERLAP_CLAIM : (atoi(ov) == 2 ? BWD_OVERLAP_HALF : BWD_OVERLAP_OFF);
+    if (mode == BWD_OVERLAP_OFF) return mode;
+    int dev = 0, can = 0;
+    if (hipGetDevice(&dev) != hipSuccess || hipDeviceGetAttribute(&can, hipDeviceAttributeCanUseStreamWaitValue, dev) != hipSuccess) {
+        (void)hipGetLastError();
+        can = 0;
+    }
+    return can ? mode : BWD_OVERLAP_OFF;
+}
+
 static size_t carve(const sctc_brnn_config* c, const Dims& d, sctc_brnn* h, void* ws, size_t bytes)
 {
     Arena ar;
@@ -197,6 +220,10 @@
         dBuf = f(F * LD(d.Hp));
         if (d.TL > 0) { dF = f(F * LD(d.Hp)); dBk = f(F * LD(d.Hp)); }
     }
+    const int n_dx = Bm >= 17 && bwd_overlap_wanted() != BWD_OVERLAP_OFF
+                         ? bwd_overlap_extra_bufs(d.NL, d.TL, d.Hp, c->operand_dtype == SCTC_F32, c->train != 0) : 0;
+    float* dX[BWD_MAX_EXTRA] = {};
+    for (int k = 0; k < n_dx; ++k) dX[k] = f(F * LD(d.Hp));
     const bool h16 = c->operand_dtype == SCTC_F16;
     std::vector<uint16_t*> act16f(d.NL + 1, nullptr), act16b(d.NL + 1, nullptr), WT16b(d.NL + 1, nullptr);
     uint16_t *hF16b = nullptr, *hB16b = nullptr, *dF16b = nullptr, *dBk16b = nullptr, *dlogits16 = nullptr,
@@ -262,6 +289,8 @@
         h->d_idx_lo = d_idx_lo; h->d_idx_hi = d_idx_hi; h->d_perm = d_perm; h->d_xbase = d_xbase;
         h->ctc_ws = ctc_ws; h->ctc_ws_bytes = ctc_bytes;
         h->splitk_ws = splitk_ws; h->splitk_floats = sk;
+        h->n_dx = n_dx;
+        for (int k = 0; k < BWD_MAX_EXTRA; ++k) h->dX[k] = dX[k];
         h->xbuf = xbuf; h->counters = counters; h->rec_debug = rec_debug;
         h->act16f = act16f; h->act16b = act16b; h->WT16b = WT16b; h->W16f = W16f;
         h->hF16b = hF16b; h->hB16b = hB16b; h->dF16b = dF16b; h->dBk16b = dBk16b;
@@ -415,6 +444,38 @@
         g.splitk_ws = h->splitk_ws;
     }
     return launch_gemm_f32(g, s);
+}
+
+static int bwd_overlap_mode(const sctc_brnn* h)
+{
+    if (h->bwd_overlap == BWD_OVERLAP_OFF || h->n_dx == 0 || !h->ov_stream || h->Tmax < 2) return BWD_OVERLAP_OFF;
+    if (!bwd_overlap_eligible(h->NL, h->TL, h->Hp, h->cfg.operand_dtype == SCTC_F32, h->cfg.train != 0, h->B)) return BWD_OVERLAP_OFF;
+    if (h->rec_variant != REC_V_AUTO || h->rec_force_fallback || h->rec_retrying || h->profiling == 1 ||
+        recurrent_shared_device_mode())
+        return BWD_OVERLAP_OFF;
+    return h->bwd_overlap;
+}
+
+struct HeldGemms {
+    sctc_brnn* h;
+    hipStream_t s;
+    std::vector<GemmArgs> g;
+    bool timed, forked;
+};
+static int launch_held_beside(void* ctx)
+{
+    HeldGemms* hg = static_cast<HeldGemms*>(ctx);
+    sctc_brnn* h = hg->h;
+    SCTC_HIP_TRY(hipEventRecord(h->ov_fork, hg->s));
+    SCTC_HIP_TRY(hipStreamWaitEvent(h->ov_stream, h->ov_fork, 0));
+    hg->forked = true;
+    for (int g = 0; g < 2; ++g)
+        SCTC_HIP_TRY(hipStreamWaitValue32(h->ov_stream, rec_resident_word(h->counters, g), 2, hipStreamWaitValueGte, 0xFFFFFFFFu));
+    if (hg->timed) SCTC_HIP_TRY(hipEventRecord(h->ov_ev[0], h->ov_stream));
+    for (GemmArgs& g : hg->g) SCTC_TRY(launch_gemm(h, g, h->ov_stream));
+    if (hg->timed) SCTC_HIP_TRY(hipEventRecord(h->ov_ev[1], h->ov_stream));
+    SCTC_HIP_TRY(hipEventRecord(h->ov_join, h->ov_stream));
+    return SCTC_OK;
 }
 
 static const float* tensor_ptr(const sctc_brnn* h, const float* base, int idx)
@@ -550,8 +611,10 @@
                     attempt == 0 ? "under the device lease" : "on the per-step fallback");
         ++h->rec_retries;
         h->rec_force_fallback = attempt == 1;
+        h->rec_retrying = 1;
         rc = step();
         h->rec_force_fallback = 0;
+        h->rec_retrying = 0;
     }
     return rc;
 }
@@ -618,8 +681,14 @@
     const float* d_in = h->dlogits;
     const uint16_t* d_in16 = h->dlogits16;
     int d_in_ld = LD(h->Ap);
-    float* bufs[2] = {h->dA, h->dBuf};
-    uint16_t* bufs16[2] = {h->dA16, h->dBuf16};
+    const int ov = bwd_overlap_mode(h);
+    h->bwd_overlap_last = ov;
+    h->ov_timed = false;
+    BwdRoute route;
+    if (!bwd_route(h->NL, h->TL, ov != BWD_OVERLAP_OFF, &route)) return set_error(SCTC_ERR_ARG, "brnn: no delta buffer route for %d layers", h->NL);
+    const auto delta_buf = [&](int b) { return b == BWD_BUF_A ? h->dA : (b == BWD_BUF_B ? h->dBuf : h->dX[b - BWD_BUF_X0]); };
+    const auto delta_buf16 = [&](int b) { return b == BWD_BUF_A ? h->dA16 : (b == BWD_BUF_B ? h->dBuf16 : (uint16_t*)nullptr); };
+    HeldGemms held = {h, s, {}, false, false};
     if (h16) {
         SCTC_TRY(launch_cvt16(h->dlogits, nullptr, h->dlogits16, N * LD(h->Ap), s));
         for (int l = 1; l <= h->NL; ++l) {
@@ -628,7 +697,6 @@
             SCTC_TRY(launch_transpose_bf16(h->params + wl.offset, LD(h->Hp), h->WT16b[l], LD(outp), outp, h->Hp, s));
         }
     }
-    int which = 0;
     bool fused_sum = false;
     for (int i = h->NL; i >= 0; --i) {
         pt.begin(SCTC_PHASE_BWD_GEMM);
@@ -653,13 +721,18 @@
                 g.A = reinterpret_cast<const float*>(d_in16);
                 g.B = reinterpret_cast<const float*>(h->act16b[i]);
             }
-            SCTC_TRY(launch_gemm(h, g, s));
+            if (route.deferred[i]) {
+                held.g.push_back(g);
+            } else {
+                SCTC_TRY(launch_gemm(h, g, s));
+            }
             if (!(h->TL > 0 && i >= h->TL))
                 SCTC_HIP_TRY(hipEventRecord(h->grad_ev[weight_index(h, i)], s));
         }
         if (i == 0) break;
         pt.begin(SCTC_PHASE_BWD_GEMM);
-        float* d_out = bufs[which];
+        float* d_out = delta_buf(route.d_out[i]);
+        uint16_t* d_out16 = delta_buf16(route.d_out[i]);
         {
             GemmArgs g = gemm_args({d_in, d_in_ld, 1}, {W, LD(inp), 0}, N, inp, outp, d_out, LD(inp), bprec);
             if (i != h->TL) { g.mask = h->act[i]; g.ldmask = LD(h->Hp); }
@@ -669,7 +742,7 @@
                 g.B = reinterpret_cast<const float*>(h->WT16b[i]);
                 g.ldb = LD(outp);
                 g.b_kcontig = 1;
-                g.C16b = bufs16[which];
+                g.C16b = d_out16;
                 g.ldc16 = LD(inp);
                 if (i != h->TL) {
                     g.mask = nullptr;
@@ -681,13 +754,35 @@
             SCTC_TRY(launch_gemm(h, g, s));
         }
         if (i == h->TL) {
-            pt.begin(SCTC_PHASE_BWD_REC);
-            const RecArgs r = rec_args(h, true, d_out);
-            SCTC_TRY(launch_recurrent(r, s, &h->rec_path[1]));
+            RecArgs r = rec_args(h, true, d_out);
+            if (ov == BWD_OVERLAP_OFF) {
+                pt.begin(SCTC_PHASE_BWD_REC);
+                SCTC_TRY(launch_recurrent(r, s, &h->rec_path[1]));
+            } else {
+                held.timed = h->profiling == 2 && h->ov_ev[0];
+                pt.begin(SCTC_PHASE_BWD_REC);
+                r.variant = ov == BWD_OVERLAP_HALF ? REC_V_T_HALF : REC_V_T_CLAIM;
+                RecBeside beside = {launch_held_beside, &held, 0};
+                const int rc = launch_recurrent(r, s, &h->rec_path[1], &beside);
+                if (held.forked) {
+                    if (rc != SCTC_OK)
+                        for (int g = 0; g < 2; ++g) (void)hipMemsetD32Async((hipDeviceptr_t)rec_resident_word(h->counters, g), 2, 1, s);
+                    if (h->profiling == 2) pt.mark(-1);
+                    const hipError_t je = hipStreamWaitEvent(s, h->ov_join, 0);
+                    if (rc == SCTC_OK) SCTC_HIP_TRY(je);
+                    h->ov_timed = held.timed && rc == SCTC_OK;
+                }
+                SCTC_TRY(rc);
+                pt.begin(SCTC_PHASE_BWD_GEMM);
+                if (!held.forked) {
+                    for (GemmArgs& g : held.g) SCTC_TRY(launch_gemm(h, g, s));
+                    h->bwd_overlap_last = BWD_OVERLAP_OFF;
+                }
+            }
             for (int l = h->NL; l >= h->TL; --l)
                 SCTC_HIP_TRY(hipEventRecord(h->grad_ev[weight_index(h, l)], s));
             pt.begin(SCTC_PHASE_BWD_GEMM);
-            if (h16) SCTC_TRY(launch_add16(nullptr, h->dF, h->dBk, nullptr, bufs16[which], N * LD(h->Hp), s,
+            if (h16) SCTC_TRY(launch_add16(nullptr, h->dF, h->dBk, nullptr, d_out16, N * LD(h->Hp), s,
                                            h->dF16b, h->dBk16b));
             for (int k = 0; k < 2; ++k) {
                 const sctc_tensor_info& ri = h->tinfo[k == 0 ? wf_index(h) : wb_index(h)];
@@ -727,9 +822,8 @@
             }
         }
         d_in = d_out;
-        d_in16 = bufs16[which];
+        d_in16 = d_out16;
         d_in_ld = LD(h->Hp);
-        which ^= 1;
     }
     h->last_delta1 = d_in;
     h->last_delta1_16 = h16 ? d_in16 : nullptr;
@@ -1070,6 +1164,16 @@
     const char* pd = getenv("SCTC_REC_POLL_DELAY");
     h->rec_poll_delay = pd ? atoi(pd) : -1;
     if (const char* fa = getenv("SCTC_FUSE_ADD")) h->fuse_add = atoi(fa) != 0;
+    h->bwd_overlap = bwd_overlap_wanted();
+    if (h->bwd_overlap != BWD_OVERLAP_OFF && h->n_dx > 0) {
+        if (hipStreamCreateWithFlags(&h->ov_stream, hipStreamNonBlocking) != hipSuccess ||
+            hipEventCreateWithFlags(&h->ov_fork, hipEventDisableTiming) != hipSuccess ||
+            hipEventCreateWithFlags(&h->ov_join, hipEventDisableTiming) != hipSuccess) {
+            (void)hipGetLastError();
+            if (h->ov_stream) (void)hipStreamDestroy(h->ov_stream);
+            h->ov_stream = nullptr;
+        }
+    }
     const char* dbg = getenv("SCTC_REC_DEBUG");
     h->rec_debug_on = dbg ? atoi(dbg) : 0;
     *out = h;
@@ -1089,6 +1193,12 @@
         if (e) (void)hipEventDestroy(e);
     for (hipEvent_t e : h->tev)
         if (e) (void)hipEventDestroy(e);
+    for (hipEvent_t e : {h->ov_ev[0], h->ov_ev[1], h->ov_fork, h->ov_join})
+        if (e) (void)hipEventDestroy(e);
+    if (h->ov_stream) {
+        (void)hipStreamSynchronize(h->ov_stream);
+        (void)hipStreamDestroy(h->ov_stream);
+    }
     delete h;
     return SCTC_OK;
 }
@@ -1310,6 +1420,8 @@
     return SCTC_OK;
 }
 
+int sctc_brnn_bwd_overlap_mode(sctc_brnn_t h) { return h ? h->bwd_overlap_last : -1; }
+
 int sctc_brnn_recurrent_path(sctc_brnn_t h, int32_t* forward_path, int32_t* bptt_path, int32_t* retries)
 {
     SCTC_CHECK_ARG(h, "brnn_recurrent_path: null handle");
@@ -1480,6 +1592,7 @@
     if (enable == 2 && h->tev.empty()) {
         h->tev.resize(128);
         for (hipEvent_t& e : h->tev) SCTC_HIP_TRY(hipEventCreate(&e));
+        for (hipEvent_t& e : h->ov_ev) SCTC_HIP_TRY(hipEventCreate(&e));
     }
     h->profiling = enable == 2 ? 2 : (enable ? 1 : 0);
     h->tev_n = 0;
@@ -1497,6 +1610,11 @@
             float ms = 0.f;
             SCTC_HIP_TRY(hipEventElapsedTime(&ms, h->tev[i], h->tev[i + 1]));
             h->phase_ms[h->tev_phase[i]] += ms;
+        }
+        if (h->ov_timed) {
+            float gemm = 0.f;
+            SCTC_HIP_TRY(hipEventElapsedTime(&gemm, h->ov_ev[0], h->ov_ev[1]));
+            h->phase_ms[SCTC_PHASE_BWD_GEMM] += gemm;
         }
     }
     memcpy(ms_out, h->phase_ms, sizeof(h->phase_ms));
diff --git a/stanford-ctc_amd/csrc/bwd_overlap_plan.h b/stanford-ctc_amd/csrc/bwd_overlap_plan.h
--- /dev/null
+++ b/stanford-ctc_amd/csrc/bwd_overlap_plan.h
@@ -0,0 +1,79 @@
+#pragma once
+
+namespace sctc {
+
+enum BwdOverlapMode : int {
+    BWD_OVERLAP_OFF = 0,
+    BWD_OVERLAP_CLAIM = 1,
+    BWD_OVERLAP_HALF = 2,
+};
+static constexpr int BWD_OVERLAP_DEFAULT = BWD_OVERLAP_HALF;
+
+enum BwdBuf : int { BWD_BUF_LOGITS = 0, BWD_BUF_A = 1, BWD_BUF_B = 2, BWD_BUF_X0 = 3 };
+static constexpr int BWD_MAX_EXTRA = 5;
+static constexpr int BWD_MAX_LAYERS = 64;
+
+static inline int bwd_overlap_hh_above(int NL, int TL) { return TL > 0 && TL < NL ? NL - TL : 0; }
+
+static inline bool bwd_overlap_config_ok(int NL, int TL, int Hp, bool fp32, bool train)
+{
+    const int hh = bwd_overlap_hh_above(NL, TL);
+    return train && fp32 && (Hp == 1824 || Hp == 2048) && hh >= 2 && hh - 1 <= BWD_MAX_EXTRA && NL < BWD_MAX_LAYERS;
+}
+static inline int bwd_overlap_extra_bufs(int NL, int TL, int Hp, bool fp32, bool train)
+{
+    return bwd_overlap_config_ok(NL, TL, Hp, fp32, train) ? bwd_overlap_hh_above(NL, TL) - 1 : 0;
+}
+static inline bool bwd_overlap_eligible(int NL, int TL, int Hp, bool fp32, bool train, int B)
+{
+    return bwd_overlap_config_ok(NL, TL, Hp, fp32, train) && B >= 17 && B <= 32;
+}
+
+struct BwdRoute {
+    int d_in[BWD_MAX_LAYERS];
+    int d_out[BWD_MAX_LAYERS];
+    bool deferred[BWD_MAX_LAYERS];
+};
+
+static inline bool bwd_route(int NL, int TL, bool overlap, BwdRoute* r)
+{
+    if (NL < 0 || NL >= BWD_MAX_LAYERS) return false;
+    if (overlap && (bwd_overlap_hh_above(NL, TL) < 2 || bwd_overlap_hh_above(NL, TL) - 1 > BWD_MAX_EXTRA)) return false;
+    int d_in = BWD_BUF_LOGITS;
+    for (int i = NL; i >= 0; --i) {
+        r->d_in[i] = d_in;
+        r->deferred[i] = overlap && i >= TL;
+        r->d_out[i] = -1;
+        if (i == 0) break;
+        const bool front = overlap && i >= TL;
+        const int k = front || !overlap ? NL - i : TL - 1 - i;
+        r->d_out[i] = front && k >= 2 ? BWD_BUF_X0 + (k - 2) : (k % 2 ? BWD_BUF_B : BWD_BUF_A);
+        d_in = r->d_out[i];
+    }
+    return true;
+}
+
+static inline int bwd_route_check(int NL, int TL, bool overlap, const BwdRoute& r)
+{
+    int writer[BWD_BUF_X0 + BWD_MAX_EXTRA + 1];
+    for (int& w : writer) w = -1;
+    writer[BWD_BUF_LOGITS] = NL + 1;
+    const auto read_ok = [&](int i) { return r.d_in[i] >= 0 && r.d_in[i] <= BWD_BUF_X0 + BWD_MAX_EXTRA && writer[r.d_in[i]] == i + 1; };
+    const auto delta = [&](int i) {
+        if (!read_ok(i) || r.d_out[i] <= BWD_BUF_LOGITS || r.d_out[i] > BWD_BUF_X0 + BWD_MAX_EXTRA || r.d_out[i] == r.d_in[i]) return false;
+        writer[r.d_out[i]] = i;
+        return true;
+    };
+    const int first_serial = overlap ? TL - 1 : NL;
+    if (overlap) {
+        for (int i = NL; i >= TL; --i) if (i >= 1 && !delta(i)) return i + 1;
+        for (int i = NL; i >= TL; --i) if (!r.deferred[i] || !read_ok(i)) return i + 1;
+    }
+    for (int i = first_serial; i >= 0; --i) {
+        if (r.deferred[i] || !read_ok(i)) return i + 1;
+        if (i >= 1 && !delta(i)) return i + 1;
+    }
+    return 0;
+}
+
+}
diff --git a/stanford-ctc_amd/csrc/recurrent.h b/stanford-ctc_amd/csrc/recurrent.h
--- a/stanford-ctc_amd/csrc/recurrent.h
+++ b/stanford-ctc_amd/csrc/recurrent.h
@@ -50,7 +50,13 @@
 static constexpr int REC_PATH_PERSISTENT = 1;
 static constexpr int REC_PATH_PERSISTENT_LEASED = 2;
 static constexpr int REC_PATH_FALLBACK = 3;
-int launch_recurrent(const RecArgs& a, hipStream_t stream, int* path = nullptr);
+struct RecBeside {
+    int (*fn)(void* ctx);
+    void* ctx;
+    int called;
+};
+static inline unsigned* rec_resident_word(unsigned* counters, int g) { return counters + 32 + (size_t)(g * 2 * 64) * REC_FLAG_STRIDE; }
+int launch_recurrent(const RecArgs& a, hipStream_t stream, int* path = nullptr, RecBeside* beside = nullptr);
 int recurrent_clear_error(unsigned* counters, hipStream_t stream);
 int recurrent_shared_device_mode();
 void recurrent_set_shared_device_mode(int on);
diff --git a/stanford-ctc_amd/csrc/recurrent.hip b/stanford-ctc_amd/csrc/recurrent.hip
--- a/stanford-ctc_amd/csrc/recurrent.hip
+++ b/stanford-ctc_amd/csrc/recurrent.hip
@@ -532,7 +532,7 @@
     static_for_seq(std::make_integer_sequence<int, N>(), static_cast<F&&>(f));
 }
 
-template <int NCQ, int NREGF, int NT, int NBAT, int R, int PUB, int PB, int UG = 2>
+template <int NCQ, int NREGF, int NT, int NBAT, int R, int PUB, int PB, int UG = 2, int HALF = 0>
 __global__ __launch_bounds__(256, 1) void brnn_recurrent_t_kernel(RecArgs p)
 {
     extern __shared__ __attribute__((aligned(16))) float4 lds4[];
@@ -542,6 +542,7 @@
     constexpr int NC = UG * NT;
     constexpr int NPL = UG == 1 ? 2 : 1;
     static_assert(UG == 1 || UG == 2, "16 or 32 units per block");
+    static_assert(!HALF || (UG == 2 && NT == 1), "both tiles of a direction: 32 units, one tile per sub-chain");
     static_assert(NC <= 4 && NPL * NC <= 4, "one result per wave, one 16-byte flag load per lane");
     static_assert(NBAT % R == 0 && NBAT >= 2 * R && R >= 2, "ring");
     static_assert((NBAT - 1) * XB < NCQ, "no empty batch");
@@ -551,7 +552,8 @@
     const int tid = threadIdx.x, lane = tid & 63;
     const int wave = __builtin_amdgcn_readfirstlane(tid >> 6);
     const int Hp = p.Hp, nch = Hp >> 4, nprod = nch / UG;
-    const int combo = blockIdx.x & (2 * UG - 1), ublk = blockIdx.x / (2 * UG);
+    constexpr int NCOMBO = HALF ? 2 : 2 * UG;
+    const int combo = blockIdx.x & (NCOMBO - 1), ublk = blockIdx.x / NCOMBO;
     const int g = combo & 1, half = combo >> 1;
     const int row0 = ublk * 16 * UG;
     const int uj = lane & 15, kq = lane >> 4;
@@ -618,7 +620,7 @@
     auto init_sub = [&](Sub& S, int sub) {
 #pragma unroll
         for (int i = 0; i < NT; ++i) {
-            const int tile = (i * 2 + sub) * UG + half;
+            const int tile = HALF ? i * 2 + sub : (i * 2 + sub) * UG + half;
             S.trow[i] = (unsigned)tile * 16u;
             S.ub[i] = tile * 16 + uj;
             S.uT[i] = S.ub[i] < p.B ? p.T_b[S.ub[i]] : 0;
@@ -1454,7 +1456,8 @@
     SCTC_REC_T(X, 29, 25, 1, 8, 4, 1, 5, 2) SCTC_REC_T(X, 29, 25, 1, 6, 3, 1, 4, 2) SCTC_REC_T(X, 29, 25, 1, 8, 2, 1, 7, 2) \
     SCTC_REC_T(X, 29, 25, 2, 6, 3, 1, 4, 2) SCTC_REC_T(X, 29, 25, 2, 8, 4, 1, 5, 2) SCTC_REC_T(X, 29, 25, 2, 8, 2, 1, 7, 2) \
     SCTC_REC_T(X, 32, 31, 1, 8, 4, 1, 5, 2) SCTC_REC_T(X, 32, 31, 1, 6, 3, 1, 4, 2)                             \
-    SCTC_REC_T(X, 32, 31, 2, 8, 4, 1, 5, 2) SCTC_REC_T(X, 32, 31, 2, 6, 3, 1, 4, 2)
+    SCTC_REC_T(X, 32, 31, 2, 8, 4, 1, 5, 2) SCTC_REC_T(X, 32, 31, 2, 6, 3, 1, 4, 2)                             \
+    SCTC_REC_T(X, 29, 25, 1, 8, 4, 1, 5, 2, 1) SCTC_REC_T(X, 32, 31, 1, 8, 4, 1, 5, 2, 1)
 
 static RecKernel rec_kernel(const RecCandidate& c)
 {
@@ -1543,6 +1546,7 @@
     hipStream_t stream;
     int* path;
     int tcfg;
+    RecBeside* beside;
 };
 
 static int read_error_word(const RecArgs& a, hipStream_t stream, unsigned* e)
@@ -1581,6 +1585,10 @@
         return SCTC_OK;
     }
     SCTC_TRY(g_gate.admit_and_launch(cx.dev, cx.stream, need_cus, cx.cus, [&]() -> int {
+        if (cx.beside && !cx.beside->called && smem >= REC_LDS_EXCLUDES_GEMM) {
+            cx.beside->called = 1;
+            SCTC_TRY(cx.beside->fn(cx.beside->ctx));
+        }
         hipLaunchKernelGGL(k, dim3(grid), dim3(REC_THREADS), smem, cx.stream, a);
         SCTC_HIP_TRY(hipGetLastError());
         return SCTC_OK;
@@ -1621,7 +1629,7 @@
     return SCTC_OK;
 }
 
-int launch_recurrent(const RecArgs& a_in, hipStream_t stream, int* path)
+int launch_recurrent(const RecArgs& a_in, hipStream_t stream, int* path, RecBeside* beside)
 {
     RecArgs a = a_in;
     if (a.poll_delay < 0) a.poll_delay = a.Hp > 1024 ? 5 : 0;
@@ -1641,6 +1649,8 @@
     cx.cus = 0;
     static const int tcfg = getenv("SCTC_REC_TCFG") ? atoi(getenv("SCTC_REC_TCFG")) : 0;
     cx.tcfg = tcfg;
+    cx.beside = nullptr;
+    if (beside) beside->called = 0;
     SCTC_HIP_TRY(hipGetDevice(&cx.dev));
     SCTC_HIP_TRY(hipDeviceGetAttribute(&cx.cus, hipDeviceAttributeMultiprocessorCount, cx.dev));
     for (int b0 = 0; b0 < a_in.B;) {
@@ -1652,6 +1662,7 @@
         c.B = nb;
         if (a_in.T_host) c.Tmax = std::min(a_in.Tmax, (int)a_in.T_host[b0]);
         if (c.variant == REC_V_NO_CUT) c.variant = REC_V_AUTO;
+        cx.beside = (b0 == 0 && nb == a_in.B) ? beside : nullptr;
         SCTC_TRY(launch_recurrent_one(c, cx));
         b0 += nb;
     }
diff --git a/stanford-ctc_amd/csrc/recurrent_plan.h b/stanford-ctc_amd/csrc/recurrent_plan.h
--- a/stanford-ctc_amd/csrc/recurrent_plan.h
+++ b/stanford-ctc_amd/csrc/recurrent_plan.h
@@ -16,6 +16,8 @@
     REC_V_SLAB_LARGE = 47,
     REC_V_T_SMALL = 50,
     REC_V_Q_AT_32 = 51,
+    REC_V_T_HALF = 52,
+    REC_V_T_CLAIM = 53,
     REC_V_NO_PIPE = 40,
     REC_V_ROW_MAJOR = 46,
     REC_V_Q_LINEAR = 2,
@@ -26,7 +28,7 @@
 static inline bool rec_variant_known(int v)
 {
     for (int known : {REC_V_AUTO, REC_V_SLAB, REC_V_FALLBACK, REC_V_S_TO_8, REC_V_Q_FROM_1, REC_V_NO_CUT, REC_V_SLAB_LARGE,
-                      REC_V_T_SMALL, REC_V_Q_AT_32, REC_V_NO_PIPE, REC_V_ROW_MAJOR, REC_V_Q_LINEAR, REC_V_Q_PRIO_DIR,
+                      REC_V_T_SMALL, REC_V_Q_AT_32, REC_V_T_HALF, REC_V_T_CLAIM, REC_V_NO_PIPE, REC_V_ROW_MAJOR, REC_V_Q_LINEAR, REC_V_Q_PRIO_DIR,
                       REC_V_Q_PRIO_TILE, REC_V_Q_PRIO_PARITY, REC_V_T_STALE})
         if (v == known) return true;
     return false;
@@ -50,7 +52,7 @@
 
 struct RecCandidate {
     RecFamily family;
-    int ntarg, targ[8];
+    int ntarg, targ[9];
     int grid;
     size_t lds;
     int per_cu;
@@ -58,7 +60,7 @@
     int linear_map;
     int variant;
 };
-static constexpr int REC_MAX_CANDIDATES = 5;
+static constexpr int REC_MAX_CANDIDATES = 6;
 
 struct RecTForm { int nregf, nbat, r, pub, pb; };
 constexpr RecTForm rec_t84(int nregf) { return {nregf, 8, 4, 1, 5}; }
@@ -91,6 +93,7 @@
 }
 
 static constexpr size_t REC_LDS_MAX = 160 * 1024, REC_F4 = 16;
+static constexpr size_t REC_LDS_EXCLUDES_GEMM = REC_LDS_MAX - 16 * 1024;
 static inline size_t rec_lds_q(const RecSize& r) { return REC_F4 * ((size_t)4 * (r.ncq - r.nreg) * 64 + 3 * 64); }
 static inline size_t rec_lds_s(int Hp, int sb) { return sizeof(float) * 2 * sb * Hp; }
 static inline size_t rec_lds_mh(int Hp) { return (((size_t)16 * (Hp + 8) * 2 + 15) / 16) * 16 + 3 * 64 * REC_F4; }
@@ -117,9 +120,12 @@
                          std::max(rec_lds_t(r, f, nt, ug), lds_min), 1, 0);
 }
 
-static inline int rec_plan(const RecShape& s, RecCandidate out[REC_MAX_CANDIDATES])
+static inline int rec_plan(const RecShape& s_in, RecCandidate out[REC_MAX_CANDIDATES])
 {
-    if (!rec_variant_known(s.variant)) return -1;
+    if (!rec_variant_known(s_in.variant)) return -1;
+    RecShape s = s_in;
+    const bool t_half = s_in.variant == REC_V_T_HALF, t_claim = s_in.variant == REC_V_T_CLAIM;
+    if (t_half || t_claim) s.variant = REC_V_AUTO;
     const int nwg = s.Hp / 16, ntiles = (s.B + 15) / 16, v = s.variant, B = s.B, sb = B <= 4 ? 4 : 8;
     const RecSize* r = rec_size(s.Hp);
     const int tcfg = s.tcfg >= 0 && s.tcfg <= 3 ? s.tcfg : 0;
@@ -135,8 +141,14 @@
         out[n++] = rec_candidate(s, REC_FAM_S, {r->nk, sb}, 2 * nwg, rec_lds_s(s.Hp, sb), 2, 4);
     if (persistent && r && s.prec16 && B > 5 && B <= 16 && v != REC_V_SLAB && rec_lds_mh(s.Hp) <= REC_LDS_MAX)
         out[n++] = rec_candidate(s, REC_FAM_MH, {r->nch, s.transpose != 0}, 2 * nwg, rec_lds_mh(s.Hp), 1, 2);
+    if (t_half && persistent && r && r->t_default && ntiles == 2 && !s.prec16) {
+        RecCandidate c = rec_candidate_t(s, *r, r->t_one[0], 1, 2, REC_LDS_EXCLUDES_GEMM);
+        c.targ[c.ntarg++] = 1;
+        c.grid = 2 * (s.Hp / 32);
+        out[n++] = c;
+    }
     if (persistent && r && r->t_ug1[tcfg].nbat && ntiles == 2 && !s.prec16 && (v == REC_V_AUTO || v == REC_V_ROW_MAJOR || v == REC_V_T_STALE))
-        out[n++] = rec_candidate_t(s, *r, r->t_ug1[tcfg], 1, 1, (size_t)81 * 1024);
+        out[n++] = rec_candidate_t(s, *r, r->t_ug1[tcfg], 1, 1, t_claim ? REC_LDS_EXCLUDES_GEMM : (size_t)81 * 1024);
     if (persistent && r && ntiles == 2 && v != REC_V_SLAB && 4 * nwg <= 2 * s.cus)
         out[n++] = rec_candidate(s, REC_FAM_Q, {r->ncq, r->nreg}, 4 * nwg, rec_lds_q(*r), 2, 0);
     if (persistent && ntiles > 2 && rec_tiled_large(s))
diff --git a/stanford-ctc_amd/nnets/brnnet.py b/stanford-ctc_amd/nnets/brnnet.py
--- a/stanford-ctc_amd/nnets/brnnet.py
+++ b/stanford-ctc_amd/nnets/brnnet.py
@@ -476,6 +476,9 @@
                                                          ctypes.byref(r)), "recurrentPath")
         return f.value, b.value, r.value
 
+    def bwdOverlapMode(self):
+        return int(_sctc.lib().sctc_brnn_bwd_overlap_mode(self._h))
+
     def debugBuffer(self, which):
         torch = _sctc.require_gpu()
         ptr, rows, cols, ld = ctypes.c_void_p(), ctypes.c_int64(), ctypes.c_int64(), ctypes.c_int64()
```
